# ArthurBrussee/brush

Hardware: AMD Instinct MI355X
Metric: train views/sec @ 1M Gaussians, 1080p (fwd + L1/SSIM loss + bwd + Adam per view) (higher is better)
Workload: dtype f32

## Files before the change

brush_amd/__init__.py:

```python
from .host import (
    Camera, Context, RasterPass, RenderAux, SplatTrainer, Splats, TrainConfig, SceneBatch,
    get_context, image_loss, image_loss_backward, image_loss_value_and_grad, prefix_sum, radix_argsort, tile_sort_offsets, render_splats,
    render_splats_bwd, adam_step, gather_stats, RefineStats, splat_bounds, bounds_median_size, fov_to_focal, focal_to_fov,
    splat_to_ply, load_splat_from_ply, ply_parse_header, ParseMetadata, BatchUploader, SceneLoader, set_list_slicing, last_list_counts, set_view_id,
    render_splats_diff, RenderNode, compute_pup_scores, decimate_to_count, lod_target_count, pup_accumulate, pup_accumulate_view, pup_scores,
    knn_log_scales, to_init_splats, load_init_splats, ply_vertex_has_property, EvalSample, EvalResult, eval_metrics, eval_stats, run_eval,
    Lpips, lpips, lpips_value_and_grad, splat_to_compressed_ply, view_output_size, resize_image, render_depth,
    PoseOptimizer, pose_twist, ExposureTable, depth_loss_value_and_grad, eval_depth_metrics,
    splat_normals, render_normal, depth_to_normal, depth_to_normal_backward, normal_consistency_value_and_grad,
    render_distortion, distortion_loss, BilateralGridTable,
    TsdfVolume, mesh_to_ply, fuse_views,
    render_features, feature_loss_value_and_grad, FeatureField,
    SceneTransform, SceneRegion, select_region, crop_splats,
    LiftAccumulator, lift_labels, compact_splats,
    EnvironmentMap,
)
from ._ffi import BrushHipError
```

brush_amd/_ffi.py:

```python
import ctypes as C
import os

_DIR = os.path.dirname(os.path.abspath(__file__))
LIB_PATH = os.environ.get("BRUSH_HIP_LIB") or os.path.join(_DIR, "libbrush_hip.so")

FLAG_MIP = 1
FLAG_BWD_INFO = 2
FLAG_SMOOTH_CUTOFF = 4
FLAG_SLICED_LISTS = 8

fp = C.POINTER(C.c_float)
u32p = C.POINTER(C.c_uint32)


class BhCamera(C.Structure):
    _fields_ = [
        ("vm", C.c_float * 12),
        ("fx", C.c_float), ("fy", C.c_float), ("cx", C.c_float), ("cy", C.c_float),
        ("lim_pos_x", C.c_float), ("lim_pos_y", C.c_float),
        ("lim_neg_x", C.c_float), ("lim_neg_y", C.c_float),
        ("cam_pos", C.c_float * 3),
        ("img_w", C.c_uint32), ("img_h", C.c_uint32),
        ("tile_row_begin", C.c_uint32), ("tile_row_end", C.c_uint32),
        ("model", C.c_uint32), ("dist", C.c_float * 8), ("half_max_render_fov", C.c_float),
# ... 353 lines not shown
REGION_BOX, REGION_ELLIPSOID = 0, 1


class BhSceneTransform(C.Structure):
    _fields_ = [("q", C.c_double * 4), ("t", C.c_double * 3), ("s", C.c_double), ("rot", C.c_float * 9), ("quat", C.c_float * 4),
                ("trans", C.c_float * 3), ("scale", C.c_float), ("log_scale", C.c_float), ("sh_rot", C.c_float * 164),
                ("reserved", C.c_uint32 * 2)]


class BhSceneRegion(C.Structure):
    _fields_ = [("kind", C.c_uint32), ("invert", C.c_uint32), ("center", C.c_float * 3), ("half_extent", C.c_float * 3),
                ("rot", C.c_float * 9), ("min_raw_opacity", C.c_float), ("reserved", C.c_uint32)]


SCENE_SYMBOLS = {
    "bh_scene_transform_make": (C.c_int, [dp, dp, C.c_double, C.POINTER(BhSceneTransform)]),
    "bh_scene_transform_compose": (C.c_int, [C.POINTER(BhSceneTransform), C.POINTER(BhSceneTransform), C.POINTER(BhSceneTransform)]),
    "bh_scene_transform_invert": (C.c_int, [C.POINTER(BhSceneTransform), C.POINTER(BhSceneTransform)]),
    "bh_camera_apply_scene_transform": (C.c_int, [C.POINTER(BhCamera), C.POINTER(BhSceneTransform), C.POINTER(BhCamera)]),
    "bh_splats_transform": (C.c_int, [C.c_void_p, C.POINTER(BhSceneTransform), C.c_uint32, C.c_uint32] + [C.c_void_p] * 6),
    "bh_splats_select_region": (C.c_int, [C.c_void_p, C.POINTER(BhSceneRegion), C.c_void_p, C.c_void_p, C.c_uint32, C.c_void_p, u32p]),
}

LIFT_MAX_LABELS, LIFT_UNASSIGNED, LIFT_ANY_LABEL = 256, 255, 0xFFFFFFFF
LIFT_VOTE_ONE = 16777216.0


class BhLiftSelect(C.Structure):
    _fields_ = [("label", C.c_uint32), ("min_share", C.c_float), ("min_weight", C.c_float), ("min_max_weight", C.c_float),
                ("min_pixels", C.c_uint32), ("invert", C.c_uint32)]


LIFT_SYMBOLS = {
    "bh_lift_accumulate": (C.c_int, [C.c_void_p, C.POINTER(BhRenderOut), C.c_void_p, C.c_uint32, C.c_void_p, C.c_void_p, C.c_void_p]),
    "bh_lift_assign": (C.c_int, [C.c_void_p, C.c_void_p, C.c_uint32, C.c_uint32, C.c_float, C.c_void_p, C.c_void_p]),
    "bh_lift_select": (C.c_int, [C.c_void_p, C.c_void_p, C.c_void_p, C.c_void_p, C.c_uint32, C.c_uint32, C.POINTER(BhLiftSelect), C.c_void_p]),
}

ENVMAP_MAX_RESOLUTION = 1024
ENVMAP_SYMBOLS = {
    "bh_envmap_create": (C.c_int, [C.c_void_p, C.c_uint32, C.POINTER(C.c_void_p)]),
    "bh_envmap_destroy": (C.c_int, [C.c_void_p, C.c_void_p]),
    "bh_envmap_set_params": (C.c_int, [C.c_void_p, C.c_void_p, fp]),
    "bh_envmap_get_params": (C.c_int, [C.c_void_p, C.c_void_p, fp]),
    "bh_envmap_get_grad": (C.c_int, [C.c_void_p, C.c_void_p, fp]),
    "bh_envmap_get_state": (C.c_int, [C.c_void_p, C.c_void_p, fp, fp, u32p]),
    "bh_envmap_set_state": (C.c_int, [C.c_void_p, C.c_void_p, fp, fp, C.c_uint32]),
    "bh_envmap_set_adam": (C.c_int, [C.c_void_p, C.c_void_p, C.c_double, C.c_double, C.c_double, C.c_double]),
    "bh_envmap_composite": (C.c_int, [C.c_void_p, C.c_void_p, C.POINTER(BhCamera), C.c_void_p, C.c_uint32, C.c_uint32, C.c_void_p]),
    "bh_envmap_backward": (C.c_int, [C.c_void_p, C.c_void_p, C.POINTER(BhCamera), C.c_void_p, C.c_void_p, C.c_uint32, C.c_uint32, C.c_void_p, C.c_int]),
    "bh_train_set_envmap": (C.c_int, [C.c_void_p, C.c_void_p]),
}

ABI_VERSION = 7
STRUCT_MIRRORS = (BhCamera, BhRenderOut, BhLossConfig, BhTrainConfig, BhTrainState, BhTrainBatch, BhTrainStats, BhRefineConfig, BhRefineStats, BhPlyInfo)

_lib = None
_lib_th = None
TEST_HOOKS_LIB_PATH = os.path.join(_DIR, "libbrush_hip_testhooks.so")
TEST_HOOK_SYMBOLS = {"bh_debug_fill_train_scratch": (C.c_int, [C.c_void_p, C.c_uint32]),
                     "bh_debug_split_counts": (C.c_int, [C.c_void_p, C.POINTER(C.c_uint32)])}


class BrushHipError(RuntimeError):
    pass


def _bind(path, symbols):
    if not os.path.exists(path):
        raise BrushHipError(
            "%s not found: build it with `python -c 'import __graft_entry__ as g; g.build()'` "
            "(hipcc --offload-arch=gfx950). There is no CPU fallback." % path)
    lib = C.CDLL(path)
    for name, (res, args) in symbols.items():
        fn = getattr(lib, name)
        fn.restype = res
        fn.argtypes = args
    if lib.bh_abi_version() != ABI_VERSION:
        raise BrushHipError("%s speaks ABI %d, this binding ABI %d" % (path, lib.bh_abi_version(), ABI_VERSION))
    for i, mirror in enumerate(STRUCT_MIRRORS):
        if lib.bh_struct_size(i) != C.sizeof(mirror):
            raise BrushHipError("%s: sizeof(%s) is %d in the library, %d in this binding" % (path, mirror.__name__, lib.bh_struct_size(i), C.sizeof(mirror)))
    return lib


def load():
    global _lib
    if _lib is None:
        _lib = _bind(LIB_PATH, dict(SYMBOLS, **LPIPS_SYMBOLS, **COMPRESSED_PLY_SYMBOLS, **IMAGE_SYMBOLS, **DEPTH_SYMBOLS, **POSE_SYMBOLS, **EXPOSURE_SYMBOLS, **BILAGRID_SYMBOLS, **DEPTH_LOSS_SYMBOLS, **NORMAL_SYMBOLS, **NORMAL_LOSS_SYMBOLS, **DISTORTION_SYMBOLS, **MESH_SYMBOLS, **FEATURE_SYMBOLS, **FEATURE_TRAIN_SYMBOLS, **SCENE_SYMBOLS, **LIFT_SYMBOLS, **ENVMAP_SYMBOLS))
    return _lib


def load_test_hooks():
    global _lib_th
    if _lib_th is None:
        _lib_th = _bind(TEST_HOOKS_LIB_PATH, dict(SYMBOLS, **LPIPS_SYMBOLS, **COMPRESSED_PLY_SYMBOLS, **IMAGE_SYMBOLS, **DEPTH_SYMBOLS, **POSE_SYMBOLS, **EXPOSURE_SYMBOLS, **BILAGRID_SYMBOLS, **DEPTH_LOSS_SYMBOLS, **NORMAL_SYMBOLS, **NORMAL_LOSS_SYMBOLS, **DISTORTION_SYMBOLS, **MESH_SYMBOLS, **FEATURE_SYMBOLS, **FEATURE_TRAIN_SYMBOLS, **SCENE_SYMBOLS, **LIFT_SYMBOLS, **ENVMAP_SYMBOLS,
                                                   **TEST_HOOK_SYMBOLS))
    return _lib_th
```

brush_amd/csrc/api.hip:

```cpp
#include <cmath>
#include <cstdlib>
#include <cstdio>
#include <algorithm>
#include <cstring>
#include <new>

#include "context.h"
#include "device_rng.h"
#include "param_table.h"

namespace bh {

__global__ __launch_bounds__(256) void zero_two_kernel(float4* __restrict__ a, size_t na, float4* __restrict__ b, size_t nb) {
    const size_t stride = (size_t)gridDim.x * 256;
    const float4 z = make_float4(0.0f, 0.0f, 0.0f, 0.0f);
    for (size_t i = (size_t)blockIdx.x * 256 + threadIdx.x; i < na + nb; i += stride) {
        if (i < na) a[i] = z;
        else b[i - na] = z;
    }
}

int set_error(bh_ctx* ctx, int code, const std::string& msg) {
    if (ctx) ctx->last_error = msg;
    return code;
// ... 317 lines not shown
        return true;
    }},
    {"cut_sort_all", "0|1: with per-tile cuts, still depth-sort every visible splat",
     [](bh_ctx* c, const char* v) { return parse_flag(v, &c->knob_cut_sort_all); }},
    {"auto_exact_share", "0..1: a view whose last cut frame listed more than this share of its pairs renders complete lists (default 0.9; 0 = never)", [](bh_ctx* c, const char* v) {
        char* end = nullptr;
        const float x = strtof(v, &end);
        if (end == v || *end != '\0' || !(x >= 0.0f && x <= 1.0f)) return false;
        c->auto_exact_share = x;
        return true;
    }},
    {"no_view_hash", "0|1: frames without a view id share ONE table instead of being keyed by their camera",
     [](bh_ctx* c, const char* v) { return parse_flag(v, &c->knob_no_view_hash); }},
    {"k16_order", "0 index order | 1 by the view's last per-tile work | 2 dealt: the forward blend's tile order",
     [](bh_ctx* c, const char* v) { return parse_u32(v, 0, 2, &c->knob_k16_order); }},
    {"band_mode", "0|1: XCD bands of the blend kernels — contiguous eighths of the tile range, or dealt in chunks of 8 adjacent tiles (default 1)",
     [](bh_ctx* c, const char* v) { return parse_u32(v, 0, 1, &c->knob_band_mode); }},
    {"k16_waves", "0..8: forward blend: resident one-wave tiles per SIMD (0 = 8 = all resident at once; fewer: the lighter tiles are dispatched as the heavier ones finish)",
     [](bh_ctx* c, const char* v) { return parse_u32(v, 0, 8, &c->knob_k16_waves); }},
    {"k16_split", "0..1000: forward blend: a tile whose forecast work is at least max(256, k16_split / 100 x its band's mean) is blended by four quadrant waves (default 250; 0: no tile is split)",
     [](bh_ctx* c, const char* v) { return parse_u32(v, 0, 1000, &c->knob_k16_split); }},
    {"k16_split_of_max", "0..100: ... and at least this many percent of its band's heaviest tile (default 45)",
     [](bh_ctx* c, const char* v) { return parse_u32(v, 0, 100, &c->knob_k16_split_of_max); }},
    {"k16_split_min", "1..1023: a tile below this many blended splats (forecast) is never split (default 256)",
     [](bh_ctx* c, const char* v) { return parse_u32(v, 1, 1023, &c->knob_k16_split_min); }},
    {"k5_exact_spw", "16|32|64: splats per wave of the list builder for complete lists",
     [](bh_ctx* c, const char* v) { uint32_t u = 0; if (!parse_u32(v, 16, 64, &u) || !(u == 16 || u == 32 || u == 64)) return false; c->knob_k5_exact_spw = u; return true; }},
    {"bwd_jobs", "0|1: the blend backward works on checkpointed 128-entry segments of the tiles' lists (default 1) or on whole tiles",
     [](bh_ctx* c, const char* v) { return parse_flag(v, &c->knob_bwd_jobs); }},
    {"bwd_wide_rows", "0|1: the blend backward addresses the gradient accumulator in 64 bits, as it does by itself from 2^32 bytes of accumulator on (default 0)",
     [](bh_ctx* c, const char* v) { return parse_flag(v, &c->knob_bwd_wide_rows); }},
    {"no_lpt", "0|1: the blend backward takes its tiles in index order",
     [](bh_ctx* c, const char* v) { return parse_flag(v, &c->knob_no_lpt); }},
    {"lpt_classes", "log|linear: work classes of the backward's longest-first tile order — two per octave of blended splats, or 1/64 of the mean list length wide",
     [](bh_ctx* c, const char* v) { const std::string w(v); if (w == "log") { c->knob_lpt_linear = false; return true; } if (w == "linear") { c->knob_lpt_linear = true; return true; } return false; }},
    {"generic_depth_sort", "0|1: depth order by the generic radix sort + scan instead of the fused split sort",
     [](bh_ctx* c, const char* v) { return parse_flag(v, &c->knob_generic_depth_sort); }},
    {"dsort_splitters", "0|1: the fused depth sort splits at the 254 depth quantiles of the view's previous frame (default 1) or always linearly over the frame's key range",
     [](bh_ctx* c, const char* v) { return parse_flag(v, &c->knob_dsort_splitters); }},
    {"tile_sort", "auto|bucket|lsd: the forward's tile sort (auto: bucket sort unless the view's pairs are concentrated in few tiles)",
     [](bh_ctx* c, const char* v) { const std::string w(v); if (w == "auto") { c->knob_tile_sort = 0; return true; } if (w == "bucket") { c->knob_tile_sort = 1; return true; } if (w == "lsd") { c->knob_tile_sort = 2; return true; } return false; }},
    {"spec_k5", "0|1: queue the list builder before the host has read the frame's counts (default 1; 0: behind the count readback)",
     [](bh_ctx* c, const char* v) { return parse_flag(v, &c->knob_spec_k5); }},
    {"event_waits", "0|1: the host's mid-step waits use events behind the kernels instead of polled tag words",
     [](bh_ctx* c, const char* v) { return parse_flag(v, &c->knob_event_waits); }},
    {"readback_copy", "0|1: counts and gate word reach the host through copy launches",
     [](bh_ctx* c, const char* v) { return parse_flag(v, &c->knob_readback_copy); }},
    {"force_exchange", "0|1: a one-rank communicator still walks the whole gradient-exchange path (overhead measurement)",
     [](bh_ctx* c, const char* v) { return parse_flag(v, &c->knob_force_exchange); }},
    {"zero_grads", "0|1: the single-GPU train step zero-fills its gradient span like the exchange path",
     [](bh_ctx* c, const char* v) { return parse_flag(v, &c->knob_zero_grads); }},
    {"loss_bands", "0|1: the fused loss's blocks take their tiles by XCD column bands (1) or row-major (0)",
     [](bh_ctx* c, const char* v) { return parse_u32(v, 0, 1, &c->knob_loss_bands); }},
    {"update_rows", "0|64|128|256: splats per block of the update kernel (0 = default)",
     [](bh_ctx* c, const char* v) { uint32_t u = 0; if (!parse_u32(v, 0, 256, &u) || !(u == 0 || u == 64 || u == 128 || u == 256)) return false; c->knob_update_rows = u; return true; }},
    {"no_dormant", "0|1: the update kernel fetches and updates dormant splats like everyone else",
     [](bh_ctx* c, const char* v) { return parse_flag(v, &c->knob_no_dormant); }},
    {"sort_kpt", "0|4|8|16: keys per thread of the generic radix sort (0 = default)",
     [](bh_ctx* c, const char* v) { uint32_t u = 0; if (!parse_u32(v, 0, 16, &u) || !(u == 0 || u == 4 || u == 8 || u == 16)) return false; c->knob_sort_kpt = u; return true; }},
    {"grad_allreduce", "ring|direct: the dense gradient block's collective — ncclAllReduce, or reduce-scatter + all-gather over grouped send/recv",
     [](bh_ctx* c, const char* v) { const std::string w(v); if (w == "ring") { c->knob_direct_allreduce = false; return true; } if (w == "direct") { c->knob_direct_allreduce = true; return true; } return false; }},
    {"update_sparse", "0..256: an update block with at most this many non-dormant rows fetches them in one round trip (0: never; 256: every block that may skip dormant rows; default 64 at SH degree 0, else 0)",
     [](bh_ctx* c, const char* v) { uint32_t u = 0; if (!parse_u32(v, 0, 256, &u)) return false; c->knob_update_sparse = (int)u; return true; }},
    {"feature_chunk", "0|4|8|16: channels per pass over the lists of the feature-map blends (0 = chosen per channel count)",
     [](bh_ctx* c, const char* v) { uint32_t u = 0; if (!parse_u32(v, 0, 16, &u) || !(u == 0 || u == 4 || u == 8 || u == 16)) return false; c->feature_chunk = u; return true; }},
};
constexpr int kOptionCount = (int)(sizeof(kOptions) / sizeof(kOptions[0]));
}

extern "C" int bh_option_count(void) { return kOptionCount; }
extern "C" const char* bh_option_name(int i) { return i >= 0 && i < kOptionCount ? kOptions[i].name : nullptr; }
extern "C" const char* bh_option_help(int i) { return i >= 0 && i < kOptionCount ? kOptions[i].help : nullptr; }

extern "C" int bh_set_option(bh_ctx* ctx, const char* key, const char* value) {
    if (!ctx) return BH_ERR_INVALID_ARG;
    if (!key || !value) return set_error(ctx, BH_ERR_INVALID_ARG, "set_option: null key or value");
    const std::string k(key);
    for (const Option& o : kOptions) {
        if (k != o.name) continue;
        if (!o.apply(ctx, value)) return set_error(ctx, BH_ERR_INVALID_ARG, "set_option: bad value '" + std::string(value) + "' for '" + k + "'");
        return 0;
    }
    return set_error(ctx, BH_ERR_INVALID_ARG, "set_option: unknown key '" + k + "' (bh_option_name lists the keys)");
}

namespace {
struct Kb4Law {
    double k[4];
    explicit Kb4Law(const float* d) { for (int i = 0; i < 4; ++i) k[i] = d ? (double)d[i] : 0.0; }
    double value(double th) const {
        const double t2 = th * th, t3 = t2 * th, t5 = t3 * t2, t7 = t5 * t2, t9 = t7 * t2;
        return th + k[0] * t3 + k[1] * t5 + k[2] * t7 + k[3] * t9;
    }
    double slope(double th) const {
        const double t2 = th * th, t4 = t2 * t2, t6 = t4 * t2, t8 = t6 * t2;
        return 1.0 + 3.0 * k[0] * t2 + 5.0 * k[1] * t4 + 7.0 * k[2] * t6 + 9.0 * k[3] * t8;
    }
    double invert(double target) const {
        if (target <= 0.0) return 0.0;
        const double pi = 3.14159265358979323846;
        double th = target < pi - 1e-6 ? target : pi - 1e-6;
        for (int it = 0; it < 50; ++it) {
            const double fp = slope(th);
            if (std::fabs(fp) < 1e-12) break;
            double next = th - (value(th) - target) / fp;
            next = next < 0.0 ? 0.0 : (next > pi ? pi : next);
// ... 750 lines not shown
    BH_HIP(ctx, hipMemcpyAsync(info, ctx->slots[SLOT_SLICE].ptr, sizeof info, hipMemcpyDeviceToHost, ctx->stream));
    BH_HIP(ctx, hipStreamSynchronize(ctx->stream));
    deliver_pending_loss(ctx);
    *near_pairs = info[1];
    *far_pairs = info[2] ? info[3] : 0u;
    return 0;
}

const float* bh_last_v_combined(bh_ctx* ctx) { return ctx ? (const float*)ctx->slots[SLOT_V_COMBINED].ptr : nullptr; }

int bh_radix_argsort(bh_ctx* ctx, const uint32_t* keys, const uint32_t* vals, uint32_t n, uint32_t bits,
                     uint32_t* out_keys, uint32_t* out_vals) {
    if (!ctx) return BH_ERR_INVALID_ARG;
    if (n > 0 && (!keys || !out_keys || !out_vals)) return set_error(ctx, BH_ERR_INVALID_ARG, "radix_argsort: null argument");
    BH_HIP(ctx, hipSetDevice(ctx->device));
    return radix_argsort(ctx, keys, vals, n, bits, out_keys, out_vals);
}

int bh_prefix_sum(bh_ctx* ctx, const uint32_t* in, uint32_t n, uint32_t* out) {
    if (!ctx) return BH_ERR_INVALID_ARG;
    if (n > 0 && (!in || !out)) return set_error(ctx, BH_ERR_INVALID_ARG, "prefix_sum: null argument");
    BH_HIP(ctx, hipSetDevice(ctx->device));
    return prefix_sum(ctx, in, nullptr, n, out, false);
}

int bh_image_loss_forward(bh_ctx* ctx, const float* pred_chw, const uint32_t* gt_packed, uint32_t channels, uint32_t h,
                          uint32_t w, const BhLossConfig* cfg, float* loss_map) {
    if (!ctx) return BH_ERR_INVALID_ARG;
    if (!pred_chw || !gt_packed || !cfg || !loss_map || h == 0 || w == 0) return set_error(ctx, BH_ERR_INVALID_ARG, "image_loss_forward: bad argument");
    BH_HIP(ctx, hipSetDevice(ctx->device));
    return launch_image_loss_forward(ctx, pred_chw, gt_packed, channels, h, w, *cfg, loss_map);
}

int bh_image_loss_backward(bh_ctx* ctx, const float* pred_chw, const uint32_t* gt_packed, const float* dl_dmap,
                           uint32_t channels, uint32_t h, uint32_t w, const BhLossConfig* cfg, float* dl_dpred) {
    if (!ctx) return BH_ERR_INVALID_ARG;
    if (!pred_chw || !gt_packed || !dl_dmap || !cfg || !dl_dpred || h == 0 || w == 0) return set_error(ctx, BH_ERR_INVALID_ARG, "image_loss_backward: bad argument");
    BH_HIP(ctx, hipSetDevice(ctx->device));
    return launch_image_loss_backward(ctx, pred_chw, gt_packed, dl_dmap, 0.0f, channels, h, w, *cfg, dl_dpred);
}

int bh_image_loss_value_and_grad(bh_ctx* ctx, const float* img_hwc4, const uint32_t* gt_packed, uint32_t h, uint32_t w,
                                 const BhLossConfig* cfg, float alpha_weight, float* loss_out, float* v_output) {
    if (!ctx) return BH_ERR_INVALID_ARG;
    if (!img_hwc4 || !gt_packed || !cfg || !loss_out || !v_output || h == 0 || w == 0)
        return set_error(ctx, BH_ERR_INVALID_ARG, "image_loss_value_and_grad: bad argument");
    BH_HIP(ctx, hipSetDevice(ctx->device));
    const size_t hw = (size_t)h * w;
    const bool alpha = alpha_weight > 0.0f;
    return launch_image_loss_fused(ctx, img_hwc4, gt_packed, h, w, *cfg, alpha, 1.0f / (float)(hw * 3), alpha ? alpha_weight / (float)hw : 0.0f,
                                   loss_out, v_output);
}

int bh_adam_step(bh_ctx* ctx, float* param, const float* grad, float* m1, float* m2, uint64_t rows, uint32_t row_len,
                 const float* col_scale, float lr, uint32_t t, int reduce_m2, float beta1, float beta2, float eps) {
    if (!ctx) return BH_ERR_INVALID_ARG;
    if (rows > 0 && (!param || !grad || !m1 || !m2)) return set_error(ctx, BH_ERR_INVALID_ARG, "adam_step: null argument");
    BH_HIP(ctx, hipSetDevice(ctx->device));
    return launch_adam(ctx, param, grad, m1, m2, rows, row_len, col_scale, lr, t, reduce_m2 != 0, beta1, beta2, eps);
}

int bh_gather_stats(bh_ctx* ctx, float* refine_weight_norm, float* vis_weight, float* max_screen_size,
                    const float* refine_weight, const float* visible, const float* screen_radius, uint64_t n) {
    if (!ctx) return BH_ERR_INVALID_ARG;
    BH_HIP(ctx, hipSetDevice(ctx->device));
    return launch_gather_stats(ctx, refine_weight_norm, vis_weight, max_screen_size, refine_weight, visible, screen_radius, n);
}

void bh_philox4x32_10(const uint32_t ctr[4], const uint32_t key[2], uint32_t out[4]) {
    const Philox4 r = philox4x32_10(ctr[0], ctr[1], ctr[2], ctr[3], key[0], key[1]);
    out[0] = r.x; out[1] = r.y; out[2] = r.z; out[3] = r.w;
}

void bh_sample_background(uint64_t seed, uint32_t step, const float base[3], float strength, float out[3]) {
    float u[3] = {0.5f, 0.5f, 0.5f};
    if (strength > 0.0f) {
        const Philox4 r = philox4x32_10(0u, step, 0u, RNG_STREAM_BACKGROUND, (uint32_t)seed, (uint32_t)(seed >> 32));
        u[0] = unit_open(r.x); u[1] = unit_open(r.y); u[2] = unit_open(r.z);
    }
    for (int k = 0; k < 3; ++k) {
        const float v = strength > 0.0f ? base[k] + (2.0f * u[k] - 1.0f) * strength : base[k];
        out[k] = v < 0.0f ? 0.0f : (v > 1.0f ? 1.0f : v);
    }
}

int bh_normal_samples(bh_ctx* ctx, uint64_t seed, uint32_t step, uint64_t n, float* out) {
    if (!ctx) return BH_ERR_INVALID_ARG;
    if (n > 0 && !out) return set_error(ctx, BH_ERR_INVALID_ARG, "normal_samples: null argument");
    if (n > 0xFFFFFFFFull) return set_error(ctx, BH_ERR_INVALID_ARG, "normal_samples: n must fit 32 bits (the splat index is one counter word)");
    BH_HIP(ctx, hipSetDevice(ctx->device));
    return launch_normal_samples(ctx, out, n, seed, step);
}

int bh_fold_min_scale(bh_ctx* ctx, const float* transforms, const float* raw_opacities, const float* min_scale, uint32_t n,
                      float* out_transforms, float* out_raw_opacities) {
    if (!ctx) return BH_ERR_INVALID_ARG;
    if (n > 0 && (!transforms || !raw_opacities || !min_scale || !out_transforms || !out_raw_opacities))
        return set_error(ctx, BH_ERR_INVALID_ARG, "fold_min_scale: null argument");
    BH_HIP(ctx, hipSetDevice(ctx->device));
    return launch_fold_min_scale(ctx, transforms, raw_opacities, min_scale, n, out_transforms, out_raw_opacities);
}

int bh_fold_min_scale_backward(bh_ctx* ctx, const float* transforms, const float* raw_opacities, const float* min_scale, uint32_t n,
                               float* v_transforms, float* v_raw_opacities) {
    if (!ctx) return BH_ERR_INVALID_ARG;
    if (n > 0 && (!transforms || !raw_opacities || !min_scale || !v_transforms || !v_raw_opacities))
// ... 44 lines not shown
```

brush_amd/csrc/context.h:

```cpp
#pragma once
#include <hip/hip_runtime.h>
#include <stdint.h>

#include <memory>
#include <string>
#include <unordered_map>
#include <vector>

#include "../../include/brush_hip.h"
#include "../../include/brush_hip_lpips.h"
#include "../../include/brush_hip_image.h"
#include "../../include/brush_hip_exposure.h"
#include "../../include/brush_hip_bilagrid.h"
#include "../../include/brush_hip_depth_loss.h"
#include "../../include/brush_hip_normal_loss.h"
#include "../../include/brush_hip_distortion.h"
#include "../../include/brush_hip_mesh.h"
#include "../../include/brush_hip_features.h"
#include "../../include/brush_hip_feature_train.h"
#include "../../include/brush_hip_envmap.h"
#include "device_math.h"

namespace bh {

enum Slot : int {
    SLOT_COUNTERS = 0,
    SLOT_DEPTH_KEYS,
    SLOT_ISECT_COUNTS,
    SLOT_MAX_RADIUS,
    SLOT_SORT_KEYS_A,
    SLOT_SORT_KEYS_B,
    SLOT_SORT_VALS_A,
    SLOT_SORT_VALS_B,
    SLOT_SORT_HIST,
    SLOT_COMM_SCRATCH,
    SLOT_BWD_CKPT,
    SLOT_BWD_TOPLIST,
    SLOT_SORT_PARTS,
    SLOT_SCAN_SUMS,
    SLOT_GLOBAL_FROM_COMPACT,
    SLOT_DEPTHS_SORTED,
    SLOT_CUM_TILES_HIT,
    SLOT_PROJECTED,
    SLOT_TILE_IDS,
    SLOT_ISECT_GIDS,
    SLOT_TILE_IDS_SORTED,
    SLOT_ISECT_GIDS_SORTED,
    SLOT_TILE_OFFSETS,
    SLOT_OUT_IMG,
    SLOT_VISIBLE,
    SLOT_V_COMBINED,
    SLOT_LOSS_MAP,
    SLOT_V_OUTPUT,
    SLOT_GRADS,
    SLOT_STATS,
    SLOT_LOSS_SCALAR,
    SLOT_MISC,
    SLOT_REFINE,
    SLOT_REFINE_BOUNDS,
    SLOT_FOLDED_TRANSFORMS,
    SLOT_FOLDED_RAW_OPAC,
    SLOT_PLY_ROWS,
    SLOT_EXCH_BLOCKS,
    SLOT_EXCH_IDX,
    SLOT_EXCH_COMPACT,
    SLOT_PROJECTED_BY_GID,
    SLOT_SLICE,
    SLOT_SLICE_STATE,
    SLOT_SLICE_COUNTS,
    SLOT_SLICE_CUM,
    SLOT_NEAR_COUNTS,
    SLOT_TILE_ORDER,
    SLOT_LOD_GRADS,
// ... 227 lines not shown
struct ParamTable;

struct DistortionTerm {
    const float* v_distortion = nullptr;
    float gain = 0.0f;
    uint32_t kind = 0;
    float near_z = 0.0f, far_z = 0.0f;
    const float* moments = nullptr;
};

struct FeatureTerm {
    const float* features = nullptr;
    uint32_t channels = 0;
    const float* v_map = nullptr;
    float* v_features = nullptr;
    const float* map_acc = nullptr;
    const float* compact = nullptr;
};

struct BackwardCall {
    const float* transforms = nullptr;
    const float* sh_coeffs = nullptr;
    const float* raw_opacities = nullptr;
    float* v_transforms = nullptr;
    float* v_sh_coeffs = nullptr;
    float* v_raw_opacities = nullptr;
    float* v_refine_weight = nullptr;
    size_t span_floats = 0;
    bool want_refine = true;
    const DepthTerm* depth = nullptr;
    const NormalTerm* normal = nullptr;
    const DistortionTerm* distortion = nullptr;
    const FeatureTerm* feature = nullptr;
    float* v_viewmat = nullptr;
};

struct StepTerms {
    const bh_lpips* lpips = nullptr;
    float lpips_weight = 0.0f;
    float* pose_grad = nullptr;
    bool depth_attached = false;
    BhDepthTarget depth_target{};
    bool normal_attached = false;
    BhNormalTermConfig normal_term{};
    bool distortion_attached = false;
    BhDistortionTermConfig distortion_term{};
    bool feature_attached = false;
    BhFeatureField feature_field{};
    BhFeatureTarget feature_target{};
    bh_exposure* exposure = nullptr;
    bh_bilagrid* bilagrid = nullptr;
    float bilagrid_tv_weight = 0.0f;
    bh_envmap* envmap = nullptr;

    bool lpips_on() const { return lpips != nullptr && lpips_weight > 0.0f; }
    bool depth_on() const { return depth_attached && depth_target.weight > 0.0f; }
    bool normal_on() const { return normal_attached && normal_term.weight > 0.0f; }
    bool distortion_on() const { return distortion_attached; }
    bool feature_on() const { return feature_attached && feature_target.weight > 0.0f; }
};

}


struct bh_ctx {
    int device = 0;
    hipStream_t stream = nullptr;
    bool owns_stream = false;
    std::string last_error;
    bh::Buffer slots[bh::SLOT_COUNT];
    uint32_t* host_counters = nullptr;
    hipEvent_t readback_ev = nullptr;
    hipEvent_t gate_ev = nullptr;
    bool counters_ready = false;
    uint32_t counter_phase = 0;
    bool have_forward = false;
    bh::ForwardState latest;
    uint64_t generation = 0;
    std::vector<bh::Retained> retained;
    std::vector<bh::Buffer> pool;
    bh::GradClears clears;
    float* pending_loss_dst = nullptr;
    void* image_tab_host = nullptr;
    size_t image_tab_cap = 0;
    hipEvent_t image_tab_ev = nullptr;
    bh::StepTerms terms;
    std::vector<bh::ParamTable*> param_tables;
    void* comm = nullptr;
    hipStream_t comm_stream = nullptr;
    hipEvent_t comm_ev = nullptr;
    int comm_rank = 0, comm_world = 1;
    float slice_fraction = 0.0f;
    float last_slice_share = 1.0f;
    bool far_direct = false;
    uint32_t readback_tag = 0;
    uint32_t gate_tag = 0;
    bool gate_signal_queued = false;
    bool gate_learn = false;
    uint32_t far_launches = 0;
    std::unordered_map<uint64_t, bh::ViewState> views;
    uint64_t seen_keys[bh::SEEN_KEYS] = {};
    uint32_t seen_pos = 0;
    uint32_t casual_views = 0;
    uint32_t view_id = 0;
    uint64_t view_clock = 0;
    float margin_scale = 1.0f;
    float ctrl_up = 1.5f, ctrl_down = 0.998f, ctrl_floor = 0.5f, ctrl_gap_exp = 1.0f / 3.0f;
    uint32_t cut_min_pairs = bh::CUT_MIN_PAIRS;
    bool knob_spec_k5 = true;
    bool knob_event_waits = false;
    bool knob_readback_copy = false;
    bool knob_no_view_hash = false;
    bool knob_fixed_margin = false;
    bool knob_cut_sort_all = false;
    uint32_t feature_chunk = 0;
    uint32_t knob_band_mode = 1;
    uint32_t knob_k16_waves = 0;
    uint32_t knob_k16_split = 250;
    uint32_t knob_k16_split_min = bh::SPLIT_MIN_WORK;
    uint32_t knob_k16_split_of_max = 45;
    const uint32_t* last_split = nullptr;
    uint32_t knob_k16_order = 1;
    uint32_t knob_cut_margin_pct = 150;
    bh::FarJob far_job;
    uint32_t refine_n = 0, refine_new_n = 0;
    bool dsort_lds_raised = false;
    uint32_t* sort_groups = nullptr;
    size_t sort_groups_cap = 0, sort_groups_dirty = 0;
    uint32_t sort_groups_cur = 0;
    uint32_t* dsort_spl = nullptr;
    bool dsort_spl_written = false;
    bool knob_dsort_splitters = true;
    bool adam_lds_raised = false;
    uint32_t update_lds_raised = 0;
    size_t lds_optin_max = 0;
    bool knob_no_lpt = false;
    bool knob_bwd_wide_rows = false;
    bool knob_bwd_jobs = true;
    bool knob_lpt_linear = false;
    bool knob_force_exchange = false;
    bool knob_break_allreduce = false;
    bool knob_generic_depth_sort = false;
    bool knob_zero_grads = false;
    uint32_t knob_fail_loss_at = 0;
    uint32_t train_steps_seen = 0;
    uint32_t knob_loss_bands = 1;
    uint32_t knob_tile_sort = 0;
    float auto_exact_share = 0.9f;
    bool knob_direct_allreduce = false;
    uint32_t knob_k5_exact_spw = 32;
    bool knob_no_dormant = false;
    int knob_update_sparse = -1;
    uint32_t knob_update_rows = 0;
    uint32_t knob_sort_kpt = 0;
    const void* marks_m2_sh = nullptr; const void* marks_m1_t = nullptr; uint32_t marks_n = 0, marks_step = 0;
    bh::Profiler prof;
};

namespace bh {

int set_error(bh_ctx* ctx, int code, const std::string& msg);
int forward_impl(bh_ctx* ctx, const ForwardRequest& req, BhRenderOut* out);
int wait_host_tag(bh_ctx* ctx, const volatile uint32_t* word, uint32_t want, const char* what);
int find_saved_bwd_forward(bh_ctx* ctx, const BhRenderOut* saved, int not_bwd_code, const char* who, const ForwardState** fs);
int backward_impl(bh_ctx* ctx, const ForwardState& fs, const float* v_output, const BackwardCall& call);
int render_forward(bh_ctx* ctx, const ForwardRequest& req, BhRenderOut* out);
enum : uint32_t { NEED_V_OUTPUT = 1u, NEED_V_DEPTH = 2u, NEED_V_NORMAL = 4u, NEED_V_DISTORTION = 8u, NEED_V_VIEWMAT = 16u, NEED_V_FEATURES = 32u };
int backward_entry(bh_ctx* ctx, const char* who, int not_bwd_code, uint32_t required, const BhRenderOut* saved, const float* v_output, BackwardCall call);
int launch_depth_backward(bh_ctx* ctx, const ForwardState& fs, const DepthTerm& term, float* v_combined, float** v_z);
int launch_depth_vz_scatter(bh_ctx* ctx, const ForwardState& fs, const float* v_z, float* v_transforms, bool mark_rows, float* v_sh_coeffs,
                            float* v_raw_opacities, float* v_refine_weight);
int launch_depth_forward(bh_ctx* ctx, const ForwardState& fs, uint32_t mode, float* out_depth);
int launch_normal_backward(bh_ctx* ctx, const ForwardState& fs, const NormalTerm& term, const float* transforms, float* v_combined, const float** v_n);
int launch_normal_vn_scatter(bh_ctx* ctx, const ForwardState& fs, const float* v_n, const float* transforms, float* v_transforms, bool mark_rows,
                             float* v_sh_coeffs, float* v_raw_opacities, float* v_refine_weight);
int launch_normal_map(bh_ctx* ctx, const ForwardState& fs, const float* transforms, uint32_t mode, float* out);
int launch_normal_loss(bh_ctx* ctx, const BhCamera& cam, const float* normal, const float* depth, const float* image, uint32_t h, uint32_t w, float weight,
                       bool accumulate_v_depth, float* loss, float* v_normal, float* v_depth, float* accum, float* accum_host);
int launch_distortion_backward(bh_ctx* ctx, const ForwardState& fs, const DistortionTerm& term, float* v_combined, float** v_z);
int launch_distortion_map(bh_ctx* ctx, const ForwardState& fs, const DistortionTerm& term, bool moments, float* out);
int check_distortion_kind(bh_ctx* ctx, uint32_t kind, float near_z, float far_z, const char* who);
int launch_distortion_loss(bh_ctx* ctx, const float* map, uint32_t h, uint32_t w, uint32_t channels, float weight, float* loss, float* accum,
                           float* accum_host);
int launch_feature_backward(bh_ctx* ctx, const ForwardState& fs, const FeatureTerm& term, float* v_combined, const float** v_compact);
int launch_feature_scatter(bh_ctx* ctx, const ForwardState& fs, const FeatureTerm& term, const float* v_compact);
int launch_feature_gather(bh_ctx* ctx, const ForwardState& fs, const float* features, uint32_t channels, float* feat);
int launch_feature_forward(bh_ctx* ctx, const ForwardState& fs, uint32_t channels, const float* feat, float* out);
int feature_term_rows(bh_ctx* ctx, const ForwardState& fs, uint32_t channels, float** feat);
int launch_feature_loss(bh_ctx* ctx, const float* map, const BhFeatureTarget& t, float* loss, float* v_map, float* accum, float* accum_host);
int launch_depth_loss(bh_ctx* ctx, const float* depth, const BhDepthTarget& t, float* loss, float* v_depth, float* accum, float* accum_host);
double* loss_partials(bh_ctx* ctx, uint64_t pixels, uint32_t* blocks);
int launch_loss_pair_final(bh_ctx* ctx, uint32_t rows, const double* partials, float c, float* loss, float* accum, float* accum_host);
int launch_pose_grad(bh_ctx* ctx, const ViewUniforms& u, uint32_t nv, bool mip, uint32_t sh_degree, const float* transforms,
                     const float* sh, const uint32_t* gid, const float* v_combined, float* v_viewmat);
int launch_exposure_apply(bh_ctx* ctx, const bh_exposure* tab, uint32_t view, const float* img, uint32_t h, uint32_t w, float* out);
int launch_exposure_backward(bh_ctx* ctx, bh_exposure* tab, uint32_t view, const float* img, const float* v_exposed, uint32_t h, uint32_t w,
                             float* v_img, bool update);
int launch_bilagrid_slice(bh_ctx* ctx, const bh_bilagrid* tab, uint32_t view, const float* img, uint32_t h, uint32_t w, float* out);
// ... 95 lines not shown
                         float* projected, const uint32_t* cum_tiles_hit, uint32_t* tile_ids, uint32_t* isect_gids,
                         float4* zero_span = nullptr, uint32_t zero_f4 = 0, uint32_t budget = 0xFFFFFFFFu, uint32_t* slice_info = nullptr,
                         const uint32_t* zcut = nullptr, const uint32_t* depth_keys_sorted = nullptr, const uint32_t* nv_dev = nullptr, uint32_t pair_cap = 0xFFFFFFFFu);
int launch_map_gaussians_far(bh_ctx* ctx, uint32_t nv, const ViewUniforms& u, const float* projected_by_gid, const uint32_t* gid,
                             float* projected, const uint32_t* cum_tiles_hit, uint32_t budget, const uint32_t* done_bits, const uint32_t* gate,
                             uint32_t* counts, uint32_t* block_totals, uint32_t* group_totals, uint32_t* slice_info, uint32_t* tile_ids, uint32_t* isect_gids);
int launch_project_backward(bh_ctx* ctx, const ViewUniforms& u, uint32_t nv, bool mip, uint32_t sh_degree,
                            const float* transforms, const float* sh, const float* raw_opac, const uint32_t* gid,
                            float* v_combined, float* v_transforms, float* v_sh, float* v_raw_opac,
                            float* v_refine, bool mark_written = false, const float* projected = nullptr);
struct SortGroups {
    uint32_t* sums = nullptr;
    uint32_t* stale = nullptr;
    uint32_t stale_words = 0;
};
inline uint32_t sort_group_count(uint32_t nblocks) { return (nblocks + SORT_GROUP_BLOCKS - 1u) / SORT_GROUP_BLOCKS; }
int sort_groups_next(bh_ctx* ctx, size_t words, SortGroups* out);
constexpr uint32_t SORT_DIRECT_GROUPS = 32;
inline bool sort_groups_scanned(uint32_t ngroups) { return ngroups > SORT_DIRECT_GROUPS; }
int sort_groups_scan(bh_ctx* ctx, uint32_t* sums, uint32_t ngroups, uint32_t tables, uint32_t* totals);
int radix_argsort(bh_ctx* ctx, const uint32_t* keys, const uint32_t* vals, uint32_t n, uint32_t bits,
                  uint32_t* out_keys, uint32_t* out_vals);
int radix_argsort_dev(bh_ctx* ctx, const uint32_t* keys, const uint32_t* vals, uint32_t n_max, const uint32_t* n_dev, const uint32_t* gate,
                      const uint32_t* out_base, uint32_t bits, uint32_t* out_keys, uint32_t* out_vals, uint32_t alloc_n = 0);
bool tile_sort_supported(uint32_t bits, uint32_t n);
int tile_sort_offsets(bh_ctx* ctx, const uint32_t* keys, const uint32_t* vals, uint32_t n, uint32_t bits, uint32_t num_tiles,
                      uint32_t* out_keys, uint32_t* out_vals, uint32_t* tile_offsets, uint32_t alloc_n = 0);
bool depth_sort_supported(uint32_t n);
int depth_sort_scan(bh_ctx* ctx, const uint32_t* keys, const uint32_t* minmax, const uint32_t* counts, uint32_t n, uint32_t* out_keys,
                    uint32_t* out_vals, uint32_t* cum, const uint32_t* rb_set = nullptr, uint32_t* rb_host = nullptr, hipEvent_t rb_done = nullptr,
                    uint32_t rb_tag = 0, uint32_t* rb_dev = nullptr, uint32_t* spl = nullptr, bool* spl_written = nullptr);
int prefix_sum(bh_ctx* ctx, const uint32_t* in, const uint32_t* gather, uint32_t n, uint32_t* out, bool exclusive, const uint32_t* gate = nullptr);
int launch_tile_offsets(bh_ctx* ctx, const uint32_t* tile_ids_sorted, uint32_t num_isect, uint32_t num_tiles,
                        uint32_t* tile_offsets, bool pre_zeroed = false);
int launch_tile_offsets_dev(bh_ctx* ctx, const uint32_t* tile_ids_sorted, uint32_t n_max, const uint32_t* n_dev, const uint32_t* gate,
                            const uint32_t* base, uint32_t num_tiles, uint32_t* tile_offsets);

int launch_rasterize(bh_ctx* ctx, const ViewUniforms& u, const float bg[3], bool bwd_info, bool smooth,
                     const uint32_t* isect_gids, uint32_t* tile_offsets, const float* projected,
                     const uint32_t* global_from_compact, float* out_img, uint32_t* out_packed, float* visible,
                     uint32_t* lpt, float class_width, int phase = 0, const RasterSlice* slice = nullptr);
int launch_rasterize_backward(bh_ctx* ctx, const ViewUniforms& u, const float bg[3], bool smooth,
                              const uint32_t* isect_gids, const uint32_t* tile_offsets, const float* projected,
                              const float* out_img, const float* v_output, float* v_combined, const uint32_t* lpt,
                              const uint32_t* tile_offsets_far = nullptr, bool want_refine = true, const BwdJobs* jobs = nullptr,
                              uint32_t accum_rows = 0u);
int launch_image_loss_forward(bh_ctx* ctx, const float* pred, const uint32_t* gt, uint32_t channels, uint32_t h,
                              uint32_t w, const BhLossConfig& cfg, float* loss_map);
int launch_image_loss_backward(bh_ctx* ctx, const float* pred, const uint32_t* gt, const float* dl_dmap,
                               float dl_const, uint32_t channels, uint32_t h, uint32_t w, const BhLossConfig& cfg,
                               float* dl_dpred);
int launch_image_loss_fused(bh_ctx* ctx, const float* img_hwc4, const uint32_t* gt, uint32_t h, uint32_t w, const BhLossConfig& cfg,
                            bool alpha_match, float dl_rgb, float dl_alpha, float* loss_out, float* v_output, float* loss_host = nullptr,
                            uint32_t* started_host = nullptr, uint32_t started_tag = 0);
int launch_image_loss_fused_window(bh_ctx* ctx, const float* img_hwc4, const uint32_t* gt, uint32_t h, uint32_t w, const BhLossConfig& cfg,
                                   bool alpha_match, float dl_rgb, float dl_alpha, uint32_t tile_y0, uint32_t tile_y1, float* loss_out,
                                   float* v_output, float* loss_host = nullptr, uint32_t* started_host = nullptr, uint32_t started_tag = 0);
int launch_adam(bh_ctx* ctx, float* param, const float* grad, float* m1, float* m2, uint64_t rows, uint32_t row_len,
                const float* col_scale, float lr, uint32_t t, bool reduce_m2, float beta1, float beta2, float eps, float gscale = 1.0f);
struct NoiseArgs { uint64_t seed; uint32_t step; float scale, clamp_abs; };
struct UpdateCall {
    const float *g_transforms, *g_sh, *g_opac;
    const float *refine_weight, *visible, *screen_radius;
    float gscale;
    bool vis_clamp;
    float tab_t[10];
    float lr_sh, sh_rest_scale, lr_opac;
    uint32_t t;
    float beta1, beta2, eps;
    const NoiseArgs* noise;
    bool masked_rows;
};
int launch_train_update(bh_ctx* ctx, const BhTrainState* st, const UpdateCall& c);
int launch_gather_stats(bh_ctx* ctx, float* refine_weight_norm, float* vis_weight, float* max_screen_size,
                        const float* refine_weight, const float* visible, const float* screen_radius, uint64_t n);
int launch_mean_noise(bh_ctx* ctx, float* transforms, const float* raw_opac, const float* visible,
                      const float* samples, uint64_t n, float noise_scale, float clamp_abs, uint64_t seed = 0, uint32_t step = 0);
int launch_normal_samples(bh_ctx* ctx, float* out, uint64_t n, uint64_t seed, uint32_t step);

int launch_fold_min_scale(bh_ctx* ctx, const float* transforms, const float* raw_opac, const float* min_scale, uint32_t n,
                          float* out_transforms, float* out_raw_opac);
int launch_fold_min_scale_backward(bh_ctx* ctx, const float* transforms, const float* raw_opac, const float* min_scale, uint32_t n,
                                   float* v_transforms, float* v_raw_opac);
int launch_compute_min_scale(bh_ctx* ctx, const float* transforms, uint32_t n, const float* view_cams, uint32_t k, float factor, float* out);

int comm_allreduce(bh_ctx* ctx, float* buf, uint64_t count, bool max_op);
int comm_exchange_strip_halos(bh_ctx* ctx, float* img, uint32_t h, uint32_t w, uint32_t row_begin_px, uint32_t row_end_px);

int launch_union_index(bh_ctx* ctx, const float* visible_sum, uint32_t n, uint32_t* block_scratch , uint32_t* count_dev,
                       uint32_t* idx);
int launch_exchange_rows(bh_ctx* ctx, bool gather, const uint32_t* idx, uint32_t count, uint32_t c3, float* g_tr, float* g_sh, float* g_op,
                         float* g_ref , float* compact);

}
```

brush_amd/csrc/loss_fused.hip:

```cpp
#include <cmath>
#include <cstdio>
#include <cstring>

#include "context.h"

#pragma clang fp contract(fast)

namespace bh {

namespace {

constexpr int LB = 16;
constexpr int HALO = 5;
constexpr float SSIM_C1 = 0.01f * 0.01f;
constexpr float SSIM_C2 = 0.03f * 0.03f;
constexpr float INV_255 = 1.0f / 255.0f;

struct Taps { float w[11]; };

Taps gauss_taps() {
    Taps g;
    const float sigma = 1.5f;
    float sum = 0.0f;
    for (int i = 0; i < 11; ++i) {
        const float x = (float)i - 5.0f;
        g.w[i] = expf(-x * x / (2.0f * sigma * sigma));
        sum += g.w[i];
    }
    for (int i = 0; i < 11; ++i) g.w[i] /= sum;
    return g;
}

#define BH_TAP_0 0x1.0d957p-10f
#define BH_TAP_1 0x1.f1fe04p-8f
#define BH_TAP_2 0x1.26eb18p-5f
#define BH_TAP_3 0x1.bff1p-4f
#define BH_TAP_4 0x1.b43c4p-3f
#define BH_TAP_5 0x1.106562p-2f
constexpr float TAP_TABLE[11] = {BH_TAP_0, BH_TAP_1, BH_TAP_2, BH_TAP_3, BH_TAP_4, BH_TAP_5, BH_TAP_4, BH_TAP_3, BH_TAP_2, BH_TAP_1, BH_TAP_0};
BH_DEV constexpr float tap(int i) { return TAP_TABLE[i]; }
BH_DEV float in_vgpr(float x) {
    asm volatile("" : "+v"(x));
    return x;
}

int taps_mismatch() {
    const Taps g = gauss_taps();
    for (int i = 0; i < 11; ++i)
        if (memcmp(&g.w[i], &TAP_TABLE[i], sizeof(float)) != 0) return i;
    return -1;
}

struct FusedArgs {
    uint32_t h, w;
    float l1_w, ssim_w;
    float bg[3];
    int composite, mask, alpha_match;
    float dl_rgb, dl_alpha;
    uint32_t ty_base;
    uint32_t row_end;
    const float* sum_src;
    int sum_n;
    float* loss_out;
    float* loss_host;
    uint32_t* started_host;
    uint32_t started_tag;
    uint32_t gx, gy_blocks, band_w;
};

BH_DEV bool loss_tile(const FusedArgs& a, uint32_t& bx, uint32_t& by, uint32_t& linear) {
    if (a.band_w == 0u) {
        bx = blockIdx.x; by = blockIdx.y;
        linear = by * a.gx + bx;
        return true;
    }
    const uint32_t b = blockIdx.x, xcd = b & 7u, j = b >> 3;
    const uint32_t x0 = xcd * a.band_w;
    if (x0 >= a.gx) return false;
    const uint32_t wb = min(a.band_w, a.gx - x0);
    by = j / wb;
    bx = x0 + (j - by * wb);
    linear = b;
    return by < a.gy_blocks;
}

BH_DEV float gt_ch(uint32_t val, uint32_t c) { return (float)((val >> (c * 8u)) & 0xffu) * INV_255; }

}

namespace {
constexpr int TW = 16, TH = 32;
constexpr int SW = TW + 2 * HALO;
constexpr int SR = TH + 2 * HALO;
#define BH_LOSS_HP 88
#define BH_LOSS_H2P 24
constexpr int HP = BH_LOSS_HP;
constexpr int H2P = BH_LOSS_H2P;
}

__global__ __launch_bounds__(256) void loss_fused_forward_kernel(const float* __restrict__ img ,
                                                                const uint32_t* __restrict__ gt,
                                                                float* __restrict__ partials ,
                                                                float* __restrict__ block_sums , uint32_t gy, FusedArgs a) {
    __shared__ float2 s_tile[3][SR * SW];
    __shared__ float s_h[(SR - 1) * HP + TW * 5];
    float* s_red = s_h;
    if (a.started_host && blockIdx.x == 0 && blockIdx.y == 0 && threadIdx.x == 0 && threadIdx.y == 0)
        *reinterpret_cast<volatile uint32_t*>(a.started_host) = a.started_tag;
    uint32_t bx, by, blin;
    if (!loss_tile(a, bx, by, blin)) return;
    const int tx0 = (int)bx * TW, ty0 = (int)a.ty_base * LB + (int)by * TH;
    const int lx = threadIdx.x, ly = threadIdx.y;
    const int rank = ly * TW + lx;
    const size_t plane = (size_t)a.h * a.w;
    constexpr int TILE_LOADS = (SR * SW + 255) / 256;
    float lx3[TILE_LOADS][3];
    uint32_t lval[TILE_LOADS];
    bool lin[TILE_LOADS];
    const int pxx = tx0 + lx;
    const int py[2] = {ty0 + 2 * ly, ty0 + 2 * ly + 1};
    const bool inside[2] = {pxx < (int)a.w && py[0] < (int)a.h, pxx < (int)a.w && py[1] < (int)a.h};
    uint32_t own_val[2] = {0u, 0u};
#pragma unroll
    for (int k = 0; k < TILE_LOADS; ++k) {
        const int i = rank + 256 * k;
        const int r = i / SW, q = i - r * SW;
        const int y = ty0 + r - HALO, x = tx0 + q - HALO;
        lin[k] = i < SR * SW && y >= 0 && x >= 0 && y < (int)a.h && x < (int)a.w;
        const int yc = y < 0 ? 0 : (y >= (int)a.h ? (int)a.h - 1 : y), xc = x < 0 ? 0 : (x >= (int)a.w ? (int)a.w - 1 : x);
        const size_t p = (size_t)yc * a.w + (size_t)xc;
        const float* ip = &img[p * 4];
        lx3[k][0] = ip[0]; lx3[k][1] = ip[1]; lx3[k][2] = ip[2];
        lval[k] = gt[p];
    }
#pragma unroll
    for (int o = 0; o < 2; ++o) {
        const int yc = py[o] >= (int)a.h ? (int)a.h - 1 : py[o], xc = pxx >= (int)a.w ? (int)a.w - 1 : pxx;
        own_val[o] = gt[(size_t)yc * a.w + (size_t)xc];
    }
#pragma unroll
    for (int k = 0; k < TILE_LOADS; ++k) {
        const int i = rank + 256 * k;
        if (i < SR * SW) {
            float g0 = 0.f, g1 = 0.f, g2 = 0.f;
            if (!lin[k]) lx3[k][0] = lx3[k][1] = lx3[k][2] = 0.0f;
            if (lin[k]) {
                const uint32_t val = lval[k];
                const float ga = gt_ch(val, 3);
                g0 = gt_ch(val, 0); g1 = gt_ch(val, 1); g2 = gt_ch(val, 2);
                if (a.composite) {
                    g0 = g0 + (1.0f - ga) * a.bg[0];
                    g1 = g1 + (1.0f - ga) * a.bg[1];
                    g2 = g2 + (1.0f - ga) * a.bg[2];
                }
            }
            s_tile[0][i] = make_float2(lx3[k][0], g0);
            s_tile[1][i] = make_float2(lx3[k][1], g1);
            s_tile[2][i] = make_float2(lx3[k][2], g2);
        }
    }
    float ga[2] = {0.f, 0.f}, chain[2] = {0.f, 0.f};
#pragma unroll
    for (int o = 0; o < 2; ++o) {
        if (inside[o]) {
            ga[o] = gt_ch(own_val[o], 3);
            chain[o] = a.mask ? a.dl_rgb * ga[o] : a.dl_rgb;
        }
    }
    float acc_rgb = 0.0f;
    const float tap4 = in_vgpr(tap(4)), l1_w = in_vgpr(a.l1_w), ssim_w = in_vgpr(a.ssim_w);
#pragma unroll 1
    for (int c = 0; c < 3; ++c) {
        __syncthreads();
        const int probe_rows = SR * (TW / 2);
        for (int i = rank; i < probe_rows; i += 256) {
            const int r = i / (TW / 2), pair = i - r * (TW / 2);
            const float2* row = &s_tile[c][r * SW + 2 * pair];
            float x[12], y[12], xx[12], yy[12], xy[12];
#pragma unroll
            for (int k = 0; k < 12; ++k) {
                const float2 v = row[k];
                x[k] = v.x; y[k] = v.y;
                xx[k] = v.x * v.x; yy[k] = v.y * v.y; xy[k] = v.x * v.y;
            }
#pragma unroll
            for (int o = 0; o < 2; ++o) {
                const int cc = HALO + o;
                float sx = 0, sx2 = 0, sy = 0, sy2 = 0, sxy = 0;
#pragma unroll
                for (int d = 1; d < 6; ++d) {
                    const float wd = d == 1 ? tap4 : tap(5 - d);
                    sx += (x[cc - d] + x[cc + d]) * wd;
                    sx2 += (xx[cc - d] + xx[cc + d]) * wd;
                    sy += (y[cc - d] + y[cc + d]) * wd;
                    sy2 += (yy[cc - d] + yy[cc + d]) * wd;
                    sxy += (xy[cc - d] + xy[cc + d]) * wd;
                }
                const float wc = tap(5);
                sx += x[cc] * wc;
                sx2 += xx[cc] * wc;
                sy += y[cc] * wc;
                sy2 += yy[cc] * wc;
                sxy += xy[cc] * wc;
                float* op = &s_h[r * HP + (2 * pair + o) * 5];
                op[0] = sx; op[1] = sx2; op[2] = sy; op[3] = sy2; op[4] = sxy;
            }
        }
        __syncthreads();
        float v[12][5];
#pragma unroll
        for (int r = 0; r < 12; ++r) {
            const float* t = &s_h[(2 * ly + r) * HP + lx * 5];
#pragma unroll
            for (int k = 0; k < 5; ++k) v[r][k] = t[k];
        }
#pragma unroll
        for (int o = 0; o < 2; ++o) {
            float m[5] = {0.f, 0.f, 0.f, 0.f, 0.f};
#pragma unroll
            for (int d = 1; d < 6; ++d) {
                const float wd = d == 1 ? tap4 : tap(5 - d);
#pragma unroll
                for (int k = 0; k < 5; ++k) m[k] += (v[o + 5 - d][k] + v[o + 5 + d][k]) * wd;
            }
#pragma unroll
            for (int k = 0; k < 5; ++k) m[k] += v[o + 5][k] * tap(5);
            if (!inside[o]) continue;
            const float mu1 = m[0], mu2 = m[2];
            const float mu1_sq = mu1 * mu1, mu2_sq = mu2 * mu2;
            const float s1 = __builtin_fmaxf(0.0f, m[1] - mu1_sq), s2 = __builtin_fmaxf(0.0f, m[3] - mu2_sq);
            const float s12 = m[4] - mu1 * mu2;
            const float A = mu1_sq + mu2_sq + SSIM_C1;
            const float B = s1 + s2 + SSIM_C2;
            const float c_top = 2.0f * mu1 * mu2 + SSIM_C1;
            const float d_top = 2.0f * s12 + SSIM_C2;
            const float inv_a = __builtin_amdgcn_rcpf(A), inv_b = __builtin_amdgcn_rcpf(B);
            const float inv_ab = inv_a * inv_b;
            const float cd = c_top * d_top * inv_ab;
            const float ssim = clampf(cd, -1.0f, 1.0f);
            const float2 pg = s_tile[c][(2 * ly + o + HALO) * SW + lx + HALO];
            float lv = __builtin_fmaf(l1_w, __builtin_fabsf(pg.x - pg.y), ssim_w * ssim);
            if (a.mask) lv = lv * ga[o];
            acc_rgb += lv;
            const bool clamped = cd < -1.0f || cd > 1.0f;
            const float dmu1 = clamped ? 0.0f : 2.0f * mu2 * inv_ab * (d_top - c_top) - 2.0f * mu1 * cd * (inv_a - inv_b);
            const float ds1 = clamped ? 0.0f : -cd * inv_b;
            const float ds12 = clamped ? 0.0f : 2.0f * c_top * inv_ab;
            const size_t p = (size_t)py[o] * a.w + (size_t)pxx;
            float* o3 = partials + (size_t)(c * 3) * plane + p;
            o3[0] = dmu1 * chain[o];
            o3[plane] = ds1 * chain[o];
            o3[2 * plane] = ds12 * chain[o];
        }
    }
    float acc_alpha = 0.0f;
    if (a.alpha_match) {
#pragma unroll
        for (int o = 0; o < 2; ++o) {
            if (inside[o]) {
                const float pa = img[((size_t)py[o] * a.w + (size_t)pxx) * 4 + 3];
                float vv = __builtin_fabsf(pa - ga[o]);
                if (a.mask) vv = vv * ga[o];
                acc_alpha += vv;
            }
        }
    }
    float acc = acc_rgb * a.dl_rgb + acc_alpha * a.dl_alpha;
#pragma unroll
    for (int off = 32; off > 0; off >>= 1) acc += __shfl_down(acc, off);
    __syncthreads();
    if ((rank & 63) == 0) s_red[rank >> 6] = acc;
    __syncthreads();
    if (rank < 2) {
        const uint32_t tile_row = a.ty_base + 2u * by + (uint32_t)rank;
        if (tile_row < gy) block_sums[(size_t)tile_row * a.gx + bx] = s_red[2 * rank] + s_red[2 * rank + 1];
    }
}

#define BH_LOSSB_WAVES 1
__global__ __launch_bounds__(256, BH_LOSSB_WAVES) void loss_fused_backward_kernel(const float* __restrict__ img, const uint32_t* __restrict__ gt,
                                                                 const float* __restrict__ partials ,
                                                                 float* __restrict__ v_output , FusedArgs a) {
    __shared__ __align__(8) float s_part[3][SR * SW];
    __shared__ __align__(8) float s_h2[3][SR * H2P];
    const int lx = threadIdx.x, ly = threadIdx.y;
    const int rank = ly * TW + lx;
    const size_t plane = (size_t)a.h * a.w;
    if (blockIdx.x == 0 && blockIdx.y == 0 && a.loss_out) {
        __shared__ float s_w[4];
        float acc = 0.0f;
        for (int i = rank; i < a.sum_n; i += 256) acc += a.sum_src[i];
#pragma unroll
        for (int off = 32; off > 0; off >>= 1) acc += __shfl_down(acc, off);
        if ((rank & 63) == 0) s_w[rank >> 6] = acc;
        __syncthreads();
        if (rank == 0) {
            const float total = (s_w[0] + s_w[1]) + (s_w[2] + s_w[3]);
            a.loss_out[0] = total;
            if (a.loss_host) a.loss_host[0] = total;
        }
    }
    uint32_t bx, by, blin;
    if (!loss_tile(a, bx, by, blin)) return;
    const int tx0 = (int)bx * TW, ty0 = (int)a.ty_base * LB + (int)by * TH;
    const int pxx = tx0 + lx;
    const int py[2] = {ty0 + 2 * ly, ty0 + 2 * ly + 1};
    const bool inside[2] = {pxx < (int)a.w && py[0] < (int)a.h && py[0] < (int)a.row_end, pxx < (int)a.w && py[1] < (int)a.h && py[1] < (int)a.row_end};
    float4 pv[2];
    uint32_t val[2] = {0u, 0u};
#pragma unroll
    for (int o = 0; o < 2; ++o) {
        pv[o] = make_float4(0.f, 0.f, 0.f, 0.f);
        if (inside[o]) {
            const size_t p = (size_t)py[o] * a.w + (size_t)pxx;
            pv[o] = *reinterpret_cast<const float4*>(&img[p * 4]);
            val[o] = gt[p];
        }
    }
    float out[2][4] = {{0.f, 0.f, 0.f, 0.f}, {0.f, 0.f, 0.f, 0.f}};
    const bool wide_rows = (a.w & 3u) == 0u && (plane & 3u) == 0u && (reinterpret_cast<uintptr_t>(partials) & 15u) == 0;
    constexpr int ROW_ITEMS = 3 * SR * 8;
    auto fetch_rows = [&](const int c, float4 (&dst)[4]) {
        const float* pc = partials + (size_t)(c * 3) * plane;
#pragma unroll
        for (int t = 0; t < 4; ++t) {
            const int i = rank + 256 * t;
            dst[t] = make_float4(0.0f, 0.0f, 0.0f, 0.0f);
            if (i < ROW_ITEMS) {
// ... 66 lines not shown
                    for (int d = 1; d < 6; ++d) acc += (x[cc - d] + x[cc + d]) * (d == 1 ? tap4 : tap(5 - d));
                    acc += x[cc] * tap(5);
                    res[o] = acc;
                }
                *reinterpret_cast<float2*>(dst + 32 * n * H2P) = make_float2(res[0], res[1]);
            }
        }
        __syncthreads();
        float v[3][12];
#pragma unroll
        for (int j = 0; j < 3; ++j)
#pragma unroll
            for (int r = 0; r < 12; ++r) v[j][r] = s_h2[j][(2 * ly + r) * H2P + lx];
#pragma unroll
        for (int o = 0; o < 2; ++o) {
            float sres[3];
#pragma unroll
            for (int j = 0; j < 3; ++j) {
                float acc = 0.0f;
#pragma unroll
                for (int d = 1; d < 6; ++d) acc += (v[j][o + 5 - d] + v[j][o + 5 + d]) * (d == 1 ? tap4 : tap(5 - d));
                acc += v[j][o + 5] * tap(5);
                sres[j] = acc;
            }
            const float ga = gt_ch(val[o], 3);
            float chain_c = a.dl_rgb;
            if (a.mask) chain_c = chain_c * ga;
            float ge = gt_ch(val[o], c);
            if (a.composite) ge = ge + (1.0f - ga) * a.bg[c];
            const float p1 = c == 0 ? pv[o].x : (c == 1 ? pv[o].y : pv[o].z);
            const float ssim_grad = sres[0] + (2.0f * p1) * sres[1] + ge * sres[2];
            const float diff = p1 - ge;
            const float l1_sign = diff > 0.0f ? 1.0f : (diff < 0.0f ? -1.0f : 0.0f);
            out[o][c] = __builtin_fmaf(ssim_w, ssim_grad, l1_w * l1_sign * chain_c);
        }
    }
#pragma unroll
    for (int o = 0; o < 2; ++o) {
        if (!inside[o]) continue;
        if (a.alpha_match) {
            const float ga = gt_ch(val[o], 3);
            const float diff = pv[o].w - ga;
            const float sign = diff > 0.0f ? 1.0f : (diff < 0.0f ? -1.0f : 0.0f);
            float chain = a.dl_alpha;
            if (a.mask) chain = chain * ga;
            out[o][3] = sign * chain;
        }
        *reinterpret_cast<float4*>(&v_output[((size_t)py[o] * a.w + (size_t)pxx) * 4]) = make_float4(out[o][0], out[o][1], out[o][2], out[o][3]);
    }
}

int launch_image_loss_fused_window(bh_ctx* ctx, const float* img_hwc4, const uint32_t* gt, uint32_t h, uint32_t w, const BhLossConfig& cfg,
                                   bool alpha_match, float dl_rgb, float dl_alpha, uint32_t tile_y0, uint32_t tile_y1, float* loss_out,
                                   float* v_output, float* loss_host, uint32_t* started_host, uint32_t started_tag) {
    const uint32_t gx = (w + LB - 1) / LB, gy = (h + LB - 1) / LB;
    if (tile_y1 > gy) tile_y1 = gy;
    if (tile_y0 >= tile_y1) return set_error(ctx, BH_ERR_INVALID_ARG, "image loss: empty tile-row window");
    static const int bad_tap = taps_mismatch();
    if (bad_tap >= 0) {
        char msg[160];
        snprintf(msg, sizeof msg, "image loss: Gaussian tap %d is %a on this host, the kernels' table holds %a", bad_tap, (double)gauss_taps().w[bad_tap],
                 (double)TAP_TABLE[bad_tap]);
        return set_error(ctx, BH_ERR_UNSUPPORTED, msg);
    }
    const uint32_t a0 = tile_y0 > 0 ? tile_y0 - 1 : 0, a1 = tile_y1 < gy ? tile_y1 + 1 : gy;
    const dim3 block(TW, 16);
    const bool banded = ctx->knob_loss_bands != 0u && gx >= 16u;
    const size_t hw = (size_t)h * w;
    auto* partials = (float*)ensure(ctx, SLOT_LOSS_MAP, hw * 12 * sizeof(float));
    auto* block_sums = (float*)ensure(ctx, SLOT_MISC, (size_t)gx * gy * sizeof(float));
    if (!partials || !block_sums) return BH_ERR_OOM;
    FusedArgs a;
    a.h = h; a.w = w;
    a.l1_w = cfg.l1_weight; a.ssim_w = cfg.ssim_weight;
    a.bg[0] = cfg.bg[0]; a.bg[1] = cfg.bg[1]; a.bg[2] = cfg.bg[2];
    a.composite = cfg.composite_bg; a.mask = cfg.mask; a.alpha_match = alpha_match ? 1 : 0;
    a.dl_rgb = dl_rgb; a.dl_alpha = dl_alpha;
    {
        ProfScope ps(ctx, "ImageLoss");
        a.ty_base = a0;
        a.row_end = h;
        a.sum_src = nullptr; a.sum_n = 0; a.loss_out = nullptr; a.loss_host = nullptr;
        a.started_host = started_host; a.started_tag = started_tag;
        a.gx = gx; a.gy_blocks = (a1 - a0 + 1) / 2;
        a.band_w = banded ? (gx + 7u) / 8u : 0u;
        const dim3 grid_a = banded ? dim3(8u * a.band_w * a.gy_blocks) : dim3(gx, a.gy_blocks);
        hipLaunchKernelGGL(loss_fused_forward_kernel, grid_a, block, 0, ctx->stream, img_hwc4, gt, partials, block_sums, a1, a);
        BH_LAUNCH_CHECK(ctx, "loss_fused_forward_kernel");
    }
    {
        ProfScope ps(ctx, "ImageLossBackward");
        a.ty_base = tile_y0;
        a.row_end = tile_y1 * LB < h ? tile_y1 * LB : h;
        a.sum_src = block_sums + (size_t)tile_y0 * gx;
        a.sum_n = (int)((tile_y1 - tile_y0) * gx);
        a.loss_out = loss_out;
        a.loss_host = loss_host;
        a.started_host = nullptr; a.started_tag = 0;
        a.gy_blocks = (tile_y1 - tile_y0 + 1) / 2;
        const dim3 grid_b = banded ? dim3(8u * a.band_w * a.gy_blocks) : dim3(gx, a.gy_blocks);
        hipLaunchKernelGGL(loss_fused_backward_kernel, grid_b, block, 0, ctx->stream, img_hwc4, gt, partials, v_output, a);
        BH_LAUNCH_CHECK(ctx, "loss_fused_backward_kernel");
    }
    return 0;
}

int launch_image_loss_fused(bh_ctx* ctx, const float* img_hwc4, const uint32_t* gt, uint32_t h, uint32_t w, const BhLossConfig& cfg,
                            bool alpha_match, float dl_rgb, float dl_alpha, float* loss_out, float* v_output, float* loss_host, uint32_t* started_host,
                            uint32_t started_tag) {
    return launch_image_loss_fused_window(ctx, img_hwc4, gt, h, w, cfg, alpha_match, dl_rgb, dl_alpha, 0, (h + LB - 1) / LB, loss_out, v_output, loss_host,
                                          started_host, started_tag);
}

}
```

brush_amd/csrc/train.hip:

```cpp
#include <cmath>
#include <string>

#include "context.h"
#include "param_table.h"

using namespace bh;

namespace {

struct StepArgs {
    const BhTrainConfig* cfg;
    BhTrainState* st;
    const BhTrainBatch* batch;
    bh_grad_hook hook;
    void* hook_user;
    float grad_scale;
    BhTrainStats* stats;
};

struct StepPlan {
    bool lpips = false, depth = false, normal = false, distortion = false, feature = false;
    bh_exposure* exposure = nullptr;
    bh_bilagrid* bilagrid = nullptr;
    bh_envmap* envmap = nullptr;
    uint32_t tile_y0 = 0, tile_y1 = 0;
    bool whole_frame = true, window_partial = false;
    bool native_tiles = false, tile_mode = false;
    bool exchanging = false;
    bool keyed = false;
    bool masked_grads = false;
    uint32_t n = 0, C = 0, W = 0, H = 0;
    uint32_t step = 0;
    size_t o_tr = 0, o_sh = 0, o_op = 0, o_ref = 0, exch_count = 0;
};

struct StepWork {
    float* exch = nullptr;
    float* s_radius = nullptr;
    const float* r_transforms = nullptr;
    const float* r_raw_opac = nullptr;
    BhRenderOut ro{};
    float* v_output = nullptr;
    float* loss_dev = nullptr;
    float* loss_host = nullptr;
    float* composited = nullptr;
    float* corrected = nullptr;
    BackwardCall bwd;
    DepthTerm depth_term;
    NormalTerm normal_term;
    DistortionTerm distortion_term;
    FeatureTerm feature_term;
    float* v_features = nullptr;
    uint32_t* union_idx = nullptr;
    bool flags_on_side = false;
    float* visible() const { return exch; }
    float* frame() const { return composited ? composited : ro.out_img; }
};

struct LossCall {
    BhLossConfig lc{};
    bool alpha_match = false;
    float dl_rgb = 0.0f, dl_alpha = 0.0f;
};

int refuse_partial_frame(bh_ctx* ctx, const char* term) {
    return set_error(ctx, BH_ERR_INVALID_ARG, std::string("train_step: the ") + term + " needs the whole frame on this rank (no tile-row partition)");
}
int refuse_with_pose_grad(bh_ctx* ctx, const char* a_term, const char* the_term) {
    return set_error(ctx, BH_ERR_INVALID_ARG, std::string("train_step: ") + a_term + " and a pose-gradient buffer cannot be attached together (the pose pass does not carry the " +
                                                  the_term + "'s gradient)");
}
int check_frame_and_pose(bh_ctx* ctx, const StepPlan& p, const char* the_term, const char* a_term) {
    if (!p.whole_frame) return refuse_partial_frame(ctx, the_term);
    if (a_term && ctx->terms.pose_grad) return refuse_with_pose_grad(ctx, a_term, the_term);
    return 0;
}

// ... 5 lines not shown
        return set_error(ctx, BH_ERR_INVALID_ARG, "train_step: null state tensor");
    StepPlan& p = *plan;
    const StepTerms& t = ctx->terms;
    const BhCamera& cam = batch->camera;
    const ViewUniforms win_u = make_uniforms(cam);
    p.tile_y0 = win_u.tile_y0;
    p.tile_y1 = win_u.tile_y1;
    p.window_partial = win_u.tile_y0 != 0u || win_u.tile_y1 != win_u.tile_bh;
    p.whole_frame = !batch->image_hook && !p.window_partial;
    if ((p.exposure = t.exposure)) {
        if (batch->view_id == 0u || batch->view_id > p.exposure->n_views)
            return set_error(ctx, BH_ERR_INVALID_ARG, "train_step: with an exposure table the batch's view_id must be 1 .. n_views");
        BH_TRY(check_frame_and_pose(ctx, p, "exposure term", nullptr));
    }
    if ((p.bilagrid = t.bilagrid)) {
        if (p.exposure)
            return set_error(ctx, BH_ERR_INVALID_ARG, "train_step: an exposure table and a bilateral-grid table cannot be attached together (they are alternatives: detach one)");
        if (batch->view_id == 0u || batch->view_id > p.bilagrid->n_views)
            return set_error(ctx, BH_ERR_INVALID_ARG, "train_step: with a bilateral-grid table the batch's view_id must be 1 .. n_views");
        BH_TRY(check_frame_and_pose(ctx, p, "bilateral-grid term", nullptr));
        if ((uint64_t)cam.img_w * cam.img_h > 0x7FFFFFFFull)
            return set_error(ctx, BH_ERR_INVALID_ARG, "train_step: with a bilateral-grid table h * w must stay below 2^31");
    }
    if ((p.envmap = t.envmap)) {
        if (cam.model != BH_CAMERA_PINHOLE)
            return set_error(ctx, BH_ERR_INVALID_ARG, "train_step: the environment map needs a pinhole camera (no other model can be unprojected to a ray)");
        BH_TRY(check_frame_and_pose(ctx, p, "environment map", "an environment map"));
        if (batch->has_alpha && !batch->alpha_is_mask)
            return set_error(ctx, BH_ERR_INVALID_ARG, "train_step: an environment map and a target with real alpha cannot be combined (a mask is fine)");
        if ((uint64_t)cam.img_w * cam.img_h > 0x7FFFFFFFull)
            return set_error(ctx, BH_ERR_INVALID_ARG, "train_step: with an environment map h * w must stay below 2^31");
    }
    if ((p.depth = t.depth_on())) {
        const BhDepthTarget& d = t.depth_target;
        if (!d.gt) return set_error(ctx, BH_ERR_INVALID_ARG, "train_step: the depth target has no depth map");
        if (d.h != cam.img_h || d.w != cam.img_w) return set_error(ctx, BH_ERR_INVALID_ARG, "train_step: the depth target's size differs from the camera's");
        if (d.kind > BH_DEPTH_LOSS_DISPARITY) return set_error(ctx, BH_ERR_INVALID_ARG, "train_step: unknown depth loss kind");
        BH_TRY(check_frame_and_pose(ctx, p, "depth term", "a depth target"));
    }
    if ((p.normal = t.normal_on())) {
        if (cam.model != BH_CAMERA_PINHOLE)
            return set_error(ctx, BH_ERR_INVALID_ARG, "train_step: the normal term needs a pinhole camera (the normals of a depth map are defined for it alone)");
        BH_TRY(check_frame_and_pose(ctx, p, "normal term", "a normal term"));
    }
    if ((p.distortion = t.distortion_on())) BH_TRY(check_frame_and_pose(ctx, p, "distortion term", "a distortion term"));
    if ((p.feature = t.feature_on())) {
        BH_TRY(check_frame_and_pose(ctx, p, "feature term", "a feature term"));
        if (t.feature_field.n != st->n)
            return set_error(ctx, BH_ERR_INVALID_ARG, "train_step: the feature term's field has " + std::to_string(t.feature_field.n) + " rows, the state " +
                                                          std::to_string(st->n) + " splats (a refine re-rows the splats: carry the field with bh_refine_carry_rows)");
        if (t.feature_target.h != cam.img_h || t.feature_target.w != cam.img_w)
            return set_error(ctx, BH_ERR_INVALID_ARG, "train_step: the feature term's target size differs from the camera's");
    }
    p.exchanging = hook || (ctx->comm && (ctx->comm_world > 1 || ctx->knob_force_exchange));
    p.native_tiles = !batch->image_hook && p.window_partial && ctx->comm != nullptr && !hook && (batch->strip_loss || ctx->comm_world > 1);
    if (p.native_tiles && !batch->strip_loss)
        return set_error(ctx, BH_ERR_INVALID_ARG, "train_step: a tile-row window without an image hook needs strip_loss = 1 (the library exchanges the strips' halos, not whole frames)");
    p.tile_mode = batch->image_hook != nullptr || p.native_tiles;
    if ((p.lpips = t.lpips_on()) && !p.whole_frame) return refuse_partial_frame(ctx, "LPIPS term");
    p.n = st->n;
    p.C = (st->sh_degree + 1) * (st->sh_degree + 1);
    p.W = cam.img_w;
    p.H = cam.img_h;
    p.step = st->step_count + 1;
    p.masked_grads = !p.exchanging && !p.tile_mode && !ctx->knob_zero_grads && p.n > 0;
    p.keyed = p.exchanging && batch->exchange_mode == 1 && p.n > 0;
    auto pad4 = [](size_t x) { return (x + 3) & ~(size_t)3; };
    p.o_tr = pad4(p.n);
    p.o_sh = p.o_tr + pad4((size_t)p.n * 10);
    p.o_op = p.o_sh + pad4((size_t)p.n * 3 * p.C);
    p.o_ref = p.o_op + pad4(p.n);
    p.exch_count = p.o_ref + pad4(p.n);
    return 0;
}

int sum_over_ranks(bh_ctx* ctx, const StepArgs& a, float* ptr, uint64_t cnt) {
    if (a.hook) return a.hook(a.hook_user, ptr, cnt) == 0 ? 0 : set_error(ctx, BH_ERR_STATE, "gradient hook failed");
    return comm_allreduce(ctx, ptr, cnt, false);
}

int step_buffers(bh_ctx* ctx, const StepArgs& a, const StepPlan& p, StepWork& w) {
    const BhTrainState* st = a.st;
    w.exch = (float*)ensure(ctx, SLOT_GRADS, (p.exch_count ? p.exch_count : 4) * 4);
    w.s_radius = (float*)ensure(ctx, SLOT_STATS, (size_t)(p.n ? p.n : 1) * 4);
    if (!w.exch || !w.s_radius) return BH_ERR_OOM;
    w.r_transforms = st->transforms;
    w.r_raw_opac = st->raw_opacities;
    if (st->min_scale && p.n > 0) {
        ProfScope ps(ctx, "FoldMinScale");
        auto* ft = (float*)ensure(ctx, SLOT_FOLDED_TRANSFORMS, (size_t)p.n * 10 * 4);
        auto* fo = (float*)ensure(ctx, SLOT_FOLDED_RAW_OPAC, (size_t)p.n * 4);
        if (!ft || !fo) return BH_ERR_OOM;
        BH_TRY(launch_fold_min_scale(ctx, st->transforms, st->raw_opacities, st->min_scale, p.n, ft, fo));
        w.r_transforms = ft;
        w.r_raw_opac = fo;
    }
    return 0;
}

int step_forward(bh_ctx* ctx, const StepArgs& a, const StepPlan& p, StepWork& w) {
    const BhTrainBatch* batch = a.batch;
    ForwardRequest fwd;
    fwd.cam = batch->camera;
    fwd.n = p.n; fwd.sh_degree = a.st->sh_degree;
    fwd.flags = BH_FLAG_BWD_INFO | (a.cfg->render_mip ? BH_FLAG_MIP : 0) | (a.cfg->exact_lists ? 0 : BH_FLAG_SLICED_LISTS);
    fwd.transforms = w.r_transforms; fwd.sh_coeffs = a.st->sh_coeffs; fwd.raw_opacities = w.r_raw_opac;
    fwd.bg[0] = batch->background[0]; fwd.bg[1] = batch->background[1]; fwd.bg[2] = batch->background[2];
    fwd.view_id = batch->view_id;
    fwd.visible = w.visible();
    fwd.visible_floats = p.o_tr;
    fwd.max_radius = w.s_radius;
    fwd.grad_begin = w.exch + p.o_tr;
    fwd.grad_floats = p.exch_count - p.o_tr;
    if (p.masked_grads) {
        fwd.grad_begin = w.exch + p.o_ref;
        fwd.grad_floats = p.exch_count - p.o_ref;
    }
    fwd.defer_decision = !p.tile_mode;
    BH_TRY(render_forward(ctx, fwd, &w.ro));
    if (p.tile_mode) {
        ProfScope ps(ctx, "ImageExchange");
        const uint32_t r0 = p.tile_y0 * TILE_WIDTH, r1 = p.tile_y1 * TILE_WIDTH < p.H ? p.tile_y1 * TILE_WIDTH : p.H;
        if (p.native_tiles) BH_TRY(comm_exchange_strip_halos(ctx, w.ro.out_img, p.H, p.W, r0, r1));
        else if (batch->image_hook(batch->image_hook_user, w.ro.out_img, p.H, p.W, r0, r1) != 0) return set_error(ctx, BH_ERR_STATE, "image hook failed");
    }
    return 0;
}

int queue_loss(bh_ctx* ctx, const StepArgs& a, const StepPlan& p, const StepWork& w, const LossCall& l) {
    const BhTrainBatch* batch = a.batch;
    uint32_t* started_host = nullptr;
    uint32_t started_tag = 0u;
    if (ctx->far_job.pending && !ctx->far_job.gate_event_recorded && !ctx->gate_signal_queued) {
        started_host = ctx->host_counters + HOST_GATE_TAG_WORD;
        started_tag = ctx->far_job.gate_tag;
        ctx->gate_signal_queued = true;
    }
    if (p.tile_mode && batch->strip_loss) {
        return launch_image_loss_fused_window(ctx, w.ro.out_img, batch->gt_packed, p.H, p.W, l.lc, l.alpha_match, l.dl_rgb, l.dl_alpha, p.tile_y0, p.tile_y1,
                                              w.loss_dev, w.v_output, w.loss_host, started_host, started_tag);
    }
    if (p.envmap) {
        ProfScope ps(ctx, "EnvMap");
        BH_TRY(launch_envmap_composite(ctx, p.envmap, batch->camera, w.ro.out_img, p.H, p.W, w.composited));
    }
    if (p.exposure) {
        ProfScope ps(ctx, "Exposure");
        BH_TRY(launch_exposure_apply(ctx, p.exposure, batch->view_id, w.frame(), p.H, p.W, w.corrected));
    }
    if (p.bilagrid) {
        ProfScope ps(ctx, "Bilagrid");
        BH_TRY(launch_bilagrid_slice(ctx, p.bilagrid, batch->view_id, w.frame(), p.H, p.W, w.corrected));
    }
    return launch_image_loss_fused(ctx, w.corrected ? w.corrected : w.frame(), batch->gt_packed, p.H, p.W, l.lc, l.alpha_match, l.dl_rgb, l.dl_alpha, w.loss_dev, w.v_output,
                                   w.loss_host, started_host, started_tag);
}

int step_image_loss(bh_ctx* ctx, const StepArgs& a, const StepPlan& p, StepWork& w) {
    const BhTrainConfig* cfg = a.cfg;
    const BhTrainBatch* batch = a.batch;
    const bool ssim_on = cfg->ssim_weight > 0.0f;
    LossCall l;
    BhLossConfig& lc = l.lc;
    lc.l1_weight = ssim_on ? 1.0f - cfg->ssim_weight : 1.0f;
    lc.ssim_weight = ssim_on ? -cfg->ssim_weight : 0.0f;
    const bool bg_nonzero = batch->background[0] != 0.0f || batch->background[1] != 0.0f || batch->background[2] != 0.0f;
    lc.composite_bg = (batch->has_alpha && bg_nonzero) ? 1 : 0;
    lc.bg[0] = batch->background[0]; lc.bg[1] = batch->background[1]; lc.bg[2] = batch->background[2];
    lc.mask = batch->alpha_is_mask ? 1 : 0;
    l.alpha_match = batch->has_alpha && !batch->alpha_is_mask && cfg->match_alpha_weight > 0.0f;
    const size_t hw = (size_t)p.W * p.H;
    w.v_output = (float*)ensure(ctx, SLOT_V_OUTPUT, hw * 16);
    w.loss_dev = (float*)ensure(ctx, SLOT_LOSS_SCALAR, 16);
    if (!w.v_output || !w.loss_dev) return BH_ERR_OOM;
    if (p.envmap && !(w.composited = (float*)ensure(ctx, SLOT_ENVMAP_FRAME, hw * 16))) return BH_ERR_OOM;
    if ((p.exposure || p.bilagrid) && !(w.corrected = (float*)ensure(ctx, SLOT_CORRECTED, hw * 16))) return BH_ERR_OOM;
    w.loss_host = reinterpret_cast<float*>(ctx->host_counters) + HOST_LOSS_WORD;
    l.dl_rgb = 1.0f / (float)(hw * 3);
    l.dl_alpha = l.alpha_match ? cfg->match_alpha_weight / (float)hw : 0.0f;
#ifdef BH_TEST_HOOKS
    if (ctx->knob_fail_loss_at && ++ctx->train_steps_seen == ctx->knob_fail_loss_at)
        return set_error(ctx, BH_ERR_OOM, "train_step: injected failure between the forward and the loss (BH_TEST_FAIL_LOSS_AT)");
#endif
    if (far_job_decides_first(ctx)) {
        BH_TRY(finish_far_slice(ctx, nullptr));
        w.ro = ctx->latest.out;
    }
    BH_TRY(queue_loss(ctx, a, p, w, l));
    if (ctx->far_job.pending) {
        bool far_ran = false;
        BH_TRY(finish_far_slice(ctx, &far_ran));
        if (far_ran) {
            w.ro = ctx->latest.out;
            BH_TRY(queue_loss(ctx, a, p, w, l));
        }
    }
    float* const final_img = w.corrected ? w.corrected : w.frame();
    if (p.lpips) BH_TRY(lpips_train_term(ctx, final_img, batch->gt_packed, p.H, p.W, lc.composite_bg ? lc.bg : nullptr, w.v_output, w.loss_dev, w.loss_host));
    if (p.exposure) {
        ProfScope ps(ctx, "Exposure");
        BH_TRY(launch_exposure_backward(ctx, p.exposure, batch->view_id, w.frame(), w.v_output, p.H, p.W, w.v_output, true));
    }
    if (p.bilagrid) {
        ProfScope ps(ctx, "Bilagrid");
        const float tvw = ctx->terms.bilagrid_tv_weight;
        if (tvw != 0.0f) {
            float* tv_value = bilagrid_tv_scratch(ctx);
            if (!tv_value) return BH_ERR_OOM;
// ... 260 lines not shown
```

brush_amd/csrc/upload.hip:

```cpp
#include <cstring>
#include <mutex>
#include <new>
#include <vector>

#include "context.h"

namespace bh {

constexpr int UP_WG = 256;

__global__ __launch_bounds__(UP_WG) void pack_rgb8_kernel(const uint32_t* __restrict__ rgb, uint64_t pixels, uint32_t* __restrict__ out) {
    const uint64_t q = (uint64_t)blockIdx.x * UP_WG + threadIdx.x;
    const uint64_t p0 = q * 4;
    if (p0 >= pixels) return;
    if (p0 + 4 <= pixels) {
        const uint32_t a = rgb[q * 3], b = rgb[q * 3 + 1], c = rgb[q * 3 + 2];
        uint4 o;
        o.x = (a & 0x00FFFFFFu) | 0xFF000000u;
        o.y = (a >> 24) | ((b & 0x0000FFFFu) << 8) | 0xFF000000u;
        o.z = (b >> 16) | ((c & 0x000000FFu) << 16) | 0xFF000000u;
        o.w = (c >> 8) | 0xFF000000u;
        *reinterpret_cast<uint4*>(out + p0) = o;
    } else {
        const uint8_t* bytes = reinterpret_cast<const uint8_t*>(rgb);
        for (uint64_t p = p0; p < pixels; ++p)
            out[p] = (uint32_t)bytes[p * 3] | ((uint32_t)bytes[p * 3 + 1] << 8) | ((uint32_t)bytes[p * 3 + 2] << 16) | 0xFF000000u;
    }
}

__global__ __launch_bounds__(UP_WG) void pack_rgba8_kernel(const uint32_t* __restrict__ rgba, uint64_t pixels, int premultiply,
                                                          uint32_t* __restrict__ out) {
    const uint64_t p = (uint64_t)blockIdx.x * UP_WG + threadIdx.x;
    if (p >= pixels) return;
    const uint32_t v = rgba[p];
    if (!premultiply) { out[p] = v; return; }
    const uint32_t a = v >> 24;
    const uint32_t r = ((v & 0xFFu) * a + 127u) / 255u;
    const uint32_t g = (((v >> 8) & 0xFFu) * a + 127u) / 255u;
    const uint32_t b = (((v >> 16) & 0xFFu) * a + 127u) / 255u;
    out[p] = r | (g << 8) | (b << 16) | (a << 24);
}

static hipError_t enqueue_pack(hipStream_t st, const uint8_t* raw, uint64_t pixels, uint32_t channels, int premultiply, uint32_t* out) {
    if (channels == 3) {
        const uint64_t groups = (pixels + 3) / 4;
        hipLaunchKernelGGL(pack_rgb8_kernel, dim3((unsigned)((groups + UP_WG - 1) / UP_WG)), dim3(UP_WG), 0, st, (const uint32_t*)raw, pixels, out);
    } else {
        hipLaunchKernelGGL(pack_rgba8_kernel, dim3((unsigned)((pixels + UP_WG - 1) / UP_WG)), dim3(UP_WG), 0, st, (const uint32_t*)raw, pixels,
                           premultiply, out);
    }
    return hipGetLastError();
}

}

struct bh_uploader {
    bh_ctx* ctx = nullptr;
    hipStream_t copy_stream = nullptr;
    uint64_t max_pixels = 0;
    struct Slot {
        uint8_t* pinned = nullptr;
        uint8_t* raw_dev = nullptr;
        uint32_t* packed = nullptr;
        hipEvent_t ready = nullptr;
        hipEvent_t consumed = nullptr;
        uint32_t w = 0, h = 0, channels = 0;
        int state = 0;
        bool consumed_pending = false;
        void* tab_pinned = nullptr;
        size_t tab_cap = 0;
    };
    std::vector<Slot> slots;
    uint8_t* view_scratch = nullptr;
    size_t view_scratch_cap = 0;
    uint32_t next = 0;
    std::mutex mu;
    std::string last_error;
};

using namespace bh;

static int up_fail(bh_uploader* up, int code, const char* msg) {
    if (up) up->last_error = msg;
    return code;
}

extern "C" {

bh_uploader* bh_uploader_create(bh_ctx* ctx, uint64_t max_pixels, uint32_t num_slots) {
    if (!ctx || max_pixels == 0 || num_slots < 2 || num_slots > 16) return nullptr;
    if (hipSetDevice(ctx->device) != hipSuccess) { (void)hipGetLastError(); return nullptr; }
    bh_uploader* up = new (std::nothrow) bh_uploader();
    if (!up) return nullptr;
    up->ctx = ctx;
    up->max_pixels = max_pixels;
    bool ok = hipStreamCreateWithFlags(&up->copy_stream, hipStreamNonBlocking) == hipSuccess;
    up->slots.resize(num_slots);
    const size_t bytes = (size_t)max_pixels * 4 + 16;
    for (auto& s : up->slots) {
        ok = ok && hipHostMalloc((void**)&s.pinned, bytes, hipHostMallocDefault) == hipSuccess;
        ok = ok && hipMalloc((void**)&s.raw_dev, bytes) == hipSuccess;
        ok = ok && hipMalloc((void**)&s.packed, (size_t)max_pixels * 4) == hipSuccess;
        ok = ok && hipEventCreateWithFlags(&s.ready, hipEventDisableTiming) == hipSuccess;
        ok = ok && hipEventCreateWithFlags(&s.consumed, hipEventDisableTiming) == hipSuccess;
    }
    if (!ok) {
        (void)hipGetLastError();
        bh_uploader_destroy(up);
        return nullptr;
    }
    return up;
}

void bh_uploader_destroy(bh_uploader* up) {
    if (!up) return;
    (void)hipSetDevice(up->ctx->device);
    if (up->copy_stream) (void)hipStreamSynchronize(up->copy_stream);
    for (auto& s : up->slots) {
        if (s.consumed_pending && s.consumed) (void)hipEventSynchronize(s.consumed);
        if (s.pinned) (void)hipHostFree(s.pinned);
        if (s.raw_dev) (void)hipFree(s.raw_dev);
        if (s.packed) (void)hipFree(s.packed);
        if (s.ready) (void)hipEventDestroy(s.ready);
        if (s.consumed) (void)hipEventDestroy(s.consumed);
        if (s.tab_pinned) (void)hipHostFree(s.tab_pinned);
    }
    if (up->view_scratch) (void)hipFree(up->view_scratch);
    if (up->copy_stream) (void)hipStreamDestroy(up->copy_stream);
    delete up;
}

const char* bh_uploader_last_error(bh_uploader* up) { return up ? up->last_error.c_str() : "null uploader"; }

int bh_uploader_begin(bh_uploader* up, uint64_t bytes, void** pinned) {
    if (!up || !pinned) return BH_ERR_INVALID_ARG;
    std::lock_guard<std::mutex> lk(up->mu);
    if (bytes > up->max_pixels * 4) return up_fail(up, BH_ERR_INVALID_ARG, "uploader_begin: image larger than the slot size");
    const uint32_t idx = up->next;
    bh_uploader::Slot& s = up->slots[idx];
    if (s.state == 1 || s.state == 3) return up_fail(up, BH_ERR_STATE, "uploader_begin: the next slot is still mapped or acquired (release it first)");
    if (s.state == 2) return up_fail(up, BH_ERR_STATE, "uploader_begin: ring full — the oldest batch was never acquired");
    if (hipSetDevice(up->ctx->device) != hipSuccess) { (void)hipGetLastError(); return up_fail(up, BH_ERR_HIP, "hipSetDevice"); }
    if (s.consumed_pending) {
        if (hipEventSynchronize(s.consumed) != hipSuccess) { (void)hipGetLastError(); return up_fail(up, BH_ERR_HIP, "hipEventSynchronize(consumed)"); }
        s.consumed_pending = false;
    }
    s.state = 1;
    up->next = (idx + 1) % (uint32_t)up->slots.size();
    *pinned = s.pinned;
    return (int)idx;
}

int bh_uploader_commit(bh_uploader* up, int slot, uint32_t w, uint32_t h, uint32_t channels, int premultiply) {
    if (!up || slot < 0 || slot >= (int)up->slots.size()) return BH_ERR_INVALID_ARG;
    std::lock_guard<std::mutex> lk(up->mu);
    bh_uploader::Slot& s = up->slots[slot];
    if (s.state != 1) return up_fail(up, BH_ERR_STATE, "uploader_commit: slot was not mapped with uploader_begin");
    const uint64_t pixels = (uint64_t)w * h;
    if (pixels == 0 || pixels > up->max_pixels || (channels != 3 && channels != 4)) {
        s.state = 0;
        return up_fail(up, BH_ERR_INVALID_ARG, "uploader_commit: image must be RGB8 or RGBA8 and fit the slot");
    }
    if (hipSetDevice(up->ctx->device) != hipSuccess) { (void)hipGetLastError(); return up_fail(up, BH_ERR_HIP, "hipSetDevice"); }
    const size_t bytes = ((size_t)pixels * channels + 3) & ~(size_t)3;
    hipError_t e = hipMemcpyAsync(s.raw_dev, s.pinned, bytes, hipMemcpyHostToDevice, up->copy_stream);
    if (e == hipSuccess) e = enqueue_pack(up->copy_stream, s.raw_dev, pixels, channels, premultiply, s.packed);
    if (e == hipSuccess) e = hipEventRecord(s.ready, up->copy_stream);
    if (e != hipSuccess) {
        (void)hipGetLastError();
        s.state = 0;
        return up_fail(up, BH_ERR_HIP, hipGetErrorString(e));
    }
    s.w = w; s.h = h; s.channels = channels;
    s.state = 2;
    return 0;
}

int bh_uploader_commit_view(bh_uploader* up, int slot, const BhViewLoad* d) {
    if (!up || slot < 0 || slot >= (int)up->slots.size() || !d) return BH_ERR_INVALID_ARG;
    const uint32_t w = d->w, h = d->h, ch = d->channels;
    const uint64_t pixels = (uint64_t)w * h, slot_bytes = up->max_pixels * 4;
    const bool has_mask = d->mask_w != 0 || d->mask_h != 0;
    const uint64_t mask_bytes = (uint64_t)d->mask_w * d->mask_h;
    uint32_t nw = 0, nh = 0;
    const int size_rc = bh_view_output_size(w, h, d->max_resolution, d->scale, &nw, &nh);
    const bool resize = size_rc == 0 && (nw != w || nh != h);
    const bool mask_resize = has_mask && (d->mask_w != w || d->mask_h != h);
    ResizeTable tabs[4];
    if (size_rc == 0 && pixels != 0 && pixels <= up->max_pixels && mask_bytes <= slot_bytes && (!has_mask || mask_bytes != 0)) {
        try {
            if (mask_resize) {
                tabs[0] = resize_table(d->mask_h, h, BH_FILTER_TRIANGLE);
                tabs[1] = resize_table(d->mask_w, w, BH_FILTER_TRIANGLE);
            }
            if (resize) {
                tabs[2] = resize_table(h, nh, BH_FILTER_LANCZOS3);
                tabs[3] = resize_table(w, nw, BH_FILTER_LANCZOS3);
            }
        } catch (const std::bad_alloc&) {
            for (auto& t : tabs) t.reset();
        }
    }

    std::lock_guard<std::mutex> lk(up->mu);
    bh_uploader::Slot& s = up->slots[slot];
    if (s.state != 1) return up_fail(up, BH_ERR_STATE, "uploader_commit_view: slot was not mapped with uploader_begin");
    auto refuse = [&](int code, const char* msg) {
        s.state = 0;
        return up_fail(up, code, msg);
    };
    if (pixels == 0 || pixels > up->max_pixels || (ch != 3 && ch != 4))
        return refuse(BH_ERR_INVALID_ARG, "uploader_commit_view: image must be RGB8 or RGBA8 and fit the slot");
    if (d->reserved != 0) return refuse(BH_ERR_INVALID_ARG, "uploader_commit_view: reserved must be 0");
    uint64_t end = pixels * ch;
    if (has_mask) {
        if (mask_bytes == 0) return refuse(BH_ERR_INVALID_ARG, "uploader_commit_view: a mask needs mask_w and mask_h > 0");
        if (d->mask_offset < end || d->mask_offset > slot_bytes || mask_bytes > slot_bytes - d->mask_offset)
            return refuse(BH_ERR_INVALID_ARG, "uploader_commit_view: the mask must lie behind the image inside the slot's 4 * max_pixels bytes");
        end = d->mask_offset + mask_bytes;
// ... 24 lines not shown
    if (scratch > up->view_scratch_cap) {
        e = hipStreamSynchronize(up->copy_stream);
        if (e == hipSuccess && up->view_scratch) e = hipFree(up->view_scratch);
        up->view_scratch = nullptr;
        up->view_scratch_cap = 0;
        const size_t cap = a256(scratch + scratch / 4);
        if (e == hipSuccess) e = hipMalloc((void**)&up->view_scratch, cap);
        if (e != hipSuccess) return fail_hip(e);
        up->view_scratch_cap = cap;
    }
    if (tab > s.tab_cap) {
        if (s.tab_pinned) e = hipHostFree(s.tab_pinned);
        s.tab_pinned = nullptr;
        s.tab_cap = 0;
        if (e == hipSuccess) e = hipHostMalloc(&s.tab_pinned, tab, hipHostMallocDefault);
        if (e != hipSuccess) return fail_hip(e);
        s.tab_cap = tab;
    }
    uint8_t* ht = (uint8_t*)s.tab_pinned;
    for (const ResizeTable& t : tabs) {
        if (!t) continue;
        std::memcpy(ht, t->data(), t->size());
        ht += t->size();
    }
    uint8_t* sc = up->view_scratch;
    const int32_t* dt = (const int32_t*)sc;
    float* tmp = (float*)(sc + off_tmp);
    const hipStream_t st = up->copy_stream;

    e = hipMemcpyAsync(s.raw_dev, s.pinned, (size_t)((end + 3) & ~(uint64_t)3), hipMemcpyHostToDevice, st);
    if (e == hipSuccess && tab) e = hipMemcpyAsync(sc, s.tab_pinned, tab, hipMemcpyHostToDevice, st);
    const uint8_t* mask = s.raw_dev + d->mask_offset;
    if (e == hipSuccess && mask_resize) {
        uint8_t* mdst = sc + off_mask;
        e = enqueue_resize(st, mask, d->mask_w, d->mask_h, 1, w, h, dt, (const int32_t*)((const uint8_t*)dt + tmv), tmp, mdst, RESIZE_OUT_U8);
        mask = mdst;
    }
    const int32_t* vt = (const int32_t*)((const uint8_t*)dt + tmv + tmh);
    const int32_t* hz = (const int32_t*)((const uint8_t*)dt + tmv + tmh + tv);
    const int mode = (cm == 4 && premul) ? RESIZE_OUT_PACKED_PREMUL : RESIZE_OUT_PACKED;
    if (e == hipSuccess) {
        if (has_mask && resize) {
            uint32_t* merged = (uint32_t*)(sc + off_merged);
            e = enqueue_mask_merge(st, s.raw_dev, ch, mask, pixels, d->invert_mask ? 1 : 0, 0, merged);
            if (e == hipSuccess) e = enqueue_resize(st, (const uint8_t*)merged, w, h, 4, nw, nh, vt, hz, tmp, s.packed, mode);
        } else if (has_mask) {
            e = enqueue_mask_merge(st, s.raw_dev, ch, mask, pixels, d->invert_mask ? 1 : 0, premul, s.packed);
        } else if (resize) {
            e = enqueue_resize(st, s.raw_dev, w, h, ch, nw, nh, vt, hz, tmp, s.packed, mode);
        } else {
            e = enqueue_pack(st, s.raw_dev, pixels, ch, premul, s.packed);
        }
    }
    if (e == hipSuccess) e = hipEventRecord(s.ready, st);
    if (e != hipSuccess) return fail_hip(e);
    s.w = nw; s.h = nh; s.channels = cm;
    s.state = 2;
    return 0;
}

int bh_uploader_submit(bh_uploader* up, const uint8_t* pixels, uint32_t w, uint32_t h, uint32_t channels, int premultiply) {
    if (!up || !pixels) return BH_ERR_INVALID_ARG;
    void* dst = nullptr;
    const uint64_t bytes = (uint64_t)w * h * channels;
    const int slot = bh_uploader_begin(up, bytes, &dst);
    if (slot < 0) return slot;
    std::memcpy(dst, pixels, (size_t)bytes);
    const int rc = bh_uploader_commit(up, slot, w, h, channels, premultiply);
    return rc < 0 ? rc : slot;
}

int bh_uploader_acquire(bh_uploader* up, int slot, const uint32_t** packed, uint32_t* w, uint32_t* h, int* has_alpha) {
    if (!up || slot < 0 || slot >= (int)up->slots.size() || !packed) return BH_ERR_INVALID_ARG;
    std::lock_guard<std::mutex> lk(up->mu);
    bh_uploader::Slot& s = up->slots[slot];
    if (s.state != 2) return up_fail(up, BH_ERR_STATE, "uploader_acquire: slot holds no committed image");
    if (hipSetDevice(up->ctx->device) != hipSuccess) { (void)hipGetLastError(); return up_fail(up, BH_ERR_HIP, "hipSetDevice"); }
    if (hipStreamWaitEvent(up->ctx->stream, s.ready, 0) != hipSuccess) { (void)hipGetLastError(); return up_fail(up, BH_ERR_HIP, "hipStreamWaitEvent"); }
    s.state = 3;
    *packed = s.packed;
    if (w) *w = s.w;
    if (h) *h = s.h;
    if (has_alpha) *has_alpha = s.channels == 4;
    return 0;
}

int bh_uploader_release(bh_uploader* up, int slot) {
    if (!up || slot < 0 || slot >= (int)up->slots.size()) return BH_ERR_INVALID_ARG;
    std::lock_guard<std::mutex> lk(up->mu);
    bh_uploader::Slot& s = up->slots[slot];
    if (s.state != 3) return up_fail(up, BH_ERR_STATE, "uploader_release: slot was not acquired");
    if (hipSetDevice(up->ctx->device) != hipSuccess) { (void)hipGetLastError(); return up_fail(up, BH_ERR_HIP, "hipSetDevice"); }
    if (hipEventRecord(s.consumed, up->ctx->stream) != hipSuccess) { (void)hipGetLastError(); return up_fail(up, BH_ERR_HIP, "hipEventRecord"); }
    s.consumed_pending = true;
    s.state = 0;
    return 0;
}

}
```

brush_amd/host.py:

```python
import ctypes as C
import enum
import math
import os
from contextlib import contextmanager
from dataclasses import dataclass, field
from typing import Optional, Tuple

import torch

from . import _ffi
from ._ffi import BrushHipError
from .parallel import (DIRECT_ALLREDUCE_MIN_FLOATS, allreduce_direct, allreduce_exchange, allreduce_refine_maxima, allgather_strips, exchange_strip_halos, strip_spans_px,
                       strips_allow_halo_loss, tile_rows_for_rank)


_LEGACY_ENV_OPTIONS = (
    ("BH_NO_LPT", "no_lpt", "1"), ("BH_GENERIC_DEPTH_SORT", "generic_depth_sort", "1"), ("BH_FORCE_PG", "force_exchange", "1"),
    ("BH_TRAIN_ZERO_GRADS", "zero_grads", "1"), ("BH_CUT_MIN_PAIRS", "cut_min_pairs", None), ("BH_CUT_SORT_ALL", "cut_sort_all", "1"),
    ("BH_NO_VIEW_HASH", "no_view_hash", "1"), ("BH_CUT_MARGIN_FIXED", "cut_margin_fixed", "1"), ("BH_CUT_CTRL", "cut_ctrl", None),
    ("BH_READBACK_COPY", "readback_copy", "1"), ("BH_EVENT_WAITS", "event_waits", "1"), ("BH_K16_ORDER", "k16_order", None),
    ("BH_CUT_MARGIN_PCT", "cut_margin_pct", None), ("BH_UPDATE_NO_DORMANT", "no_dormant", "1"),
    ("BH_K5_EXACT_SPW", "k5_exact_spw", None), ("BH_TILE_SORT_LSD", "tile_sort", "lsd"), ("BH_LOSS_BANDS", "loss_bands", None),
    ("BH_UPDATE_ROWS", "update_rows", None), ("BH_SORT_KPT", "sort_kpt", None),
)
# ... 1260 lines not shown
    if k.dim() != 1 or v.shape != k.shape:
        raise BrushHipError("tile_sort_offsets: tile ids and splat ids must be 1-D and of the same length")
    ok, ov = torch.empty_like(k), torch.empty_like(k)
    offs = torch.empty((int(num_tiles), 2), dtype=torch.int32, device=dev)
    ctx.check(ctx.lib.bh_tile_sort_offsets(ctx._h, _ptr(k), _ptr(v), k.numel(), int(num_tiles), _ptr(ok), _ptr(ov), _ptr(offs)))
    return ok, ov, offs


def prefix_sum(x, ctx: Optional[Context] = None):
    dev = x.device if isinstance(x, torch.Tensor) and x.is_cuda else torch.device("cuda", torch.cuda.current_device())
    ctx = ctx or get_context(dev)
    a = _as_u32(x, dev)
    o = torch.empty_like(a)
    ctx.check(ctx.lib.bh_prefix_sum(ctx._h, _ptr(a), a.numel(), _ptr(o)))
    return o


def _loss_cfg(l1_weight, ssim_weight, composite_bg, mask):
    cfg = _ffi.BhLossConfig()
    cfg.l1_weight, cfg.ssim_weight = float(l1_weight), float(ssim_weight)
    bg = composite_bg if composite_bg is not None else (0.0, 0.0, 0.0)
    cfg.bg[0], cfg.bg[1], cfg.bg[2] = [float(b) for b in bg]
    cfg.composite_bg = 1 if composite_bg is not None else 0
    cfg.mask = 1 if mask else 0
    return cfg


def image_loss(pred_hwc, gt_packed, l1_weight=0.8, ssim_weight=-0.2, composite_bg=None, mask=False, ctx: Optional[Context] = None):
    dev = pred_hwc.device
    ctx = ctx or get_context(dev)
    h, w, c = pred_hwc.shape
    pred_chw = pred_hwc.permute(2, 0, 1).contiguous().float()
    gt = _as_u32(gt_packed, dev).reshape(h, w)
    out = torch.empty_like(pred_chw)
    cfg = _loss_cfg(l1_weight, ssim_weight, composite_bg, mask)
    ctx.check(ctx.lib.bh_image_loss_forward(ctx._h, _ptr(pred_chw), _ptr(gt), c, h, w, C.byref(cfg), _ptr(out)))
    return out.permute(1, 2, 0).contiguous()


def image_loss_backward(pred_hwc, gt_packed, dl_dmap_hwc, l1_weight=0.8, ssim_weight=-0.2, composite_bg=None, mask=False,
                        ctx: Optional[Context] = None):
    dev = pred_hwc.device
    ctx = ctx or get_context(dev)
    h, w, c = pred_hwc.shape
    pred_chw = pred_hwc.permute(2, 0, 1).contiguous().float()
    dl = dl_dmap_hwc.permute(2, 0, 1).contiguous().float()
    gt = _as_u32(gt_packed, dev).reshape(h, w)
    out = torch.empty_like(pred_chw)
    cfg = _loss_cfg(l1_weight, ssim_weight, composite_bg, mask)
    ctx.check(ctx.lib.bh_image_loss_backward(ctx._h, _ptr(pred_chw), _ptr(gt), _ptr(dl), c, h, w, C.byref(cfg), _ptr(out)))
    return out.permute(1, 2, 0).contiguous()


def image_loss_value_and_grad(img_hwc4, gt_packed, l1_weight=0.8, ssim_weight=-0.2, composite_bg=None, mask=False,
                              alpha_weight=0.0, ctx: Optional[Context] = None):
    dev = img_hwc4.device
    ctx = ctx or get_context(dev)
    h, w, c = img_hwc4.shape
    if c != 4:
        raise ValueError("img must be [H,W,4]")
    img = img_hwc4.contiguous().float()
    gt = _as_u32(gt_packed, dev).reshape(h, w)
    loss = torch.empty(1, dtype=torch.float32, device=dev)
    v_out = torch.empty_like(img)
    cfg = _loss_cfg(l1_weight, ssim_weight, composite_bg, mask)
    ctx.check(ctx.lib.bh_image_loss_value_and_grad(ctx._h, _ptr(img), _ptr(gt), h, w, C.byref(cfg), float(alpha_weight), _ptr(loss), _ptr(v_out)))
    return loss, v_out


def gather_stats(refine_weight_norm, vis_weight, max_screen_size, refine_weight, visible, screen_radius, ctx: Optional[Context] = None):
    ctx = ctx or get_context(refine_weight.device)
    n = refine_weight.numel()
    ctx.check(ctx.lib.bh_gather_stats(ctx._h, _ptr(refine_weight_norm), _ptr(vis_weight), _ptr(max_screen_size), _ptr(refine_weight), _ptr(visible),
                                      _ptr(screen_radius), n))


def adam_step(param, grad, m1, m2, lr, t, col_scale=None, reduce_m2=False, beta1=0.9, beta2=0.999, eps=1e-15, ctx: Optional[Context] = None):
    ctx = ctx or get_context(param.device)
    rows = param.shape[0]
    row_len = param.numel() // rows if rows else 1
    ctx.check(ctx.lib.bh_adam_step(ctx._h, _ptr(param), _ptr(grad), _ptr(m1), _ptr(m2), rows, row_len,
                                   _ptr(col_scale) if col_scale is not None else None, float(lr), int(t), int(bool(reduce_m2)),
                                   float(beta1), float(beta2), float(eps)))


@dataclass
class TrainConfig:
    total_train_iters: int = 30000
    lr_mean: float = 2e-5
    lr_mean_end: float = 2e-7
    lr_coeffs_dc: float = 2e-3
    lr_coeffs_sh_scale: float = 10.0
    lr_opac: float = 0.012
    lr_scale: float = 5e-3
    lr_rotation: float = 2e-3
    ssim_weight: float = 0.2
    match_alpha_weight: float = 0.1
    mean_noise_weight: float = 50.0
    background_color: Tuple[float, float, float] = (0.0, 0.0, 0.0)
    background_noise_strength: float = 0.1
    render_mip: bool = False
    exact_lists: bool = False
    max_splats: int = 10_000_000
    refine_every: int = 200
    growth_grad_threshold: float = 0.0025
    growth_select_fraction: float = 0.25
    growth_stop_iter: int = 15000
    split_at_screen_size: float = 0.5
    opac_decay: float = 0.004
    lpips_loss_weight: float = 0.0
    depth_loss_weight: float = 0.0
    depth_loss_weight_end: Optional[float] = None
    depth_loss_kind: str = "l1"
    normal_loss_weight: float = 0.0
    normal_loss_from_iter: int = 0
    distortion_loss_weight: float = 0.0
    distortion_loss_from_iter: int = 0
    distortion_kind: str = "z"
# ... 146 lines not shown
        self.ctx.check(self.ctx.lib.bh_tsdf_integrate(self.ctx._h, C.byref(g), n, cams, dptr, iptr, C.byref(cfg)))

    def count(self):
        g = self.grid()
        nv, nt = C.c_uint32(), C.c_uint32()
        self.ctx.check(self.ctx.lib.bh_tsdf_extract_count(self.ctx._h, C.byref(g), C.byref(nv), C.byref(nt)))
        return int(nv.value), int(nt.value)

    def extract_mesh(self):
        n_v, n_t = self.count()
        dev = self.device
        vertices = torch.empty((n_v, 3), dtype=torch.float32, device=dev)
        colours = torch.empty((n_v, 3), dtype=torch.float32, device=dev) if self.rgb is not None else None
        triangles = torch.empty((n_t, 3), dtype=torch.int32, device=dev)
        g = self.grid()
        nv, nt = C.c_uint32(), C.c_uint32()
        self.ctx.check(self.ctx.lib.bh_tsdf_extract(self.ctx._h, C.byref(g), _ptr(vertices), _ptr(colours) if colours is not None else None, _ptr(triangles),
                                                    n_v, n_t, C.byref(nv), C.byref(nt)))
        return vertices, colours, triangles

    def to_ply(self) -> bytes:
        vertices, colours, triangles = self.extract_mesh()
        return mesh_to_ply(vertices, triangles, colours, ctx=self.ctx)


def fuse_views(splats: "Splats", cameras, img_size, volume: TsdfVolume, depth_mode="expected", pass_: "RasterPass" = None, depth_min=0.0,
               depth_max=math.inf, alpha_min=0.5):
    pass_ = RasterPass.Backward if pass_ is None else pass_
    ctx = volume.ctx
    w, h = int(img_size[0]), int(img_size[1])
    cameras = list(cameras)
    for first in range(0, len(cameras), _ffi.TSDF_MAX_BATCH):
        cams, depths, images = [], [], []
        for camera in cameras[first:first + _ffi.TSDF_MAX_BATCH]:
            node = render_splats_diff(splats, camera, (w, h), (0.0, 0.0, 0.0), pass_, ctx=ctx)
            depths.append(node.depth(depth_mode))
            images.append(node.img.clone())
            cams.append(camera if isinstance(camera, _ffi.BhCamera) else camera.uniforms((w, h)))
        volume.integrate(depths, cams, images, depth_min=depth_min, depth_max=depth_max, alpha_min=alpha_min)
    return volume


@dataclass
class SceneBatch:
    img_packed: torch.Tensor
    camera: Camera
    has_alpha: bool = False
    alpha_is_mask: bool = False
    view_id: int = 0
    depth: Optional[torch.Tensor] = None
    depth_scale: float = 1.0
    depth_offset: float = 0.0
    features: Optional[torch.Tensor] = None

    def img_size(self):
        return tuple(self.img_packed.shape)


@dataclass
class TrainStepStats:
    num_visible: int
    num_intersections: int
    lr_mean: float
    loss: float
    exchange_rows: int = 0


def view_output_size(w: int, h: int, max_resolution: int = 1920, scale: float = 1.0):
    lib = _ffi.load()
    ow, oh = C.c_uint32(), C.c_uint32()
    rc = lib.bh_view_output_size(int(w), int(h), int(max_resolution or 0), float(scale), C.byref(ow), C.byref(oh))
    if rc < 0:
        raise ValueError("view_output_size: w, h > 0 and a finite scale > 0")
    return int(ow.value), int(oh.value)


_FILTERS = {"lanczos3": _ffi.FILTER_LANCZOS3, "triangle": _ffi.FILTER_TRIANGLE}


def resize_image(t, size, filter="lanczos3", ctx: Optional[Context] = None):
    if filter not in _FILTERS:
        raise ValueError("filter must be 'lanczos3' or 'triangle'")
    if t.dtype != torch.uint8 or t.dim() not in (2, 3) or (t.dim() == 3 and t.shape[2] not in (1, 3, 4)):
        raise ValueError("resize_image: a uint8 [H,W] or [H,W,1|3|4] tensor")
    if t.device.type != "cuda":
        raise ValueError("resize_image: the image must be on the device")
    ctx = ctx or get_context(t.device)
    nw, nh = int(size[0]), int(size[1])
    c = 1 if t.dim() == 2 else int(t.shape[2])
    src = t.contiguous()
    out = torch.empty((nh, nw) + tuple(t.shape[2:]), dtype=torch.uint8, device=t.device)
    ctx.check(ctx.lib.bh_resize_u8(ctx._h, _ptr(src), int(t.shape[1]), int(t.shape[0]), c, _ptr(out), nw, nh, _FILTERS[filter]))
    return out


class BatchUploader:

    def __init__(self, max_pixels, slots=3, ctx: Optional[Context] = None):
        self.ctx = ctx or get_context()
        self.lib = self.ctx.lib
        self._h = C.c_void_p(self.lib.bh_uploader_create(self.ctx._h, int(max_pixels), int(slots)))
        if not self._h:
            raise BrushHipError("bh_uploader_create failed (max_pixels > 0, 2 <= slots <= 16, enough pinned memory)")
        self.max_pixels, self.slots = int(max_pixels), int(slots)

    def close(self):
        if getattr(self, "_h", None):
            self.lib.bh_uploader_destroy(self._h)
            self._h = None

    def __del__(self):
        try:
            self.close()
        except Exception:
            pass

    def _check(self, rc):
        if rc < 0:
            raise BrushHipError("uploader error %d: %s" % (rc, self.lib.bh_uploader_last_error(self._h).decode()))
        return rc

    def map(self, nbytes):
        import numpy as np
        p = C.c_void_p()
        slot = self._check(self.lib.bh_uploader_begin(self._h, int(nbytes), C.byref(p)))
        buf = (C.c_uint8 * int(nbytes)).from_address(p.value)
        return slot, np.frombuffer(buf, dtype=np.uint8)

    def commit(self, slot, w, h, channels, premultiply):
        self._check(self.lib.bh_uploader_commit(self._h, int(slot), int(w), int(h), int(channels), int(bool(premultiply))))

    def submit(self, img_u8, premultiply=True):
        import numpy as np
        a = np.ascontiguousarray(img_u8, dtype=np.uint8)
        if a.ndim != 3 or a.shape[2] not in (3, 4):
            raise ValueError("image must be [H,W,3] or [H,W,4] uint8")
        h, w, c = a.shape
        return self._check(self.lib.bh_uploader_submit(self._h, a.ctypes.data_as(C.c_void_p), w, h, c, int(bool(premultiply) and c == 4)))

    def submit_view(self, img_u8, mask=None, invert_mask=False, max_resolution=1920, scale=1.0, premultiply=None):
        import numpy as np
        a = np.ascontiguousarray(img_u8, dtype=np.uint8)
        if a.ndim != 3 or a.shape[2] not in (3, 4):
            raise ValueError("image must be [H,W,3] or [H,W,4] uint8")
        h, w, c = a.shape
        m = None
        if mask is not None:
            m = np.ascontiguousarray(mask, dtype=np.uint8)
            if m.ndim == 3 and m.shape[2] == 1:
                m = m[:, :, 0]
            if m.ndim != 2 or m.size == 0:
                raise ValueError("mask must be a one-channel uint8 [h,w] array")
        if premultiply is None:
            premultiply = m is None
        img_bytes = a.size
        total = img_bytes + (m.size if m is not None else 0)
        slot, buf = self.map(total)
        try:
            buf[:img_bytes] = a.reshape(-1)
            if m is not None:
                buf[img_bytes:total] = m.reshape(-1)
        except Exception:
            self.lib.bh_uploader_commit_view(self._h, int(slot), C.byref(_ffi.BhViewLoad()))
            raise
        d = _ffi.BhViewLoad(w=w, h=h, channels=c, mask_w=m.shape[1] if m is not None else 0, mask_h=m.shape[0] if m is not None else 0,
                            invert_mask=int(bool(invert_mask)), mask_offset=img_bytes if m is not None else 0,
                            max_resolution=int(max_resolution or 0), scale=float(scale), premultiply=int(bool(premultiply)))
        self._check(self.lib.bh_uploader_commit_view(self._h, int(slot), C.byref(d)))
        return slot

    def acquire(self, slot):
        p, w, h, ha = C.c_void_p(), C.c_uint32(), C.c_uint32(), C.c_int()
        self._check(self.lib.bh_uploader_acquire(self._h, int(slot), C.byref(p), C.byref(w), C.byref(h), C.byref(ha)))
        return _view(p.value, (int(h.value), int(w.value)), torch.int32, self.ctx.device), bool(ha.value)

    def release(self, slot):
        self._check(self.lib.bh_uploader_release(self._h, int(slot)))


class SceneLoader:

    def __init__(self, views, seed=0, uploader: Optional[BatchUploader] = None, slots=3, rank=0, world=1, ctx: Optional[Context] = None,
                 max_resolution: Optional[int] = None, image_scale: float = 1.0, invert_masks: bool = False):
        import queue
        import threading
        self.views = [v for i, v in enumerate(views) if i % world == rank]
        self.view_ids = [i + 1 for i in range(len(views)) if i % world == rank]
        if not self.views:
            raise ValueError("Need at least one view in dataset")
        self.max_resolution, self.image_scale, self.invert_masks = max_resolution, float(image_scale), bool(invert_masks)
        if not (self.image_scale > 0.0 and math.isfinite(self.image_scale)):
            raise ValueError("image_scale must be finite and > 0")
        self._own_uploader = uploader is None
        if uploader is None:
            mp = 0
            for v in self.views:
                img = v[0]() if callable(v[0]) else v[0]
                mask = self._view_mask(v)
                px = img.shape[0] * img.shape[1]
                staged = img.size + (mask.size if mask is not None else 0)
                mp = max(mp, px, (staged + 3) // 4)
            uploader = BatchUploader(mp, slots, ctx)
        self.up = uploader
        self._seed = int(seed) & 0xFFFFFFFFFFFFFFFF
        self._q = queue.Queue(maxsize=max(1, self.up.slots - 1))
        self._stop = threading.Event()
        self._held = None
        self._thread = threading.Thread(target=self._run, name="brush-hip-loader", daemon=True)
        self._thread.start()

    @staticmethod
    def _view_mask(view):
        m = view[3] if len(view) > 3 else None
        return m() if callable(m) else m

    @staticmethod
    def _splitmix(state):
        state = (state + 0x9E3779B97F4A7C15) & 0xFFFFFFFFFFFFFFFF
        z = state
        z = ((z ^ (z >> 30)) * 0xBF58476D1CE4E5B9) & 0xFFFFFFFFFFFFFFFF
        z = ((z ^ (z >> 27)) * 0x94D049BB133111EB) & 0xFFFFFFFFFFFFFFFF
        return state, z ^ (z >> 31)

    def epoch_order(self, epoch):
        n = len(self.views)
        order = list(range(n))
        st = (self._seed ^ (0xD1B54A32D192ED03 * (epoch + 1))) & 0xFFFFFFFFFFFFFFFF
        for i in range(n - 1, 0, -1):
            st, r = self._splitmix(st)
            j = r % (i + 1)
            order[i], order[j] = order[j], order[i]
        return order

    def _run(self):
        import queue
        epoch = 0
        try:
            while not self._stop.is_set():
                for idx in self.epoch_order(epoch):
                    view = self.views[idx]
                    img = view[0]() if callable(view[0]) else view[0]
                    mask_img = self._view_mask(view)
                    flag = view[2] if len(view) > 2 else None
                    mask = bool(flag) if flag is not None else mask_img is not None
                    while not self._stop.is_set() and self._q.full():
                        self._stop.wait(0.0005)
                    if self._stop.is_set():
                        return
                    if mask_img is None and self.max_resolution is None and self.image_scale == 1.0:
                        slot = self.up.submit(img, premultiply=not mask)
                    else:
                        slot = self.up.submit_view(img, mask=mask_img, invert_mask=self.invert_masks, max_resolution=self.max_resolution or 0,
                                                   scale=self.image_scale, premultiply=not mask)
                    self._q.put((slot, idx, view[1], mask))
                epoch += 1
        except Exception as e:
            try:
                self._q.put(e, timeout=1.0)
            except queue.Full:
                pass

    def next_batch(self):
        if self._held is not None:
            self.up.release(self._held)
            self._held = None
        item = self._q.get()
        if isinstance(item, Exception):
            raise BrushHipError("Scene loader failed to load an image: %r" % (item,))
        slot, idx, cam, mask = item
        packed, has_alpha = self.up.acquire(slot)
        self._held = slot
        b = SceneBatch(packed, cam, has_alpha=has_alpha, alpha_is_mask=mask, view_id=self.view_ids[idx])
        b.view_index = idx
        return b

    def close(self):
        self._stop.set()
        try:
            while True:
                self._q.get_nowait()
        except Exception:
            pass
        self._thread.join(timeout=5.0)
        if self._own_uploader:
            self.up.close()


class SplatTrainer:

    def __init__(self, config: TrainConfig, median_scene_scale: float = 1.0, process_group=None, ctx: Optional[Context] = None,
                 partition: str = "cameras", native_comm: bool = False, sparse_exchange: bool = True, seed: Optional[int] = None,
                 allreduce: str = "ring", lpips: Optional["Lpips"] = None, pose_optimizer: Optional["PoseOptimizer"] = None,
                 exposure: Optional["ExposureTable"] = None, exposure_lr=None, bilagrid: Optional["BilateralGridTable"] = None, bilagrid_lr=None,
                 bilagrid_tv_weight: float = 10.0, envmap: Optional["EnvironmentMap"] = None, envmap_lr=None,
                 feature_field: Optional["FeatureField"] = None):
        if partition not in ("cameras", "tiles"):
            raise ValueError("partition must be 'cameras' or 'tiles'")
        if pose_optimizer is not None and partition == "tiles":
            raise ValueError("pose_optimizer is not available with partition 'tiles'")
        if exposure is not None and partition == "tiles":
            raise ValueError("exposure is not available with partition 'tiles'")
        if feature_field is not None and partition == "tiles":
            raise ValueError("feature_field is not available with partition 'tiles'")
        if feature_field is not None and pose_optimizer is not None:
            raise ValueError("feature_field and pose_optimizer cannot be combined (the pose pass does not carry the feature term's gradient)")
        if envmap is not None and partition == "tiles":
            raise ValueError("envmap is not available with partition 'tiles'")
        if envmap is not None and any(float(b) != 0.0 for b in config.background_color):
            raise ValueError("envmap needs background_color (0, 0, 0): the map is what lies behind the splats")
        if envmap is not None and pose_optimizer is not None:
            raise ValueError("envmap and pose_optimizer cannot be combined (the pose pass does not carry the lookup's dependence on the rotation)")
        self.envmap, self.envmap_lr = envmap, envmap_lr
        self.feature_field = feature_field
        self.pose_optimizer = pose_optimizer
        self._pose_buf = None
        self.exposure, self.exposure_lr = exposure, exposure_lr
        if bilagrid is not None and partition == "tiles":
            raise ValueError("bilagrid is not available with partition 'tiles'")
        if bilagrid is not None and exposure is not None:
            raise ValueError("bilagrid and exposure are alternatives: pass one of them")
        self.bilagrid, self.bilagrid_lr, self.bilagrid_tv_weight = bilagrid, bilagrid_lr, float(bilagrid_tv_weight)
        if allreduce not in ("ring", "direct"):
            raise ValueError("allreduce must be 'ring' (all_reduce / ncclAllReduce) or 'direct' (reduce-scatter + all-gather over point-to-point messages)")
        self.allreduce = allreduce
        if native_comm and process_group is not None:
            raise ValueError("native_comm excludes process_group")
# ... 147 lines not shown
        c, ff, ftarget = self.config, self.feature_field, batch.features
        fw = float(c.feature_loss_weight) if ftarget is not None else 0.0
        if ff is None:
            if fw > 0.0:
                raise ValueError("feature_loss_weight > 0 and a batch with a feature target need SplatTrainer(..., feature_field=FeatureField(...))")
            return None, None
        if not (fw > 0.0 and self.step_count + 1 >= int(c.feature_loss_from_iter)):
            return None, None
        fk = c.feature_loss_kind
        fk = int(FEATURE_LOSS_KINDS[fk]) if isinstance(fk, str) else int(fk)
        ch = int(ff.features.shape[1])
        if fk == _ffi.FEATURE_LOSS_CROSS_ENTROPY:
            ftgt = torch.as_tensor(ftarget, dtype=torch.uint8, device=dev).contiguous()
            if ftgt.dim() != 2:
                raise ValueError("SceneBatch.features: cross-entropy labels must be uint8 [H, W]")
        else:
            ftgt = _f32c(ftarget, dev)
            if ftgt.dim() != 3 or int(ftgt.shape[2]) != ch:
                raise ValueError("SceneBatch.features: an l1 target must be float32 [H, W, %d]" % ch)
        if ftgt is not ftarget and not ctx.uses_torch_stream:
            torch.cuda.current_stream(dev).synchronize()
        ft = _ffi.BhFeatureTarget()
        ft.target, ft.h, ft.w, ft.channels, ft.kind, ft.weight = ftgt.data_ptr(), int(ftgt.shape[0]), int(ftgt.shape[1]), ch, fk, fw
        return ft, ftgt

    def _step_terms(self, ctx, batch, b, dev):
        c, lib, step = self.config, ctx.lib, self.step_count + 1
        lw = float(c.lpips_loss_weight)
        if lw > 0.0 and self.lpips is None:
            raise ValueError("lpips_loss_weight > 0 needs SplatTrainer(..., lpips=Lpips.from_state_dict(...))")
        ff = self.feature_field
        ft, ftgt = self._feature_target(ctx, batch, dev)
        off = (None,)
        terms = []
        dgt = None
        if batch.depth is not None:
            dt, dgt = _depth_target(batch.depth, dev, c.depth_loss_kind, c.depth_weight_at(step), batch.depth_scale, batch.depth_offset, shape=batch.img_size())
            terms.append((lib.bh_train_set_depth, (C.byref(dt),), off))
        else:
            terms.append((lib.bh_train_set_depth, off, off))
        nw = float(c.normal_loss_weight)
        if nw > 0.0 and step >= int(c.normal_loss_from_iter):
            terms.append((lib.bh_train_set_normal, (C.byref(_ffi.BhNormalTermConfig(weight=nw)),), off))
        else:
            terms.append((lib.bh_train_set_normal, off, off))
        xw = float(c.distortion_loss_weight)
        if xw > 0.0 and step >= int(c.distortion_loss_from_iter):
            xt = _ffi.BhDistortionTermConfig(weight=xw, kind=_distortion_kind(c.distortion_kind), near_z=float(c.distortion_near), far_z=float(c.distortion_far))
            terms.append((lib.bh_train_set_distortion, (C.byref(xt),), off))
        else:
            terms.append((lib.bh_train_set_distortion, off, off))
        if ff is not None:
            terms.append((lib.bh_train_set_features, (C.byref(ff.as_struct()), C.byref(ft)) if ft is not None else (None, None), (None, None)))
        if self.batch_patch is not None:
            terms.append(lambda: self.batch_patch(b))
        terms.append((lib.bh_train_set_lpips, (self.lpips._h if lw > 0.0 else None, lw if lw > 0.0 else 0.0), None))
        if self.pose_optimizer is not None:
            terms.append((lib.bh_train_set_pose_grad, (_ptr(self._pose_buf),), off))
        ex, grid = self.exposure, self.bilagrid
        if ex is not None:
            if self.exposure_lr is not None:
                terms.append(lambda: ex.set_lr(self.exposure_lr(step)))
            terms.append((lib.bh_train_set_exposure, (ex._h,), off))
        if grid is not None:
            if self.bilagrid_lr is not None:
                terms.append(lambda: grid.set_lr(self.bilagrid_lr(step)))
            terms.append((lib.bh_train_set_bilagrid, (grid._h, self.bilagrid_tv_weight), (None, 0.0)))
        env = self.envmap
        if env is not None:
            if self.envmap_lr is not None:
                terms.append(lambda: env.set_lr(self.envmap_lr(step)))
            terms.append((lib.bh_train_set_envmap, (env._h,), off))
        return terms, (dgt, ftgt), ft

    @staticmethod
    @contextmanager
    def _attached(ctx, terms):
        try:
            for t in terms:
                if callable(t):
                    t()
                else:
                    ctx.check(t[0](ctx._h, *t[1]))
            yield
        finally:
            for t in terms:
                if not callable(t) and t[2] is not None:
                    t[0](ctx._h, *t[2])

    def step(self, batch: SceneBatch, splats: Splats, background=None, noise_samples=None) -> Tuple[Splats, TrainStepStats]:
        ctx = self.ctx or get_context(splats.device)
        dev = splats.device
        if self.state is None:
            self._init_state(splats)
        cfg, st = self._train_config(splats), self._train_state(splats, self.state)
        st.min_scale = splats.min_scale.data_ptr() if splats.min_scale is not None else None
        h, w = batch.img_size()
        b = _ffi.BhTrainBatch()
        b.camera = batch.camera if isinstance(batch.camera, _ffi.BhCamera) else batch.camera.uniforms((w, h))
        tiles = self._tile_window(ctx, b, h, dev)
        gt = _as_u32(batch.img_packed, dev)
        b.gt_packed = gt.data_ptr()
        b.has_alpha, b.alpha_is_mask = int(batch.has_alpha), int(batch.alpha_is_mask)
        jitter = self.seed is not None and self.envmap is None
        bg = background if background is not None else (self.sample_background() if jitter else self.config.background_color)
        b.background[0], b.background[1], b.background[2] = [float(v) for v in bg]
        ns = None
        if noise_samples is not None:
            ns = _f32c(noise_samples, dev).reshape(-1, 3)
            b.noise_samples = ns.data_ptr()
        elif self.seed is not None:
            b.device_noise, b.noise_seed = 1, self.seed
        stats = _ffi.BhTrainStats()
        b.exchange_mode = 1 if (self.sparse_exchange and (self.pg is not None or self.native_comm)) else 0
        b.view_id = int(batch.view_id) & 0xFFFFFFFF
        po = self.pose_optimizer
        if po is not None:
            b.camera = po.camera(b.view_id, b.camera)
            if self._pose_buf is None:
                self._pose_buf = torch.zeros((12,), dtype=torch.float32, device=dev)
                if not ctx.uses_torch_stream:
                    torch.cuda.current_stream(dev).synchronize()
        hook, scale = None, 1.0
        if self.native_comm:
            scale = 1.0 if tiles else 1.0 / ctx.comm_world()
        if self.pg is not None:
# ... 759 lines not shown
```

include/brush_hip.hpp:

```cpp
#pragma once
#include <hip/hip_runtime_api.h>

#include <algorithm>
#include <array>
#include <cmath>
#include <cstddef>
#include <cstdint>
#include <cstring>
#include <functional>
#include <numeric>
#include <optional>
#include <stdexcept>
#include <string>
#include <utility>
#include <vector>

#include "brush_hip.h"
#include "brush_hip_lpips.h"
#include "brush_hip_compressed_ply.h"
#include "brush_hip_image.h"
#include "brush_hip_depth.h"
#include "brush_hip_pose.h"
#include "brush_hip_exposure.h"
#include "brush_hip_depth_loss.h"
#include "brush_hip_normal.h"
#include "brush_hip_normal_loss.h"
#include "brush_hip_distortion.h"
#include "brush_hip_bilagrid.h"
#include "brush_hip_mesh.h"
#include "brush_hip_features.h"
#include "brush_hip_feature_train.h"
#include "brush_hip_scene.h"
#include "brush_hip_lift.h"
#include "brush_hip_envmap.h"

namespace brush_hip {

struct Error : std::runtime_error {
    int code;
    Error(int c, const std::string& m) : std::runtime_error("brush_hip error " + std::to_string(c) + ": " + m), code(c) {}
};

inline void hip_check(hipError_t e, const char* what) {
    if (e != hipSuccess) throw Error(BH_ERR_HIP, std::string(what) + ": " + hipGetErrorString(e));
}

template <class T>
class DeviceBuffer {
  public:
    DeviceBuffer() = default;
    explicit DeviceBuffer(size_t n) { resize(n); }
    explicit DeviceBuffer(const std::vector<T>& host) { upload(host); }
    DeviceBuffer(const DeviceBuffer&) = delete;
    DeviceBuffer& operator=(const DeviceBuffer&) = delete;
    DeviceBuffer(DeviceBuffer&& o) noexcept : p_(o.p_), n_(o.n_) { o.p_ = nullptr; o.n_ = 0; }
    DeviceBuffer& operator=(DeviceBuffer&& o) noexcept {
        if (this != &o) { release(); p_ = o.p_; n_ = o.n_; o.p_ = nullptr; o.n_ = 0; }
        return *this;
    }
    ~DeviceBuffer() { release(); }
    void resize(size_t n) {
        release();
        if (n) hip_check(hipMalloc((void**)&p_, n * sizeof(T)), "hipMalloc");
        n_ = n;
    }
    void upload(const std::vector<T>& host) {
        if (host.size() != n_) resize(host.size());
        if (n_) hip_check(hipMemcpy(p_, host.data(), n_ * sizeof(T), hipMemcpyHostToDevice), "hipMemcpy H2D");
    }
    std::vector<T> download() const {
        std::vector<T> out(n_);
        if (n_) hip_check(hipMemcpy(out.data(), p_, n_ * sizeof(T), hipMemcpyDeviceToHost), "hipMemcpy D2H");
        return out;
    }
    void zero() { if (n_) hip_check(hipMemset(p_, 0, n_ * sizeof(T)), "hipMemset"); }
    T* data() { return p_; }
    const T* data() const { return p_; }
    size_t size() const { return n_; }

  private:
    void release() { if (p_) (void)hipFree(p_); p_ = nullptr; n_ = 0; }
    T* p_ = nullptr;
    size_t n_ = 0;
};

template <class T>
std::vector<T> download(const T* dev, size_t n) {
// ... 1390 lines not shown
inline BhDepthTarget depth_target(const float* gt, uint32_t h, uint32_t w, uint32_t kind = BH_DEPTH_LOSS_L1, float weight = 1.0f, float scale = 1.0f,
                                  float offset = 0.0f) {
    static_assert(BH_DEPTH_LOSS_L1 == 0u && BH_DEPTH_LOSS_DISPARITY == 1u, "depth loss kinds");
    BhDepthTarget t{};
    t.gt = gt; t.h = h; t.w = w; t.kind = kind; t.weight = weight; t.scale = scale; t.offset = offset;
    return t;
}
inline void depth_loss_value_and_grad(const Context& ctx, const float* depth, const BhDepthTarget& target, float* loss, float* v_depth) {
    ctx.check(bh_depth_loss_value_and_grad(ctx.get(), depth, &target, loss, v_depth));
}
inline void eval_depth_metrics(const Context& ctx, const float* depth, const BhDepthTarget& target, float* metrics) {
    ctx.check(bh_eval_depth_metrics(ctx.get(), depth, &target, metrics));
}
inline void train_set_depth(const Context& ctx, const BhDepthTarget* target) { ctx.check(bh_train_set_depth(ctx.get(), target)); }

inline BhFeatureTarget feature_target(const void* target, uint32_t h, uint32_t w, uint32_t channels, uint32_t kind = BH_FEATURE_LOSS_L1, float weight = 1.0f) {
    static_assert(BH_FEATURE_LOSS_L1 == 0u && BH_FEATURE_LOSS_CROSS_ENTROPY == 1u && BH_FEATURE_MAX_CHANNELS == 256u, "feature loss kinds");
    BhFeatureTarget t{};
    t.target = target; t.h = h; t.w = w; t.channels = channels; t.kind = kind; t.weight = weight;
    return t;
}
inline void feature_loss_value_and_grad(const Context& ctx, const float* map, const BhFeatureTarget& target, float* loss, float* v_map) {
    ctx.check(bh_feature_loss_value_and_grad(ctx.get(), map, &target, loss, v_map));
}

inline DeviceBuffer<float> splat_normals(const Context& ctx, const Splats& splats, const Camera& camera) {
    static_assert(BH_NORMAL_ACCUMULATED == 0u && BH_NORMAL_UNIT == 1u, "normal modes");
    const BhCamera cam = camera.uniforms(16, 16);
    const detail::Folded f = detail::fold(ctx, splats);
    DeviceBuffer<float> out;
    out.resize((size_t)splats.num_splats() * 3);
    ctx.check(bh_splat_normals(ctx.get(), &cam, f.t, splats.num_splats(), out.data()));
    ctx.sync();
    return out;
}
inline DeviceBuffer<float> depth_to_normal(const Context& ctx, const Camera& camera, const float* depth, uint32_t h, uint32_t w) {
    const BhCamera cam = camera.uniforms(w, h);
    DeviceBuffer<float> out;
    out.resize((size_t)h * w * 3);
    ctx.check(bh_depth_to_normal(ctx.get(), &cam, depth, h, w, out.data()));
    ctx.sync();
    return out;
}
inline DeviceBuffer<float> depth_to_normal_backward(const Context& ctx, const Camera& camera, const float* depth, const float* v_normal, uint32_t h,
                                                    uint32_t w) {
    const BhCamera cam = camera.uniforms(w, h);
    DeviceBuffer<float> out;
    out.resize((size_t)h * w);
    ctx.check(bh_depth_to_normal_backward(ctx.get(), &cam, depth, v_normal, h, w, out.data()));
    ctx.sync();
    return out;
}

inline void normal_consistency_value_and_grad(const Context& ctx, const Camera& camera, const float* normal, const float* depth, const float* image,
                                              uint32_t h, uint32_t w, float weight, bool accumulate_v_depth, float* loss, float* v_normal, float* v_depth) {
    static_assert(sizeof(BhNormalTermConfig) == 16, "BhNormalTermConfig layout");
    const BhCamera cam = camera.uniforms(w, h);
    ctx.check(bh_normal_consistency_value_and_grad(ctx.get(), &cam, normal, depth, image, h, w, weight, accumulate_v_depth ? 1u : 0u, loss, v_normal, v_depth));
}
inline void train_set_normal(const Context& ctx, const BhNormalTermConfig* cfg) { ctx.check(bh_train_set_normal(ctx.get(), cfg)); }
inline void train_set_normal(const Context& ctx, float weight) {
    BhNormalTermConfig cfg{};
    cfg.weight = weight;
    train_set_normal(ctx, &cfg);
}

inline void distortion_loss(const Context& ctx, const float* map, uint32_t h, uint32_t w, uint32_t channels, float weight, float* loss) {
    ctx.check(bh_distortion_loss(ctx.get(), map, h, w, channels, weight, loss));
}
inline void train_set_distortion(const Context& ctx, const BhDistortionTermConfig* cfg) {
    static_assert(sizeof(BhDistortionTermConfig) == 16, "BhDistortionTermConfig layout");
    ctx.check(bh_train_set_distortion(ctx.get(), cfg));
}
inline void train_set_distortion(const Context& ctx, float weight, uint32_t kind = BH_DISTORTION_Z, float near_z = 0.2f, float far_z = 1000.0f) {
    BhDistortionTermConfig cfg{};
    cfg.weight = weight;
    cfg.kind = kind;
    cfg.near_z = near_z;
    cfg.far_z = far_z;
    train_set_distortion(ctx, &cfg);
}

inline uint64_t knn_log_scales(const Context& ctx, Splats& splats, DeviceBuffer<float>* nn_dist = nullptr) {
    const uint32_t n = splats.num_splats();
    if (nn_dist) nn_dist->resize((size_t)n * 2);
    uint64_t pairs = 0;
    ctx.check(bh_knn_log_scales(ctx.get(), splats.transforms.data(), n, nn_dist ? nn_dist->data() : nullptr, &pairs));
    return pairs;
}
inline Splats to_init_splats(const Context& ctx, const std::vector<float>& means, const std::vector<float>& rotations = {},
                             const std::vector<float>& log_scales = {}, const std::vector<float>& sh_coeffs = {},
                             const std::vector<float>& raw_opacities = {}, bool render_mip = false) {
    const size_t n = means.size() / 3;
    if (means.size() != n * 3 || (!rotations.empty() && rotations.size() != n * 4) || (!log_scales.empty() && log_scales.size() != n * 3) ||
        (!raw_opacities.empty() && raw_opacities.size() != n) || (!sh_coeffs.empty() && (n == 0 || sh_coeffs.size() % (3 * n) != 0)))
        throw Error(BH_ERR_INVALID_ARG, "to_init_splats: means [N,3], rotations [N,4], log_scales [N,3], sh_coeffs [N,C,3], raw_opacities [N]");
    std::vector<float> tr(n * 10);
    for (size_t i = 0; i < n; ++i) {
        for (int k = 0; k < 3; ++k) tr[i * 10 + k] = means[i * 3 + k];
        for (int k = 0; k < 4; ++k) tr[i * 10 + 3 + k] = rotations.empty() ? (k == 0 ? 1.0f : 0.0f) : rotations[i * 4 + k];
        for (int k = 0; k < 3; ++k) tr[i * 10 + 7 + k] = log_scales.empty() ? 0.0f : log_scales[i * 3 + k];
    }
    Splats s = Splats::from_host(tr, sh_coeffs.empty() ? std::vector<float>(n * 3, 0.5f) : sh_coeffs,
                                 raw_opacities.empty() ? std::vector<float>(n, 0.0f) : raw_opacities, render_mip);
    if (log_scales.empty()) knn_log_scales(ctx, s);
    return s;
// ... 12 lines not shown
```

Before: 1324.

## Precompute blurred GT SSIM moments and blur only prediction moments in fused loss

Adds a kernel that computes the ground truth's two Gaussian-blurred SSIM moments per channel (mean and mean of squares) into planes of shape [3,2,H,W]. These planes are cached per batch keyed on the GT tensor's pointer, shape and version, or produced by the uploader at upload time. A templated variant of the fused loss forward reads them instead of blurring them, so it blurs three moments instead of five and uses a smaller LDS footprint with a higher occupancy hint. The cost is 24 extra bytes per pixel of memory and extra global reads, and the fast path is skipped whenever the GT is composited over a non-zero background.

```diff
diff --git a/brush_amd/__init__.py b/brush_amd/__init__.py
--- a/brush_amd/__init__.py
+++ b/brush_amd/__init__.py
@@ -1,6 +1,6 @@
 from .host import (
     Camera, Context, RasterPass, RenderAux, SplatTrainer, Splats, TrainConfig, SceneBatch,
-    get_context, image_loss, image_loss_backward, image_loss_value_and_grad, prefix_sum, radix_argsort, tile_sort_offsets, render_splats,
+    get_context, image_loss, image_loss_backward, image_loss_value_and_grad, gt_moments, prefix_sum, radix_argsort, tile_sort_offsets, render_splats,
     render_splats_bwd, adam_step, gather_stats, RefineStats, splat_bounds, bounds_median_size, fov_to_focal, focal_to_fov,
     splat_to_ply, load_splat_from_ply, ply_parse_header, ParseMetadata, BatchUploader, SceneLoader, set_list_slicing, last_list_counts, set_view_id,
     render_splats_diff, RenderNode, compute_pup_scores, decimate_to_count, lod_target_count, pup_accumulate, pup_accumulate_view, pup_scores,
diff --git a/brush_amd/_ffi.py b/brush_amd/_ffi.py
--- a/brush_amd/_ffi.py
+++ b/brush_amd/_ffi.py
@@ -429,6 +429,16 @@
     "bh_train_set_envmap": (C.c_int, [C.c_void_p, C.c_void_p]),
 }
 
+GT_MOMENTS_BYTES_PER_PIXEL = 24
+GT_MOMENTS_SYMBOLS = {
+    "bh_gt_moments": (C.c_int, [C.c_void_p, C.c_void_p, C.c_uint32, C.c_uint32, C.c_void_p]),
+    "bh_image_loss_value_and_grad_pre": (C.c_int, [C.c_void_p, C.c_void_p, C.c_void_p, C.c_uint32, C.c_uint32, C.POINTER(BhLossConfig), C.c_float, C.c_void_p,
+                                                   C.c_void_p, C.c_void_p]),
+    "bh_train_set_gt_moments": (C.c_int, [C.c_void_p, C.c_void_p, C.c_uint32, C.c_uint32]),
+    "bh_uploader_enable_gt_moments": (C.c_int, [C.c_void_p, C.c_int]),
+    "bh_uploader_slot_gt_moments": (C.c_int, [C.c_void_p, C.c_int, C.POINTER(C.c_void_p)]),
+}
+
 ABI_VERSION = 7
 STRUCT_MIRRORS = (BhCamera, BhRenderOut, BhLossConfig, BhTrainConfig, BhTrainState, BhTrainBatch, BhTrainStats, BhRefineConfig, BhRefineStats, BhPlyInfo)
 
@@ -464,13 +474,13 @@
 def load():
     global _lib
     if _lib is None:
-        _lib = _bind(LIB_PATH, dict(SYMBOLS, **LPIPS_SYMBOLS, **COMPRESSED_PLY_SYMBOLS, **IMAGE_SYMBOLS, **DEPTH_SYMBOLS, **POSE_SYMBOLS, **EXPOSURE_SYMBOLS, **BILAGRID_SYMBOLS, **DEPTH_LOSS_SYMBOLS, **NORMAL_SYMBOLS, **NORMAL_LOSS_SYMBOLS, **DISTORTION_SYMBOLS, **MESH_SYMBOLS, **FEATURE_SYMBOLS, **FEATURE_TRAIN_SYMBOLS, **SCENE_SYMBOLS, **LIFT_SYMBOLS, **ENVMAP_SYMBOLS))
+        _lib = _bind(LIB_PATH, dict(SYMBOLS, **LPIPS_SYMBOLS, **COMPRESSED_PLY_SYMBOLS, **IMAGE_SYMBOLS, **DEPTH_SYMBOLS, **POSE_SYMBOLS, **EXPOSURE_SYMBOLS, **BILAGRID_SYMBOLS, **DEPTH_LOSS_SYMBOLS, **NORMAL_SYMBOLS, **NORMAL_LOSS_SYMBOLS, **DISTORTION_SYMBOLS, **MESH_SYMBOLS, **FEATURE_SYMBOLS, **FEATURE_TRAIN_SYMBOLS, **SCENE_SYMBOLS, **LIFT_SYMBOLS, **ENVMAP_SYMBOLS, **GT_MOMENTS_SYMBOLS))
     return _lib
 
 
 def load_test_hooks():
     global _lib_th
     if _lib_th is None:
-        _lib_th = _bind(TEST_HOOKS_LIB_PATH, dict(SYMBOLS, **LPIPS_SYMBOLS, **COMPRESSED_PLY_SYMBOLS, **IMAGE_SYMBOLS, **DEPTH_SYMBOLS, **POSE_SYMBOLS, **EXPOSURE_SYMBOLS, **BILAGRID_SYMBOLS, **DEPTH_LOSS_SYMBOLS, **NORMAL_SYMBOLS, **NORMAL_LOSS_SYMBOLS, **DISTORTION_SYMBOLS, **MESH_SYMBOLS, **FEATURE_SYMBOLS, **FEATURE_TRAIN_SYMBOLS, **SCENE_SYMBOLS, **LIFT_SYMBOLS, **ENVMAP_SYMBOLS,
+        _lib_th = _bind(TEST_HOOKS_LIB_PATH, dict(SYMBOLS, **LPIPS_SYMBOLS, **COMPRESSED_PLY_SYMBOLS, **IMAGE_SYMBOLS, **DEPTH_SYMBOLS, **POSE_SYMBOLS, **EXPOSURE_SYMBOLS, **BILAGRID_SYMBOLS, **DEPTH_LOSS_SYMBOLS, **NORMAL_SYMBOLS, **NORMAL_LOSS_SYMBOLS, **DISTORTION_SYMBOLS, **MESH_SYMBOLS, **FEATURE_SYMBOLS, **FEATURE_TRAIN_SYMBOLS, **SCENE_SYMBOLS, **LIFT_SYMBOLS, **ENVMAP_SYMBOLS, **GT_MOMENTS_SYMBOLS,
                                                    **TEST_HOOK_SYMBOLS))
     return _lib_th
diff --git a/brush_amd/csrc/api.hip b/brush_amd/csrc/api.hip
--- a/brush_amd/csrc/api.hip
+++ b/brush_amd/csrc/api.hip
@@ -393,6 +393,8 @@
      [](bh_ctx* c, const char* v) { return parse_flag(v, &c->knob_zero_grads); }},
     {"loss_bands", "0|1: the fused loss's blocks take their tiles by XCD column bands (1) or row-major (0)",
      [](bh_ctx* c, const char* v) { return parse_u32(v, 0, 1, &c->knob_loss_bands); }},
+    {"gt_moments", "0|1: the fused loss takes the GT's two blurred moments from a batch's planes when they are attached (1, default) or blurs all five itself (0)",
+     [](bh_ctx* c, const char* v) { return parse_u32(v, 0, 1, &c->knob_gt_moments); }},
     {"update_rows", "0|64|128|256: splats per block of the update kernel (0 = default)",
      [](bh_ctx* c, const char* v) { uint32_t u = 0; if (!parse_u32(v, 0, 256, &u) || !(u == 0 || u == 64 || u == 128 || u == 256)) return false; c->knob_update_rows = u; return true; }},
     {"no_dormant", "0|1: the update kernel fetches and updates dormant splats like everyone else",
@@ -1249,6 +1251,34 @@
                                    loss_out, v_output);
 }
 
+int bh_gt_moments(bh_ctx* ctx, const uint32_t* gt_packed, uint32_t h, uint32_t w, float* out) {
+    if (!ctx) return BH_ERR_INVALID_ARG;
+    if (!gt_packed || !out || h == 0 || w == 0) return set_error(ctx, BH_ERR_INVALID_ARG, "gt_moments: bad argument");
+    BH_HIP(ctx, hipSetDevice(ctx->device));
+    return launch_gt_moments(ctx, gt_packed, h, w, out);
+}
+
+int bh_image_loss_value_and_grad_pre(bh_ctx* ctx, const float* img_hwc4, const uint32_t* gt_packed, uint32_t h, uint32_t w, const BhLossConfig* cfg,
+                                     float alpha_weight, const float* gt_moments, float* loss_out, float* v_output) {
+    if (!ctx) return BH_ERR_INVALID_ARG;
+    if (!img_hwc4 || !gt_packed || !cfg || !loss_out || !v_output || h == 0 || w == 0)
+        return set_error(ctx, BH_ERR_INVALID_ARG, "image_loss_value_and_grad_pre: bad argument");
+    BH_HIP(ctx, hipSetDevice(ctx->device));
+    const size_t hw = (size_t)h * w;
+    const bool alpha = alpha_weight > 0.0f;
+    return launch_image_loss_fused(ctx, img_hwc4, gt_packed, h, w, *cfg, alpha, 1.0f / (float)(hw * 3), alpha ? alpha_weight / (float)hw : 0.0f,
+                                   loss_out, v_output, nullptr, nullptr, 0, gt_moments);
+}
+
+int bh_train_set_gt_moments(bh_ctx* ctx, const float* planes, uint32_t h, uint32_t w) {
+    if (!ctx) return BH_ERR_INVALID_ARG;
+    if (planes && (h == 0 || w == 0)) return set_error(ctx, BH_ERR_INVALID_ARG, "train_set_gt_moments: planes need the image size they were computed for");
+    ctx->terms.gt_moments = planes;
+    ctx->terms.gt_moments_h = planes ? h : 0u;
+    ctx->terms.gt_moments_w = planes ? w : 0u;
+    return 0;
+}
+
 int bh_adam_step(bh_ctx* ctx, float* param, const float* grad, float* m1, float* m2, uint64_t rows, uint32_t row_len,
                  const float* col_scale, float lr, uint32_t t, int reduce_m2, float beta1, float beta2, float eps) {
     if (!ctx) return BH_ERR_INVALID_ARG;
diff --git a/brush_amd/csrc/context.h b/brush_amd/csrc/context.h
--- a/brush_amd/csrc/context.h
+++ b/brush_amd/csrc/context.h
@@ -19,6 +19,7 @@
 #include "../../include/brush_hip_features.h"
 #include "../../include/brush_hip_feature_train.h"
 #include "../../include/brush_hip_envmap.h"
+#include "../../include/brush_hip_gt_moments.h"
 #include "device_math.h"
 
 namespace bh {
@@ -352,12 +353,15 @@
     bh_bilagrid* bilagrid = nullptr;
     float bilagrid_tv_weight = 0.0f;
     bh_envmap* envmap = nullptr;
+    const float* gt_moments = nullptr;
+    uint32_t gt_moments_h = 0, gt_moments_w = 0;
 
     bool lpips_on() const { return lpips != nullptr && lpips_weight > 0.0f; }
     bool depth_on() const { return depth_attached && depth_target.weight > 0.0f; }
     bool normal_on() const { return normal_attached && normal_term.weight > 0.0f; }
     bool distortion_on() const { return distortion_attached; }
     bool feature_on() const { return feature_attached && feature_target.weight > 0.0f; }
+    bool gt_moments_on() const { return gt_moments != nullptr; }
 };
 
 }
@@ -444,6 +448,7 @@
     bool knob_zero_grads = false;
     uint32_t knob_fail_loss_at = 0;
     uint32_t train_steps_seen = 0;
+    uint32_t knob_gt_moments = 1;
     uint32_t knob_loss_bands = 1;
     uint32_t knob_tile_sort = 0;
     float auto_exact_share = 0.9f;
@@ -645,10 +650,13 @@
                                float* dl_dpred);
 int launch_image_loss_fused(bh_ctx* ctx, const float* img_hwc4, const uint32_t* gt, uint32_t h, uint32_t w, const BhLossConfig& cfg,
                             bool alpha_match, float dl_rgb, float dl_alpha, float* loss_out, float* v_output, float* loss_host = nullptr,
-                            uint32_t* started_host = nullptr, uint32_t started_tag = 0);
+                            uint32_t* started_host = nullptr, uint32_t started_tag = 0, const float* gt_moments = nullptr);
 int launch_image_loss_fused_window(bh_ctx* ctx, const float* img_hwc4, const uint32_t* gt, uint32_t h, uint32_t w, const BhLossConfig& cfg,
                                    bool alpha_match, float dl_rgb, float dl_alpha, uint32_t tile_y0, uint32_t tile_y1, float* loss_out,
-                                   float* v_output, float* loss_host = nullptr, uint32_t* started_host = nullptr, uint32_t started_tag = 0);
+                                   float* v_output, float* loss_host = nullptr, uint32_t* started_host = nullptr, uint32_t started_tag = 0,
+                                   const float* gt_moments = nullptr);
+hipError_t enqueue_gt_moments(hipStream_t st, const uint32_t* gt, uint32_t h, uint32_t w, float* out );
+int launch_gt_moments(bh_ctx* ctx, const uint32_t* gt, uint32_t h, uint32_t w, float* out);
 int launch_adam(bh_ctx* ctx, float* param, const float* grad, float* m1, float* m2, uint64_t rows, uint32_t row_len,
                 const float* col_scale, float lr, uint32_t t, bool reduce_m2, float beta1, float beta2, float eps, float gscale = 1.0f);
 struct NoiseArgs { uint64_t seed; uint32_t step; float scale, clamp_abs; };
diff --git a/brush_amd/csrc/loss_fused.hip b/brush_amd/csrc/loss_fused.hip
--- a/brush_amd/csrc/loss_fused.hip
+++ b/brush_amd/csrc/loss_fused.hip
@@ -65,6 +65,7 @@
     float* loss_host;
     uint32_t* started_host;
     uint32_t started_tag;
+    const float* gt_moments;
     uint32_t gx, gy_blocks, band_w;
 };
 
@@ -85,6 +86,10 @@
 }
 
 BH_DEV float gt_ch(uint32_t val, uint32_t c) { return (float)((val >> (c * 8u)) & 0xffu) * INV_255; }
+BH_DEV float gt_ch_rounded(uint32_t val, uint32_t c) {
+#pragma clang fp contract(off)
+    return (float)((val >> (c * 8u)) & 0xffu) * INV_255;
+}
 
 }
 
@@ -96,15 +101,99 @@
 #define BH_LOSS_H2P 24
 constexpr int HP = BH_LOSS_HP;
 constexpr int H2P = BH_LOSS_H2P;
-}
-
-__global__ __launch_bounds__(256) void loss_fused_forward_kernel(const float* __restrict__ img ,
+constexpr int HP3 = 56;
+constexpr int GP = TW * 2;
+
+enum MomentSet : int {
+    MOM_ALL = 0,
+    MOM_PRED = 1,
+    MOM_GT = 2,
+};
+constexpr int moment_count(int set) { return set == MOM_ALL ? 5 : (set == MOM_PRED ? 3 : 2); }
+
+template <int SET>
+BH_DEV void put_moments(const float2 v, const int k, float (&m)[moment_count(SET)][12]) {
+    if constexpr (SET == MOM_ALL) {
+        m[0][k] = v.x; m[2][k] = v.y;
+        m[1][k] = v.x * v.x; m[3][k] = v.y * v.y; m[4][k] = v.x * v.y;
+    } else if constexpr (SET == MOM_PRED) {
+        m[0][k] = v.x;
+        m[1][k] = v.x * v.x; m[2][k] = v.x * v.y;
+    } else {
+        m[0][k] = v.y;
+        m[1][k] = v.y * v.y;
+    }
+}
+
+template <int SET, typename Px>
+BH_DEV void row_blur_item(const Px px, float* op, const float tap4) {
+    constexpr int NM = moment_count(SET);
+    float m[NM][12];
+#pragma unroll
+    for (int k = 0; k < 12; ++k) put_moments<SET>(px(k), k, m);
+#pragma unroll
+    for (int o = 0; o < 2; ++o) {
+        const int cc = HALO + o;
+        float s[NM];
+#pragma unroll
+        for (int j = 0; j < NM; ++j) s[j] = 0.0f;
+#pragma unroll
+        for (int d = 1; d < 6; ++d) {
+            const float wd = d == 1 ? tap4 : tap(5 - d);
+#pragma unroll
+            for (int j = 0; j < NM; ++j) s[j] += (m[j][cc - d] + m[j][cc + d]) * wd;
+        }
+        const float wc = tap(5);
+#pragma unroll
+        for (int j = 0; j < NM; ++j) s[j] += m[j][cc] * wc;
+#pragma unroll
+        for (int j = 0; j < NM; ++j) op[o * NM + j] = s[j];
+    }
+}
+
+template <int NM>
+BH_DEV void column_load(const float* t, const int pitch, float (&v)[12][NM]) {
+#pragma unroll
+    for (int r = 0; r < 12; ++r) {
+#pragma unroll
+        for (int k = 0; k < NM; ++k) v[r][k] = t[r * pitch + k];
+    }
+}
+template <int NM>
+BH_DEV void column_blur_at(const float (&v)[12][NM], const int o, const float tap4, float (&m)[NM]) {
+#pragma unroll
+    for (int k = 0; k < NM; ++k) m[k] = 0.0f;
+#pragma unroll
+    for (int d = 1; d < 6; ++d) {
+        const float wd = d == 1 ? tap4 : tap(5 - d);
+#pragma unroll
+        for (int k = 0; k < NM; ++k) m[k] += (v[o + 5 - d][k] + v[o + 5 + d][k]) * wd;
+    }
+#pragma unroll
+    for (int k = 0; k < NM; ++k) m[k] += v[o + 5][k] * tap(5);
+}
+
+template <bool GT_PRE> struct PassALds;
+template <> struct alignas(16) PassALds<false> {
+    float2 tile[3][SR * SW];
+    float h[(SR - 1) * HP + TW * 5];
+};
+template <> struct alignas(16) PassALds<true> {
+    float pred[3][SR * SW];
+    uint32_t gt[SR * SW];
+    float h[(SR - 1) * HP3 + TW * 3];
+};
+}
+
+template <bool GT_PRE>
+__global__ __launch_bounds__(256, GT_PRE ? 6 : 1) void loss_fused_forward_kernel(const float* __restrict__ img ,
                                                                 const uint32_t* __restrict__ gt,
                                                                 float* __restrict__ partials ,
                                                                 float* __restrict__ block_sums , uint32_t gy, FusedArgs a) {
-    __shared__ float2 s_tile[3][SR * SW];
-    __shared__ float s_h[(SR - 1) * HP + TW * 5];
-    float* s_red = s_h;
+    constexpr int NM = GT_PRE ? 3 : 5;
+    constexpr int P = GT_PRE ? HP3 : HP;
+    __shared__ PassALds<GT_PRE> s;
+    float* s_red = s.h;
     if (a.started_host && blockIdx.x == 0 && blockIdx.y == 0 && threadIdx.x == 0 && threadIdx.y == 0)
         *reinterpret_cast<volatile uint32_t*>(a.started_host) = a.started_tag;
     uint32_t bx, by, blin;
@@ -133,30 +222,39 @@
         lx3[k][0] = ip[0]; lx3[k][1] = ip[1]; lx3[k][2] = ip[2];
         lval[k] = gt[p];
     }
+    size_t own_p[2];
 #pragma unroll
     for (int o = 0; o < 2; ++o) {
         const int yc = py[o] >= (int)a.h ? (int)a.h - 1 : py[o], xc = pxx >= (int)a.w ? (int)a.w - 1 : pxx;
-        own_val[o] = gt[(size_t)yc * a.w + (size_t)xc];
+        own_p[o] = (size_t)yc * a.w + (size_t)xc;
+        own_val[o] = gt[own_p[o]];
     }
 #pragma unroll
     for (int k = 0; k < TILE_LOADS; ++k) {
         const int i = rank + 256 * k;
         if (i < SR * SW) {
-            float g0 = 0.f, g1 = 0.f, g2 = 0.f;
             if (!lin[k]) lx3[k][0] = lx3[k][1] = lx3[k][2] = 0.0f;
-            if (lin[k]) {
-                const uint32_t val = lval[k];
-                const float ga = gt_ch(val, 3);
-                g0 = gt_ch(val, 0); g1 = gt_ch(val, 1); g2 = gt_ch(val, 2);
-                if (a.composite) {
-                    g0 = g0 + (1.0f - ga) * a.bg[0];
-                    g1 = g1 + (1.0f - ga) * a.bg[1];
-                    g2 = g2 + (1.0f - ga) * a.bg[2];
+            if constexpr (GT_PRE) {
+                s.pred[0][i] = lx3[k][0];
+                s.pred[1][i] = lx3[k][1];
+                s.pred[2][i] = lx3[k][2];
+                s.gt[i] = lin[k] ? lval[k] : 0u;
+            } else {
+                float g0 = 0.f, g1 = 0.f, g2 = 0.f;
+                if (lin[k]) {
+                    const uint32_t val = lval[k];
+                    const float ga = gt_ch(val, 3);
+                    g0 = gt_ch(val, 0); g1 = gt_ch(val, 1); g2 = gt_ch(val, 2);
+                    if (a.composite) {
+                        g0 = g0 + (1.0f - ga) * a.bg[0];
+                        g1 = g1 + (1.0f - ga) * a.bg[1];
+                        g2 = g2 + (1.0f - ga) * a.bg[2];
+                    }
                 }
-            }
-            s_tile[0][i] = make_float2(lx3[k][0], g0);
-            s_tile[1][i] = make_float2(lx3[k][1], g1);
-            s_tile[2][i] = make_float2(lx3[k][2], g2);
+                s.tile[0][i] = make_float2(lx3[k][0], g0);
+                s.tile[1][i] = make_float2(lx3[k][1], g1);
+                s.tile[2][i] = make_float2(lx3[k][2], g2);
+            }
         }
     }
     float ga[2] = {0.f, 0.f}, chain[2] = {0.f, 0.f};
@@ -171,66 +269,43 @@
     const float tap4 = in_vgpr(tap(4)), l1_w = in_vgpr(a.l1_w), ssim_w = in_vgpr(a.ssim_w);
 #pragma unroll 1
     for (int c = 0; c < 3; ++c) {
+        float gm[2][2] = {{0.f, 0.f}, {0.f, 0.f}};
+        if constexpr (GT_PRE) {
+#pragma unroll
+            for (int o = 0; o < 2; ++o) {
+                const float* q = a.gt_moments + (size_t)(c * 2) * plane + own_p[o];
+                gm[o][0] = q[0];
+                gm[o][1] = q[plane];
+            }
+        }
         __syncthreads();
         const int probe_rows = SR * (TW / 2);
         for (int i = rank; i < probe_rows; i += 256) {
             const int r = i / (TW / 2), pair = i - r * (TW / 2);
-            const float2* row = &s_tile[c][r * SW + 2 * pair];
-            float x[12], y[12], xx[12], yy[12], xy[12];
-#pragma unroll
-            for (int k = 0; k < 12; ++k) {
-                const float2 v = row[k];
-                x[k] = v.x; y[k] = v.y;
-                xx[k] = v.x * v.x; yy[k] = v.y * v.y; xy[k] = v.x * v.y;
-            }
-#pragma unroll
-            for (int o = 0; o < 2; ++o) {
-                const int cc = HALO + o;
-                float sx = 0, sx2 = 0, sy = 0, sy2 = 0, sxy = 0;
-#pragma unroll
-                for (int d = 1; d < 6; ++d) {
-                    const float wd = d == 1 ? tap4 : tap(5 - d);
-                    sx += (x[cc - d] + x[cc + d]) * wd;
-                    sx2 += (xx[cc - d] + xx[cc + d]) * wd;
-                    sy += (y[cc - d] + y[cc + d]) * wd;
-                    sy2 += (yy[cc - d] + yy[cc + d]) * wd;
-                    sxy += (xy[cc - d] + xy[cc + d]) * wd;
-                }
-                const float wc = tap(5);
-                sx += x[cc] * wc;
-                sx2 += xx[cc] * wc;
-                sy += y[cc] * wc;
-                sy2 += yy[cc] * wc;
-                sxy += xy[cc] * wc;
-                float* op = &s_h[r * HP + (2 * pair + o) * 5];
-                op[0] = sx; op[1] = sx2; op[2] = sy; op[3] = sy2; op[4] = sxy;
-            }
-        }
-        __syncthreads();
-        float v[12][5];
-#pragma unroll
-        for (int r = 0; r < 12; ++r) {
-            const float* t = &s_h[(2 * ly + r) * HP + lx * 5];
-#pragma unroll
-            for (int k = 0; k < 5; ++k) v[r][k] = t[k];
-        }
+            float* op = &s.h[r * P + (2 * pair) * NM];
+            if constexpr (GT_PRE) {
+                const float* prow = &s.pred[c][r * SW + 2 * pair];
+                const uint32_t* grow = &s.gt[r * SW + 2 * pair];
+                row_blur_item<MOM_PRED>([&](const int k) { return make_float2(prow[k], gt_ch_rounded(grow[k], (uint32_t)c)); }, op, tap4);
+            } else {
+                const float2* row = &s.tile[c][r * SW + 2 * pair];
+                row_blur_item<MOM_ALL>([&](const int k) { return row[k]; }, op, tap4);
+            }
+        }
+        __syncthreads();
+        float v[12][NM];
+        column_load<NM>(&s.h[(2 * ly) * P + lx * NM], P, v);
 #pragma unroll
         for (int o = 0; o < 2; ++o) {
-            float m[5] = {0.f, 0.f, 0.f, 0.f, 0.f};
-#pragma unroll
-            for (int d = 1; d < 6; ++d) {
-                const float wd = d == 1 ? tap4 : tap(5 - d);
-#pragma unroll
-                for (int k = 0; k < 5; ++k) m[k] += (v[o + 5 - d][k] + v[o + 5 + d][k]) * wd;
-            }
-#pragma unroll
-            for (int k = 0; k < 5; ++k) m[k] += v[o + 5][k] * tap(5);
+            float m[NM];
+            column_blur_at<NM>(v, o, tap4, m);
             if (!inside[o]) continue;
-            const float mu1 = m[0], mu2 = m[2];
+            const float mu1 = m[0], ex2 = m[1];
+            const float mu2 = GT_PRE ? gm[o][0] : m[NM - 3], ey2 = GT_PRE ? gm[o][1] : m[NM - 2], exy = m[NM - 1];
             const float mu1_sq = mu1 * mu1, mu2_sq = mu2 * mu2;
-            const float s1 = __builtin_fmaxf(0.0f, m[1] - mu1_sq), s2 = __builtin_fmaxf(0.0f, m[3] - mu2_sq);
-            const float s12 = m[4] - mu1 * mu2;
-            const float A = mu1_sq + mu2_sq + SSIM_C1;
+            const float s1 = __builtin_fmaxf(0.0f, ex2 - mu1_sq), s2 = __builtin_fmaxf(0.0f, ey2 - mu2_sq);
+            const float s12 = exy - mu1 * mu2;
+            const float A = __builtin_fmaf(mu1, mu1, mu2_sq) + SSIM_C1;
             const float B = s1 + s2 + SSIM_C2;
             const float c_top = 2.0f * mu1 * mu2 + SSIM_C1;
             const float d_top = 2.0f * s12 + SSIM_C2;
@@ -238,12 +313,14 @@
             const float inv_ab = inv_a * inv_b;
             const float cd = c_top * d_top * inv_ab;
             const float ssim = clampf(cd, -1.0f, 1.0f);
-            const float2 pg = s_tile[c][(2 * ly + o + HALO) * SW + lx + HALO];
+            float2 pg;
+            if constexpr (GT_PRE) pg = make_float2(s.pred[c][(2 * ly + o + HALO) * SW + lx + HALO], gt_ch_rounded(own_val[o], (uint32_t)c));
+            else pg = s.tile[c][(2 * ly + o + HALO) * SW + lx + HALO];
             float lv = __builtin_fmaf(l1_w, __builtin_fabsf(pg.x - pg.y), ssim_w * ssim);
             if (a.mask) lv = lv * ga[o];
             acc_rgb += lv;
             const bool clamped = cd < -1.0f || cd > 1.0f;
-            const float dmu1 = clamped ? 0.0f : 2.0f * mu2 * inv_ab * (d_top - c_top) - 2.0f * mu1 * cd * (inv_a - inv_b);
+            const float dmu1 = clamped ? 0.0f : __builtin_fmaf(2.0f * mu2 * inv_ab, d_top - c_top, -(2.0f * mu1 * cd * (inv_a - inv_b)));
             const float ds1 = clamped ? 0.0f : -cd * inv_b;
             const float ds12 = clamped ? 0.0f : 2.0f * c_top * inv_ab;
             const size_t p = (size_t)py[o] * a.w + (size_t)pxx;
@@ -274,6 +351,45 @@
     if (rank < 2) {
         const uint32_t tile_row = a.ty_base + 2u * by + (uint32_t)rank;
         if (tile_row < gy) block_sums[(size_t)tile_row * a.gx + bx] = s_red[2 * rank] + s_red[2 * rank + 1];
+    }
+}
+
+__global__ __launch_bounds__(256) void gt_moments_kernel(const uint32_t* __restrict__ gt, float* __restrict__ out , uint32_t h, uint32_t w) {
+    __shared__ uint32_t s_gt[SR * SW];
+    __shared__ float s_h[SR * GP];
+    const int tx0 = (int)blockIdx.x * TW, ty0 = (int)blockIdx.y * TH;
+    const int lx = threadIdx.x, ly = threadIdx.y;
+    const int rank = ly * TW + lx;
+    const size_t plane = (size_t)h * w;
+    for (int i = rank; i < SR * SW; i += 256) {
+        const int r = i / SW, q = i - r * SW;
+        const int y = ty0 + r - HALO, x = tx0 + q - HALO;
+        const bool in = y >= 0 && x >= 0 && y < (int)h && x < (int)w;
+        s_gt[i] = in ? gt[(size_t)y * w + (size_t)x] : 0u;
+    }
+    const int pxx = tx0 + lx;
+    const float tap4 = in_vgpr(tap(4));
+#pragma unroll 1
+    for (int c = 0; c < 3; ++c) {
+        __syncthreads();
+        for (int i = rank; i < SR * (TW / 2); i += 256) {
+            const int r = i / (TW / 2), pair = i - r * (TW / 2);
+            const uint32_t* grow = &s_gt[r * SW + 2 * pair];
+            row_blur_item<MOM_GT>([&](const int k) { return make_float2(0.0f, gt_ch_rounded(grow[k], (uint32_t)c)); }, &s_h[r * GP + (2 * pair) * 2], tap4);
+        }
+        __syncthreads();
+        float v[12][2];
+        column_load<2>(&s_h[(2 * ly) * GP + lx * 2], GP, v);
+#pragma unroll
+        for (int o = 0; o < 2; ++o) {
+            float m[2];
+            column_blur_at<2>(v, o, tap4, m);
+            const int py = ty0 + 2 * ly + o;
+            if (pxx >= (int)w || py >= (int)h) continue;
+            float* q = out + (size_t)(c * 2) * plane + (size_t)py * w + (size_t)pxx;
+            q[0] = m[0];
+            q[plane] = m[1];
+        }
     }
 }
 
@@ -446,7 +562,7 @@
 
 int launch_image_loss_fused_window(bh_ctx* ctx, const float* img_hwc4, const uint32_t* gt, uint32_t h, uint32_t w, const BhLossConfig& cfg,
                                    bool alpha_match, float dl_rgb, float dl_alpha, uint32_t tile_y0, uint32_t tile_y1, float* loss_out,
-                                   float* v_output, float* loss_host, uint32_t* started_host, uint32_t started_tag) {
+                                   float* v_output, float* loss_host, uint32_t* started_host, uint32_t started_tag, const float* gt_moments) {
     const uint32_t gx = (w + LB - 1) / LB, gy = (h + LB - 1) / LB;
     if (tile_y1 > gy) tile_y1 = gy;
     if (tile_y0 >= tile_y1) return set_error(ctx, BH_ERR_INVALID_ARG, "image loss: empty tile-row window");
@@ -476,10 +592,12 @@
         a.row_end = h;
         a.sum_src = nullptr; a.sum_n = 0; a.loss_out = nullptr; a.loss_host = nullptr;
         a.started_host = started_host; a.started_tag = started_tag;
+        a.gt_moments = (gt_moments && !cfg.composite_bg && ctx->knob_gt_moments != 0u) ? gt_moments : nullptr;
         a.gx = gx; a.gy_blocks = (a1 - a0 + 1) / 2;
         a.band_w = banded ? (gx + 7u) / 8u : 0u;
         const dim3 grid_a = banded ? dim3(8u * a.band_w * a.gy_blocks) : dim3(gx, a.gy_blocks);
-        hipLaunchKernelGGL(loss_fused_forward_kernel, grid_a, block, 0, ctx->stream, img_hwc4, gt, partials, block_sums, a1, a);
+        if (a.gt_moments) hipLaunchKernelGGL(loss_fused_forward_kernel<true>, grid_a, block, 0, ctx->stream, img_hwc4, gt, partials, block_sums, a1, a);
+        else hipLaunchKernelGGL(loss_fused_forward_kernel<false>, grid_a, block, 0, ctx->stream, img_hwc4, gt, partials, block_sums, a1, a);
         BH_LAUNCH_CHECK(ctx, "loss_fused_forward_kernel");
     }
     {
@@ -491,6 +609,7 @@
         a.loss_out = loss_out;
         a.loss_host = loss_host;
         a.started_host = nullptr; a.started_tag = 0;
+        a.gt_moments = nullptr;
         a.gy_blocks = (tile_y1 - tile_y0 + 1) / 2;
         const dim3 grid_b = banded ? dim3(8u * a.band_w * a.gy_blocks) : dim3(gx, a.gy_blocks);
         hipLaunchKernelGGL(loss_fused_backward_kernel, grid_b, block, 0, ctx->stream, img_hwc4, gt, partials, v_output, a);
@@ -501,9 +620,24 @@
 
 int launch_image_loss_fused(bh_ctx* ctx, const float* img_hwc4, const uint32_t* gt, uint32_t h, uint32_t w, const BhLossConfig& cfg,
                             bool alpha_match, float dl_rgb, float dl_alpha, float* loss_out, float* v_output, float* loss_host, uint32_t* started_host,
-                            uint32_t started_tag) {
+                            uint32_t started_tag, const float* gt_moments) {
     return launch_image_loss_fused_window(ctx, img_hwc4, gt, h, w, cfg, alpha_match, dl_rgb, dl_alpha, 0, (h + LB - 1) / LB, loss_out, v_output, loss_host,
-                                          started_host, started_tag);
-}
-
-}
+                                          started_host, started_tag, gt_moments);
+}
+
+hipError_t enqueue_gt_moments(hipStream_t st, const uint32_t* gt, uint32_t h, uint32_t w, float* out) {
+    static const int bad_tap = taps_mismatch();
+    if (bad_tap >= 0) return hipErrorNotSupported;
+    hipLaunchKernelGGL(gt_moments_kernel, dim3((w + TW - 1) / TW, (h + TH - 1) / TH), dim3(TW, 16), 0, st, gt, out, h, w);
+    return hipGetLastError();
+}
+
+int launch_gt_moments(bh_ctx* ctx, const uint32_t* gt, uint32_t h, uint32_t w, float* out) {
+    ProfScope ps(ctx, "GtMoments");
+    const hipError_t e = enqueue_gt_moments(ctx->stream, gt, h, w, out);
+    if (e == hipErrorNotSupported) return set_error(ctx, BH_ERR_UNSUPPORTED, "gt_moments: the host's Gaussian taps differ from the kernels' table");
+    if (e != hipSuccess) return check_hip(ctx, e, "gt_moments_kernel");
+    return 0;
+}
+
+}
diff --git a/brush_amd/csrc/train.hip b/brush_amd/csrc/train.hip
--- a/brush_amd/csrc/train.hip
+++ b/brush_amd/csrc/train.hip
@@ -23,6 +23,7 @@
     bh_exposure* exposure = nullptr;
     bh_bilagrid* bilagrid = nullptr;
     bh_envmap* envmap = nullptr;
+    const float* gt_moments = nullptr;
     uint32_t tile_y0 = 0, tile_y1 = 0;
     bool whole_frame = true, window_partial = false;
     bool native_tiles = false, tile_mode = false;
@@ -134,6 +135,12 @@
         if (t.feature_target.h != cam.img_h || t.feature_target.w != cam.img_w)
             return set_error(ctx, BH_ERR_INVALID_ARG, "train_step: the feature term's target size differs from the camera's");
     }
+    if (t.gt_moments_on()) {
+        if (t.gt_moments_h != cam.img_h || t.gt_moments_w != cam.img_w)
+            return set_error(ctx, BH_ERR_INVALID_ARG, "train_step: the GT moments were computed for " + std::to_string(t.gt_moments_w) + " x " + std::to_string(t.gt_moments_h) +
+                                                          " pixels, the camera's image has " + std::to_string(cam.img_w) + " x " + std::to_string(cam.img_h));
+        p.gt_moments = t.gt_moments;
+    }
     p.exchanging = hook || (ctx->comm && (ctx->comm_world > 1 || ctx->knob_force_exchange));
     p.native_tiles = !batch->image_hook && p.window_partial && ctx->comm != nullptr && !hook && (batch->strip_loss || ctx->comm_world > 1);
     if (p.native_tiles && !batch->strip_loss)
@@ -220,7 +227,7 @@
     }
     if (p.tile_mode && batch->strip_loss) {
         return launch_image_loss_fused_window(ctx, w.ro.out_img, batch->gt_packed, p.H, p.W, l.lc, l.alpha_match, l.dl_rgb, l.dl_alpha, p.tile_y0, p.tile_y1,
-                                              w.loss_dev, w.v_output, w.loss_host, started_host, started_tag);
+                                              w.loss_dev, w.v_output, w.loss_host, started_host, started_tag, p.gt_moments);
     }
     if (p.envmap) {
         ProfScope ps(ctx, "EnvMap");
@@ -235,7 +242,7 @@
         BH_TRY(launch_bilagrid_slice(ctx, p.bilagrid, batch->view_id, w.frame(), p.H, p.W, w.corrected));
     }
     return launch_image_loss_fused(ctx, w.corrected ? w.corrected : w.frame(), batch->gt_packed, p.H, p.W, l.lc, l.alpha_match, l.dl_rgb, l.dl_alpha, w.loss_dev, w.v_output,
-                                   w.loss_host, started_host, started_tag);
+                                   w.loss_host, started_host, started_tag, p.gt_moments);
 }
 
 int step_image_loss(bh_ctx* ctx, const StepArgs& a, const StepPlan& p, StepWork& w) {
diff --git a/brush_amd/csrc/upload.hip b/brush_amd/csrc/upload.hip
--- a/brush_amd/csrc/upload.hip
+++ b/brush_amd/csrc/upload.hip
@@ -67,12 +67,15 @@
         uint32_t w = 0, h = 0, channels = 0;
         int state = 0;
         bool consumed_pending = false;
+        float* moments = nullptr;
+        bool has_moments = false;
         void* tab_pinned = nullptr;
         size_t tab_cap = 0;
     };
     std::vector<Slot> slots;
     uint8_t* view_scratch = nullptr;
     size_t view_scratch_cap = 0;
+    bool gt_moments = false;
     uint32_t next = 0;
     std::mutex mu;
     std::string last_error;
@@ -83,6 +86,14 @@
 static int up_fail(bh_uploader* up, int code, const char* msg) {
     if (up) up->last_error = msg;
     return code;
+}
+
+static hipError_t enqueue_slot_moments(bh_uploader* up, bh_uploader::Slot& s, uint32_t w, uint32_t h) {
+    s.has_moments = false;
+    if (!up->gt_moments || !s.moments) return hipSuccess;
+    const hipError_t e = enqueue_gt_moments(up->copy_stream, s.packed, h, w, s.moments);
+    s.has_moments = e == hipSuccess;
+    return e;
 }
 
 extern "C" {
@@ -121,6 +132,7 @@
         if (s.pinned) (void)hipHostFree(s.pinned);
         if (s.raw_dev) (void)hipFree(s.raw_dev);
         if (s.packed) (void)hipFree(s.packed);
+        if (s.moments) (void)hipFree(s.moments);
         if (s.ready) (void)hipEventDestroy(s.ready);
         if (s.consumed) (void)hipEventDestroy(s.consumed);
         if (s.tab_pinned) (void)hipHostFree(s.tab_pinned);
@@ -165,6 +177,7 @@
     const size_t bytes = ((size_t)pixels * channels + 3) & ~(size_t)3;
     hipError_t e = hipMemcpyAsync(s.raw_dev, s.pinned, bytes, hipMemcpyHostToDevice, up->copy_stream);
     if (e == hipSuccess) e = enqueue_pack(up->copy_stream, s.raw_dev, pixels, channels, premultiply, s.packed);
+    if (e == hipSuccess) e = enqueue_slot_moments(up, s, w, h);
     if (e == hipSuccess) e = hipEventRecord(s.ready, up->copy_stream);
     if (e != hipSuccess) {
         (void)hipGetLastError();
@@ -295,6 +308,7 @@
             e = enqueue_pack(st, s.raw_dev, pixels, ch, premul, s.packed);
         }
     }
+    if (e == hipSuccess) e = enqueue_slot_moments(up, s, nw, nh);
     if (e == hipSuccess) e = hipEventRecord(s.ready, st);
     if (e != hipSuccess) return fail_hip(e);
     s.w = nw; s.h = nh; s.channels = cm;
@@ -340,4 +354,30 @@
     return 0;
 }
 
-}
+int bh_uploader_enable_gt_moments(bh_uploader* up, int enable) {
+    if (!up) return BH_ERR_INVALID_ARG;
+    std::lock_guard<std::mutex> lk(up->mu);
+    if (!enable) { up->gt_moments = false; return 0; }
+    if (hipSetDevice(up->ctx->device) != hipSuccess) { (void)hipGetLastError(); return up_fail(up, BH_ERR_HIP, "hipSetDevice"); }
+    for (auto& s : up->slots) {
+        if (s.moments) continue;
+        if (hipMalloc((void**)&s.moments, (size_t)up->max_pixels * BH_GT_MOMENTS_BYTES_PER_PIXEL) != hipSuccess) {
+            (void)hipGetLastError();
+            s.moments = nullptr;
+            return up_fail(up, BH_ERR_OOM, "uploader_enable_gt_moments: out of device memory for the slots' planes");
+        }
+    }
+    up->gt_moments = true;
+    return 0;
+}
+
+int bh_uploader_slot_gt_moments(bh_uploader* up, int slot, const float** planes) {
+    if (!up || slot < 0 || slot >= (int)up->slots.size() || !planes) return BH_ERR_INVALID_ARG;
+    std::lock_guard<std::mutex> lk(up->mu);
+    bh_uploader::Slot& s = up->slots[slot];
+    if (s.state != 3) return up_fail(up, BH_ERR_STATE, "uploader_slot_gt_moments: slot was not acquired");
+    *planes = s.has_moments ? s.moments : nullptr;
+    return 0;
+}
+
+}
diff --git a/brush_amd/host.py b/brush_amd/host.py
--- a/brush_amd/host.py
+++ b/brush_amd/host.py
@@ -1336,8 +1336,26 @@
     return out.permute(1, 2, 0).contiguous()
 
 
+def gt_moments(gt_packed, ctx: Optional[Context] = None, out=None):
+    gt = torch.as_tensor(gt_packed)
+    if gt.device.type != "cuda" or gt.dim() != 2:
+        raise ValueError("gt_moments: a packed [H,W] image on the device")
+    dev = gt.device
+    ctx = ctx or get_context(dev)
+    gt = _as_u32(gt, dev)
+    h, w = (int(v) for v in gt.shape)
+    if out is None:
+        out = torch.empty((3, 2, h, w), dtype=torch.float32, device=dev)
+        if not ctx.uses_torch_stream:
+            torch.cuda.current_stream(dev).synchronize()
+    elif out.dtype != torch.float32 or tuple(out.shape) != (3, 2, h, w) or not out.is_contiguous() or out.device != dev:
+        raise ValueError("gt_moments: out must be a contiguous float32 [3,2,H,W] tensor on the GT's device")
+    ctx.check(ctx.lib.bh_gt_moments(ctx._h, _ptr(gt), h, w, _ptr(out)))
+    return out
+
+
 def image_loss_value_and_grad(img_hwc4, gt_packed, l1_weight=0.8, ssim_weight=-0.2, composite_bg=None, mask=False,
-                              alpha_weight=0.0, ctx: Optional[Context] = None):
+                              alpha_weight=0.0, ctx: Optional[Context] = None, gt_moments=None):
     dev = img_hwc4.device
     ctx = ctx or get_context(dev)
     h, w, c = img_hwc4.shape
@@ -1348,6 +1366,12 @@
     loss = torch.empty(1, dtype=torch.float32, device=dev)
     v_out = torch.empty_like(img)
     cfg = _loss_cfg(l1_weight, ssim_weight, composite_bg, mask)
+    if gt_moments is not None:
+        if gt_moments.dtype != torch.float32 or tuple(gt_moments.shape) != (3, 2, h, w) or not gt_moments.is_contiguous() or gt_moments.device != dev:
+            raise ValueError("gt_moments must be a contiguous float32 [3,2,H,W] tensor on the image's device")
+        ctx.check(ctx.lib.bh_image_loss_value_and_grad_pre(ctx._h, _ptr(img), _ptr(gt), h, w, C.byref(cfg), float(alpha_weight), _ptr(gt_moments),
+                                                           _ptr(loss), _ptr(v_out)))
+        return loss, v_out
     ctx.check(ctx.lib.bh_image_loss_value_and_grad(ctx._h, _ptr(img), _ptr(gt), h, w, C.byref(cfg), float(alpha_weight), _ptr(loss), _ptr(v_out)))
     return loss, v_out
 
@@ -1600,9 +1624,33 @@
     depth_scale: float = 1.0
     depth_offset: float = 0.0
     features: Optional[torch.Tensor] = None
+    keep_gt_moments = True
+    _gt_moments = None
+    _gt_moments_key = None
+    _gt_moments_own = False
 
     def img_size(self):
         return tuple(self.img_packed.shape)
+
+    @staticmethod
+    def _gt_key(gt):
+        return (int(gt.data_ptr()), tuple(gt.shape), int(gt._version))
+
+    def drop_gt_moments(self):
+        self._gt_moments, self._gt_moments_key, self._gt_moments_own = None, None, False
+
+    def gt_moments(self, ctx):
+        gt = self.img_packed
+        if not self.keep_gt_moments or not isinstance(gt, torch.Tensor) or gt.device.type != "cuda" or gt.dim() != 2 \
+                or gt.dtype not in (torch.int32, torch.uint32) or not gt.is_contiguous():
+            return None
+        key = self._gt_key(gt)
+        if self._gt_moments is None or self._gt_moments_key != key:
+            own = self._gt_moments if (self._gt_moments_own and self._gt_moments is not None and tuple(self._gt_moments.shape[2:]) == key[1]) else None
+            self._gt_moments = gt_moments(gt, ctx, out=own)
+            self._gt_moments_own = True
+            self._gt_moments_key = key
+        return self._gt_moments
 
 
 @dataclass
@@ -1644,13 +1692,16 @@
 
 class BatchUploader:
 
-    def __init__(self, max_pixels, slots=3, ctx: Optional[Context] = None):
+    def __init__(self, max_pixels, slots=3, ctx: Optional[Context] = None, gt_moments=False):
         self.ctx = ctx or get_context()
         self.lib = self.ctx.lib
         self._h = C.c_void_p(self.lib.bh_uploader_create(self.ctx._h, int(max_pixels), int(slots)))
         if not self._h:
             raise BrushHipError("bh_uploader_create failed (max_pixels > 0, 2 <= slots <= 16, enough pinned memory)")
         self.max_pixels, self.slots = int(max_pixels), int(slots)
+        self.gt_moments = bool(gt_moments)
+        if self.gt_moments:
+            self._check(self.lib.bh_uploader_enable_gt_moments(self._h, 1))
 
     def close(self):
         if getattr(self, "_h", None):
@@ -1722,6 +1773,13 @@
         self._check(self.lib.bh_uploader_acquire(self._h, int(slot), C.byref(p), C.byref(w), C.byref(h), C.byref(ha)))
         return _view(p.value, (int(h.value), int(w.value)), torch.int32, self.ctx.device), bool(ha.value)
 
+    def slot_gt_moments(self, slot, shape):
+        p = C.c_void_p()
+        self._check(self.lib.bh_uploader_slot_gt_moments(self._h, int(slot), C.byref(p)))
+        if not p.value:
+            return None
+        return _view(p.value, (3, 2, int(shape[0]), int(shape[1])), torch.float32, self.ctx.device)
+
     def release(self, slot):
         self._check(self.lib.bh_uploader_release(self._h, int(slot)))
 
@@ -1729,7 +1787,7 @@
 class SceneLoader:
 
     def __init__(self, views, seed=0, uploader: Optional[BatchUploader] = None, slots=3, rank=0, world=1, ctx: Optional[Context] = None,
-                 max_resolution: Optional[int] = None, image_scale: float = 1.0, invert_masks: bool = False):
+                 max_resolution: Optional[int] = None, image_scale: float = 1.0, invert_masks: bool = False, gt_moments: bool = False):
         import queue
         import threading
         self.views = [v for i, v in enumerate(views) if i % world == rank]
@@ -1748,7 +1806,7 @@
                 px = img.shape[0] * img.shape[1]
                 staged = img.size + (mask.size if mask is not None else 0)
                 mp = max(mp, px, (staged + 3) // 4)
-            uploader = BatchUploader(mp, slots, ctx)
+            uploader = BatchUploader(mp, slots, ctx, gt_moments=gt_moments)
         self.up = uploader
         self._seed = int(seed) & 0xFFFFFFFFFFFFFFFF
         self._q = queue.Queue(maxsize=max(1, self.up.slots - 1))
@@ -1820,6 +1878,11 @@
         self._held = slot
         b = SceneBatch(packed, cam, has_alpha=has_alpha, alpha_is_mask=mask, view_id=self.view_ids[idx])
         b.view_index = idx
+        planes = self.up.slot_gt_moments(slot, packed.shape)
+        if planes is not None:
+            b._gt_moments, b._gt_moments_key = planes, SceneBatch._gt_key(packed)
+        else:
+            b.keep_gt_moments = False
         return b
 
     def close(self):
@@ -2073,6 +2136,14 @@
             terms.append((lib.bh_train_set_distortion, off, off))
         if ff is not None:
             terms.append((lib.bh_train_set_features, (C.byref(ff.as_struct()), C.byref(ft)) if ft is not None else (None, None), (None, None)))
+        planes = None
+        composited = bool(b.has_alpha) and any(float(v) != 0.0 for v in b.background)
+        if not composited and isinstance(batch.img_packed, torch.Tensor) and batch.img_packed.data_ptr() == b.gt_packed and hasattr(batch, "gt_moments"):
+            planes = batch.gt_moments(ctx)
+        if planes is not None:
+            terms.append((lib.bh_train_set_gt_moments, (_ptr(planes), int(planes.shape[2]), int(planes.shape[3])), (None, 0, 0)))
+        else:
+            terms.append((lib.bh_train_set_gt_moments, (None, 0, 0), (None, 0, 0)))
         if self.batch_patch is not None:
             terms.append(lambda: self.batch_patch(b))
         terms.append((lib.bh_train_set_lpips, (self.lpips._h if lw > 0.0 else None, lw if lw > 0.0 else 0.0), None))
@@ -2092,7 +2163,7 @@
             if self.envmap_lr is not None:
                 terms.append(lambda: env.set_lr(self.envmap_lr(step)))
             terms.append((lib.bh_train_set_envmap, (env._h,), off))
-        return terms, (dgt, ftgt), ft
+        return terms, (dgt, ftgt, planes), ft
 
     @staticmethod
     @contextmanager
diff --git a/include/brush_hip.hpp b/include/brush_hip.hpp
--- a/include/brush_hip.hpp
+++ b/include/brush_hip.hpp
@@ -33,6 +33,7 @@
 #include "brush_hip_scene.h"
 #include "brush_hip_lift.h"
 #include "brush_hip_envmap.h"
+#include "brush_hip_gt_moments.h"
 
 namespace brush_hip {
 
@@ -1529,6 +1530,13 @@
     return out;
 }
 
+inline void gt_moments(const Context& ctx, const uint32_t* gt_packed, uint32_t h, uint32_t w, float* out) { ctx.check(bh_gt_moments(ctx.get(), gt_packed, h, w, out)); }
+inline void image_loss_value_and_grad_pre(const Context& ctx, const float* img_hwc4, const uint32_t* gt_packed, uint32_t h, uint32_t w, const BhLossConfig& cfg,
+                                          float alpha_weight, const float* planes, float* loss_out, float* v_output) {
+    ctx.check(bh_image_loss_value_and_grad_pre(ctx.get(), img_hwc4, gt_packed, h, w, &cfg, alpha_weight, planes, loss_out, v_output));
+}
+inline void train_set_gt_moments(const Context& ctx, const float* planes, uint32_t h, uint32_t w) { ctx.check(bh_train_set_gt_moments(ctx.get(), planes, h, w)); }
+
 inline void normal_consistency_value_and_grad(const Context& ctx, const Camera& camera, const float* normal, const float* depth, const float* image,
                                               uint32_t h, uint32_t w, float weight, bool accumulate_v_depth, float* loss, float* v_normal, float* v_depth) {
     static_assert(sizeof(BhNormalTermConfig) == 16, "BhNormalTermConfig layout");
diff --git a/include/brush_hip_gt_moments.h b/include/brush_hip_gt_moments.h
--- /dev/null
+++ b/include/brush_hip_gt_moments.h
@@ -0,0 +1,26 @@
+#ifndef BRUSH_HIP_GT_MOMENTS_H
+#define BRUSH_HIP_GT_MOMENTS_H
+
+#include "brush_hip.h"
+
+#ifdef __cplusplus
+extern "C" {
+#endif
+
+#define BH_GT_MOMENTS_BYTES_PER_PIXEL 24u
+
+int bh_gt_moments(bh_ctx* ctx, const uint32_t* gt_packed , uint32_t h, uint32_t w, float* out );
+
+int bh_image_loss_value_and_grad_pre(bh_ctx* ctx, const float* img_hwc4, const uint32_t* gt_packed, uint32_t h, uint32_t w,
+                                     const BhLossConfig* cfg , float alpha_weight, const float* gt_moments ,
+                                     float* loss_out, float* v_output);
+
+int bh_train_set_gt_moments(bh_ctx* ctx, const float* planes , uint32_t h, uint32_t w);
+
+int bh_uploader_enable_gt_moments(bh_uploader* up, int enable);
+int bh_uploader_slot_gt_moments(bh_uploader* up, int slot, const float** planes );
+
+#ifdef __cplusplus
+}
+#endif
+#endif
```

Result: no change. 1329, median of 6 (+0.4%).
